# rknightion/iq-to-audio

Measured on AMD Instinct MI355X. Metric: complex IQ MS/s end-to-end (ingest->48 kHz audio), higher is better.
Workload: dtype i8; 1 GPU; BASELINE config 2: synthetic 60 s @ 10 MS/s int16 I/Q, 1 NFM channel, +25 kHz, bw 12.5 kHz, D=104, 6401 taps, chunk 4194304; frames_per_gpu=600000000, parallelism=1 independent capture(s), one per GPU; RCCL gather of 48 kHz audio only, audio_samples_48k=2879996, mix_sign=1, settle_steps=55

## Files before the change

### iq-to-audio_amd/batch.py

```python
from __future__ import annotations

from ctypes import c_int32, c_int64, c_void_p

import numpy as np

from . import _dev as D
from . import _native as N
from . import dsp_plan as P
from .decoders.side import NAMES
from .processing import (PRECISION_GUARD, ChannelBank, ChannelDemod, Channelizer, MixSignProbe, Resampler48k, _ChannelKernel,
                         base_precision, immutable_taps, pick_precision, probe_targets, reserve_pinned_scalars)


def reject_wfm(modes) -> None:
    if any((m or "").lower() == "wfm" for m in modes):
        raise ValueError("wfm targets are not supported by the resident batch runners or sharded runs: "
                         "use ProcessingPipeline / MultiChannelPipeline")


def reject_side_decoders(**flags) -> None:
    for name in NAMES:
        if flags.get(name):
            raise ValueError(f"{name}=True is not supported by the resident batch runners or sharded runs: "
                             "use ProcessingPipeline / MultiChannelPipeline")


def _rank(precision: str) -> int:
    return _ChannelKernel.PRECISIONS.index(precision)


class ResidentCaptureRunner:

    SLOTS = 3

    def __init__(self, taps: np.ndarray, *, sample_rate: float, freq_offset: float, decimation: int, fs_channel: float,
                 chunk: int, n_frames: int, demod_mode: str = "nfm", deemph_us: float = 300.0, agc_enabled: bool = True,
                 fmt: str = "s16", iq_order: str = "iq", mix_sign_override: int | None = None, precision: str | None = None,
                 precision_guard: float | None = None, slots: int | None = None, graph_streams: int = 1, pocsag: bool = False,
                 ax25: bool = False, tones: bool = False, acars: bool = False, ais: bool = False, adsb: bool = False):
        reject_wfm([demod_mode])
        reject_side_decoders(pocsag=pocsag, ax25=ax25, tones=tones, acars=acars, ais=ais, adsb=adsb)
        torch = D.torch_mod()
        if slots is not None:
            if slots < 2:
                raise ValueError("at least two slots")
            self.SLOTS = int(slots)
        self.taps, self.fs, self.f_off, self.d, self.fs_ch = immutable_taps(taps), float(sample_rate), float(freq_offset), int(decimation), float(fs_channel)
        self.chunk, self.n_frames, self.fmt, self.iq_order = int(chunk), int(n_frames), fmt, iq_order
        self.demod_args = dict(mode=demod_mode, deemph_us=deemph_us, agc_enabled=agc_enabled)
        self.override = mix_sign_override if mix_sign_override in (1, -1) else None
        self.base_precision = precision or base_precision(demod_mode, agc_enabled)
        self.guard = PRECISION_GUARD if precision_guard is None else float(precision_guard)
        self._guarded = bool(self.guard) and self.override is None and (demod_mode or "").lower() in ("nfm", "fm")
        self._spec_sign, self._spec_precision = 1, self.base_precision
        self.redone = dict(sign=0, precision=0)
        self.n_dec = -(-self.n_frames // self.d)
        self.starts = P.chunk_output_starts(self.chunk, self.d, 0, self.n_frames)
        self.rs = Resampler48k(self.fs_ch)
        self.n48 = self.rs.plan.n_out(self.n_dec)
        self.compute = torch.cuda.current_stream()
        self._compute_raw = int(self.compute.cuda_stream)
        self.aux = D.side_stream("aux")
        self.egress = D.side_stream("egress")
        self._ring_done = None
        self.slots = [dict(z=D.empty(self.n_dec, "complex64"), audio=D.empty(self.n_dec, "float32"),
                           pcm_host=torch.empty(self.n48, dtype=torch.int16).pin_memory(), busy=None,
                           dem=ChannelDemod(demod_mode, self.fs_ch, deemph_us=deemph_us, agc_enabled=agc_enabled))
                      for _ in range(self.SLOTS)]
        self._next = 0
        self._graph_streams = [D.side_stream(f"graph{i}") for i in range(int(graph_streams))] if int(graph_streams) > 1 else []
        self._egress_pending = None
        self.egress_workgroups = 8

    def _probe(self, raw_dev, resident: bool):
        if self.override is not None:
            return None
        torch = D.torch_mod()
        warm = raw_dev[: 2 * min(self.chunk, self.n_frames)] if self.fmt != "f32" else raw_dev[: min(self.chunk, self.n_frames)]
        with D.on_stream(self.aux if resident else self.compute, self.compute):
            return MixSignProbe(warm, self.fs, self.f_off, self.taps, self.d, fmt=self.fmt, iq_order=self.iq_order,
                                record_done=False, measure_level=self._guarded)

    def _kernel_for(self, sign: int):
        return lambda name: Channelizer(self.taps, sample_rate=self.fs, freq_offset=self.f_off, mix_sign=sign, decimation=self.d,
                                        fmt=self.fmt, iq_order=self.iq_order, precision=name)._kernel

    def _needed_precision(self, probe, sign: int) -> str:
        if not self._guarded or probe is None:
            return self.base_precision
        memo = self.__dict__.setdefault("_guard_memo", {}).setdefault(sign, {})
        return pick_precision(self._kernel_for(sign), self.base_precision, self.demod_args["mode"], probe.power, probe.wideband_rms,
                              self.guard, memo)

    def _chain(self, raw_dev, slot, sign: int, events=None, halo=None, resident: bool = False, probe=None, precision: str | None = None,
               make_probe=None):
        torch = D.torch_mod()
        chan = Channelizer(self.taps, sample_rate=self.fs, freq_offset=self.f_off, mix_sign=sign, decimation=self.d,
                           fmt=self.fmt, iq_order=self.iq_order, precision=precision or self.base_precision)
        chan.plan_ahead()
        dem = slot["dem"]
        side = self.aux if resident else None
        with D.on_stream(self.aux if resident else self.compute, self.compute):
            dem.reset(ahead=resident)
        dem.prepare(self.n_dec, self.starts)
        gate = None
        if events is None:
            gate = torch.cuda.Event()
            gate.record(self.compute)
        prev = self._egress_pending
        chan.process(raw_dev, out_dev=slot["z"], events=events, last_block=True, halo=halo, edge_stream=side)
        if make_probe is not None:
            probe = make_probe()
        if events is None:
            ring_done = torch.cuda.Event()
            ring_done.record(self.compute)
        else:
            gate, ring_done = events[0], events[1]
        self._ring_done = ring_done
        if prev is not None:
            self._flush_egress(gate)
        aux_done = None
        if resident:
            aux_done = torch.cuda.Event()
            aux_done.record(self.aux)
            self.compute.wait_event(aux_done)
        if probe is not None:
            probe._done = [aux_done] if resident else [gate]
        dem.process(slot["z"], self.starts, slot["audio"])
        pcm = self.rs.process(slot["audio"], want="pcm16")
        done = torch.cuda.Event()
        ticket = dict(chan=chan, dem=dem, pcm=pcm, done=done, tail_done=None, kernel=chan._kernel.last_kernel,
                      slot=slot, egress_queued=False, resident=resident, precision=chan.precision, probe=probe)
        self._egress_pending = ticket
        return ticket

    def tail_event(self, ticket: dict):
        if ticket.get("tail_done") is None:
            ev = D.torch_mod().cuda.Event()
            ev.record(self.compute)
            ticket["tail_done"] = ev
        return ticket["tail_done"]

    def _flush_egress(self, gate=None) -> None:
        t = self._egress_pending
        if t is None or t["egress_queued"]:
            return
        torch = D.torch_mod()
        if gate is not None:
            self.egress.wait_event(gate)
        else:
            self.egress.wait_event(self.tail_event(t))
        with D.on_stream(self.egress, self.compute):
            t["pcm"].record_stream(self.egress)
            host = t["slot"]["pcm_host"]
            N.call("iqa_trickle_copy", N.ptr(t["pcm"]), c_void_p(host.data_ptr()), c_int64(host.numel() * host.element_size()),
                   c_int32(self.egress_workgroups if gate is not None else max(self.egress_workgroups, 64)), N.stream_ptr())
            t["done"].record(self.egress)
        t["egress_queued"] = True
        self._egress_pending = None

    @staticmethod
    def padded_capture_frames(decimation: int, ntaps: int) -> tuple[int, int]:
        ksteps = -(-2 * decimation // 32)
        return 0, 512 * ksteps + 34 * decimation

    def submit(self, raw_dev, events=None, enclosing=None, lead_frames: int = 0, resident: bool = False) -> dict:
        torch = D.torch_mod()
        if D.current_raw_stream() != self._compute_raw:
            raise RuntimeError("submit() must be called with the stream the runner was created on as the current stream")
        slot = self.slots[self._next % self.SLOTS]
        self._next += 1
        if slot["busy"] is not None:
            self.collect(slot["busy"])
        if resident and self._ring_done is not None:
            self.aux.wait_event(self._ring_done)
        sign = self.override if self.override is not None else self._spec_sign
        halo = (enclosing, int(lead_frames)) if enclosing is not None else None
        if resident:
            ticket = self._chain(raw_dev, slot, sign, events, halo, resident, None, self._spec_precision,
                                 make_probe=lambda: self._probe(raw_dev, True))
        else:
            ticket = self._chain(raw_dev, slot, sign, events, halo, resident, self._probe(raw_dev, resident), self._spec_precision)
        ticket.update(sign=sign, raw=raw_dev, halo=halo)
        slot["busy"] = ticket
        return ticket


    def _captured_step(self, raw_dev, slot, halo):
        sign = self.override or self._spec_sign
        chan = Channelizer(self.taps, sample_rate=self.fs, freq_offset=self.f_off, mix_sign=sign, decimation=self.d,
                           fmt=self.fmt, iq_order=self.iq_order, precision=self._spec_precision)
        chan.plan_ahead()
        dem = slot["dem"]
        probe = None
        if self.override is None:
            warm = raw_dev[: 2 * min(self.chunk, self.n_frames)] if self.fmt != "f32" else raw_dev[: min(self.chunk, self.n_frames)]
            probe = MixSignProbe(warm, self.fs, self.f_off, self.taps, self.d, fmt=self.fmt, iq_order=self.iq_order, record_done=False,
                                 measure_level=self._guarded)
        dem.reset(force=True)
        dem.prepare(self.n_dec, self.starts)
        chan.process(raw_dev, out_dev=slot["z"], last_block=True, halo=halo)
        dem.process(slot["z"], self.starts, slot["audio"])
        pcm = self.rs.process(slot["audio"], want="pcm16")
        host = slot["pcm_host"]
        N.call("iqa_trickle_copy", N.ptr(pcm), c_void_p(host.data_ptr()), c_int64(host.numel() * host.element_size()),
               c_int32(max(self.egress_workgroups, 64)), N.stream_ptr())
        return dict(chan=chan, dem=dem, pcm=pcm, probe=probe, kernel=chan._kernel.last_kernel, sign=sign, precision=chan.precision)

    def submit_captured(self, raw_dev, enclosing=None, lead_frames: int = 0) -> dict:
        torch = D.torch_mod()
        if D.current_raw_stream() != self._compute_raw:
            raise RuntimeError("submit_captured() must be called with the stream the runner was created on as the current stream")
        index = self._next % self.SLOTS
        slot = self.slots[index]
        if slot["busy"] is not None:
            self.collect(slot["busy"])
        halo = (enclosing, int(lead_frames)) if enclosing is not None else None
        def graph_key():
            return (int(raw_dev.data_ptr()), index, None if enclosing is None else int(enclosing.data_ptr()), int(lead_frames),
                    self._spec_sign, self._spec_precision)

        key = graph_key()
        graphs = self.__dict__.setdefault("_graphs", {})
        entry = graphs.get(key)
        if entry is None:
            self.collect(self.submit(raw_dev, enclosing=enclosing, lead_frames=lead_frames))
            key = graph_key()
            torch.cuda.synchronize()
            reserve_pinned_scalars(1)
            g = torch.cuda.CUDAGraph()
            with torch.cuda.graph(g):
                parts = self._captured_step(raw_dev, slot, halo)
            entry = graphs[key] = dict(graph=g, **parts)
        else:
            self._next += 1
        entry["dem"].chunk_sumsq = entry["dem"].chunk_sumsq[-1:]
        done = entry.get("done_event")
        if done is None:
            done = entry["done_event"] = torch.cuda.Event()
        if self._graph_streams:
            side = self._graph_streams[index % len(self._graph_streams)]
            with torch.cuda.stream(side):
                entry["graph"].replay()
                done.record(side)
        else:
            entry["graph"].replay()
            done.record()
        ticket = dict(chan=entry["chan"], dem=entry["dem"], pcm=entry["pcm"], done=done, tail_done=done, kernel=entry["kernel"],
                      slot=slot, egress_queued=True, resident=False, probe=None, graph_probe=entry["probe"],
                      sign=entry["sign"], precision=entry["precision"], raw=raw_dev, halo=halo)
        slot["busy"] = ticket
        return ticket

    def submit_captured_batch(self, captures: list) -> list:
        torch = D.torch_mod()
        if D.current_raw_stream() != self._compute_raw:
            raise RuntimeError("submit_captured_batch() must be called with the stream the runner was created on as the current stream")
        if not 1 <= len(captures) <= self.SLOTS:
            raise ValueError(f"a batch holds 1..{self.SLOTS} captures")
        for slot in self.slots[: len(captures)]:
            if slot["busy"] is not None:
                self.collect(slot["busy"])
        halos = [(enc, int(lead)) if enc is not None else None for _, enc, lead in captures]
        def graph_key():
            return ("batch", self._spec_sign, self._spec_precision) + tuple((int(raw.data_ptr()), None if enc is None else int(enc.data_ptr()), int(lead))
                                                                            for raw, enc, lead in captures)

        key = graph_key()
        graphs = self.__dict__.setdefault("_graphs", {})
        entry = graphs.get(key)
        if entry is None:
            self._next = 0
            for raw, enc, lead in captures:
                self.collect(self.submit(raw, enclosing=enc, lead_frames=lead))
            key = graph_key()
            torch.cuda.synchronize()
            reserve_pinned_scalars(len(captures))
            g = torch.cuda.CUDAGraph()
            with torch.cuda.graph(g):
                parts = [self._captured_step(raw, slot, halo) for (raw, _, _), slot, halo in zip(captures, self.slots, halos)]
            entry = graphs[key] = dict(graph=g, parts=parts)
        for p_ in entry["parts"]:
            p_["dem"].chunk_sumsq = p_["dem"].chunk_sumsq[-1:]
        entry["graph"].replay()
        done = torch.cuda.Event()
        done.record()
        tickets = []
        for (raw, _, _), slot, halo, p_ in zip(captures, self.slots, halos, entry["parts"]):
            t = dict(chan=p_["chan"], dem=p_["dem"], pcm=p_["pcm"], done=done, tail_done=done, kernel=p_["kernel"], slot=slot,
                     egress_queued=True, resident=False, probe=None, graph_probe=p_["probe"], sign=p_["sign"], precision=p_["precision"],
                     raw=raw, halo=halo)
            slot["busy"] = t
            tickets.append(t)
        return tickets

    def collect(self, ticket: dict) -> dict:
        slot = ticket["slot"]
        if ticket.get("collected"):
            return ticket["result"]
        if ticket.get("graph_probe") is not None:
            ticket["done"].synchronize()
            sign = ticket["graph_probe"].peek()
            need = self._needed_precision(ticket["graph_probe"], sign)
            self._spec_sign, self._spec_precision = sign, need
            if sign != ticket["sign"] or _rank(need) > _rank(ticket["precision"]):
                self.replays_redone = getattr(self, "replays_redone", 0) + 1
                self.redone["sign" if sign != ticket["sign"] else "precision"] += 1
                redo = self._chain(ticket["raw"], slot, sign, None, ticket.get("halo"), False, precision=need)
                self._flush_egress()
                ticket.update(redo, sign=sign, probe=None, raw=ticket["raw"], graph_probe=None)
        if D.current_raw_stream() != self._compute_raw:
            raise RuntimeError("collect() must be called with the stream the runner was created on as the current stream")
        sign = ticket["sign"]
        if self._egress_pending is ticket:
            self._flush_egress()
        if ticket["probe"] is not None:
            sign = ticket["probe"].result()
            need = self._needed_precision(ticket["probe"], sign)
            self._spec_sign, self._spec_precision = sign, need
            if sign != ticket["sign"] or _rank(need) > _rank(ticket["precision"]):
                self.redone["sign" if sign != ticket["sign"] else "precision"] += 1
                ticket["done"].synchronize()
                probe, raw = ticket["probe"], ticket["raw"]
                redo = self._chain(raw, slot, sign, None, ticket.get("halo"), ticket.get("resident", False), precision=need)
                self._flush_egress()
                ticket.update(redo, sign=sign, probe=probe, raw=raw)
        ticket["done"].synchronize()
        ticket["collected"] = True
        ticket["raw"] = ticket["pcm"] = None
        if slot["busy"] is ticket:
            slot["busy"] = None
        ticket["result"] = dict(pcm_host=slot["pcm_host"], sign=int(sign), audio=slot["audio"], z=slot["z"],
                                kernel=ticket["kernel"], demod=ticket["dem"], done=ticket["done"], precision=ticket["precision"])
        return ticket["result"]


class ResidentBankRunner:

    SLOTS = 3

    def __init__(self, targets: list, *, sample_rate: float, n_frames: int, chunk_size: int = 1_048_576,
                 fs_ch_target: float = 96_000.0, fmt: str = "s16", iq_order: str = "iq", precision_guard: float | None = None,
                 pocsag: bool = False, ax25: bool = False, tones: bool = False, acars: bool = False, ais: bool = False, adsb: bool = False):
        reject_wfm([t.get("demod_mode") for t in targets])
        reject_side_decoders(pocsag=pocsag, ax25=ax25, tones=tones, acars=acars, ais=ais, adsb=adsb)
        torch = D.torch_mod()
        if not targets:
            raise ValueError("at least one target is required")
        self.fs, self.n_frames, self.fmt, self.iq_order = float(sample_rate), int(n_frames), fmt, iq_order
        self.d, self.fs_ch = P.choose_decimation(self.fs, fs_ch_target)
        self.chunk = P.tune_chunk_size(self.fs, chunk_size)
        self.n_dec = -(-self.n_frames // self.d)
        self.starts = P.chunk_output_starts(self.chunk, self.d, 0, self.n_frames)
        self.rs = Resampler48k(self.fs_ch)
        self.n48 = self.rs.plan.n_out(self.n_dec)
        self.targets = []
        for t in targets:
            spec = dict(bandwidth=12_500.0, demod_mode="nfm", deemph_us=300.0, agc_enabled=True, mix_sign=None, precision=None)
            spec.update(t)
            spec["taps"] = immutable_taps(P.design_channel_filter(self.fs, spec["bandwidth"], self.d))
            spec["base_precision"] = spec["precision"] or base_precision(spec["demod_mode"], spec["agc_enabled"])
            self.targets.append(spec)
        self.guard = PRECISION_GUARD if precision_guard is None else float(precision_guard)
        self._spec_sign = [1] * len(self.targets)
        self._spec_precision = [s["base_precision"] for s in self.targets]
        self.redone = dict(sign=0, precision=0)
        self.slots = []
        for _ in range(self.SLOTS):
            per = [dict(z=D.empty(self.n_dec, "complex64"), audio=D.empty(self.n_dec, "float32"),
                        pcm_host=torch.empty(self.n48, dtype=torch.int16).pin_memory(),
                        dem=ChannelDemod(s["demod_mode"], self.fs_ch, deemph_us=s["deemph_us"], agc_enabled=s["agc_enabled"]))
                   for s in self.targets]
            self.slots.append(dict(per=per, busy=None, probe_host=torch.zeros(2 * len(self.targets) + 1, dtype=torch.float64).pin_memory()))
        self._next = 0

    def _channelizer(self, spec, sign: int, precision: str | None = None) -> Channelizer:
        return Channelizer(spec["taps"], sample_rate=self.fs, freq_offset=spec["freq_offset"], mix_sign=sign, decimation=self.d,
                           fmt=self.fmt, iq_order=self.iq_order, precision=precision or spec["base_precision"])

    def _guarded(self, spec) -> bool:
        return bool(self.guard) and spec["mix_sign"] not in (1, -1) and (spec["demod_mode"] or "").lower() in ("nfm", "fm")

    def _needed_precision(self, spec, probe, sign: int) -> str:
        if probe is None or not self._guarded(spec):
            return spec["base_precision"]
        memo = spec.setdefault("_guard_memo", {}).setdefault(sign, {})
        return pick_precision(lambda name: self._channelizer(spec, sign, name)._kernel, spec["base_precision"], spec["demod_mode"],
                              probe.power, probe.wideband_rms, self.guard, memo)

    def _finish_target(self, per, raw_unused=None) -> None:
        dem = per["dem"]
        dem.reset()
        dem.process(per["z"], self.starts, per["audio"])
        pcm = self.rs.process(per["audio"], want="pcm16")
        per["pcm_host"].copy_(pcm, non_blocking=True)
        per["pcm"] = pcm

    def submit(self, raw_dev, enclosing=None, lead_frames: int = 0, events=None) -> dict:
        torch = D.torch_mod()
        slot = self.slots[self._next % self.SLOTS]
        self._next += 1
        if slot["busy"] is not None:
            self.collect(slot["busy"])
        warm = raw_dev[: 2 * min(self.chunk, self.n_frames)] if self.fmt != "f32" else raw_dev[: min(self.chunk, self.n_frames)]
        main = torch.cuda.current_stream()
        side = D.side_stream("tail")
        arrived = torch.cuda.Event()
        arrived.record(main)
        side.wait_event(arrived)
        probes = self._queue_probes(warm, slot)
        signs = [s["mix_sign"] if s["mix_sign"] in (1, -1) else sp for s, sp in zip(self.targets, self._spec_sign)]
        precisions = list(self._spec_precision)
        chans = [self._channelizer(s, sg, pr) for s, sg, pr in zip(self.targets, signs, precisions)]
        for c in chans:
            c.plan_ahead()
        halo = (enclosing, int(lead_frames)) if enclosing is not None else None
        return self._submit_rest(raw_dev, slot, probes, signs, precisions, chans, halo, events, main, side)

    def _queue_probes(self, warm, slot) -> list:
        todo = [i for i, s in enumerate(self.targets) if s["mix_sign"] not in (1, -1)]
        grouped = probe_targets(warm, self.fs, [(self.targets[i]["freq_offset"], self.targets[i]["taps"]) for i in todo], self.d,
                                fmt=self.fmt, iq_order=self.iq_order, host=slot["probe_host"]) if len(todo) > 1 else None
        if grouped is not None:
            probes = [None] * len(self.targets)
            for i, pr in zip(todo, grouped):
                probes[i] = pr
        else:
            probes = [None if s["mix_sign"] in (1, -1) else
                      MixSignProbe(warm, self.fs, s["freq_offset"], s["taps"], self.d, fmt=self.fmt, iq_order=self.iq_order,
                                   measure_level=self._guarded(s))
                      for s in self.targets]
        return probes

    def _submit_rest(self, raw_dev, slot, probes, signs, precisions, chans, halo, events, main, side) -> dict:
        torch = D.torch_mod()
        if events:
            events[0].record()
        bank = ChannelBank(chans)
        bank.process(raw_dev, outs=[p["z"] for p in slot["per"]], last_block=True, halo=halo)
        if events:
            events[1].record()
        self.last_bank_launches = getattr(bank, "launches", None) or [bank.last_launch]
        after_pass = torch.cuda.Event()
        after_pass.record(main)
        side.wait_event(after_pass)
        for per in slot["per"]:
            with D.on_stream(side, main):
                self._finish_target(per)
                for key in ("z", "audio"):
                    per[key].record_stream(side)
        done = torch.cuda.Event()
        done.record(side)
        ticket = dict(slot=slot, probes=probes, signs=signs, precisions=[c.precision for c in chans], raw=raw_dev, halo=halo, done=done,
                      launch=bank.last_launch, kernel=chans[0]._kernel.last_kernel, collected=False)
        slot["busy"] = ticket
        return ticket

    def collect(self, ticket: dict) -> list:
        if ticket["collected"]:
            return ticket["result"]
        slot = ticket["slot"]
        ticket["done"].synchronize()
        redo = False
        for i, (probe, per, spec) in enumerate(zip(ticket["probes"], slot["per"], self.targets)):
            if probe is None:
                continue
            sign = probe.result()
            need = self._needed_precision(spec, probe, sign)
            self._spec_sign[i], self._spec_precision[i] = sign, need
            if sign != ticket["signs"][i] or _rank(need) > _rank(ticket["precisions"][i]):
                self.redone["sign" if sign != ticket["signs"][i] else "precision"] += 1
                ticket["signs"][i] = sign
                chan = self._channelizer(spec, sign, need)
                ticket["precisions"][i] = chan.precision
                chan.process(ticket["raw"], out_dev=per["z"], last_block=True, halo=ticket["halo"])
                self._finish_target(per)
                redo = True
        if redo:
            D.torch_mod().cuda.current_stream().synchronize()
        ticket["collected"] = True
        ticket["raw"] = None
        if slot["busy"] is ticket:
            slot["busy"] = None
        ticket["result"] = [dict(pcm_host=per["pcm_host"], pcm=per.get("pcm"), audio=per["audio"], z=per["z"], sign=int(sg), demod=per["dem"], precision=pr)
                            for per, sg, pr in zip(slot["per"], ticket["signs"], ticket["precisions"])]
        return ticket["result"]


def demodulate_sharded(targets: list, *, sample_rate: float, n_frames: int, axis: str, capture=None, captures=None,
                       chunk_size: int = 1_048_576, fmt: str = "s16", iq_order: str = "iq", pocsag: bool = False,
                       ax25: bool = False, tones: bool = False, acars: bool = False, ais: bool = False, adsb: bool = False):
    from . import dist as DS

    reject_wfm([t.get("demod_mode") for t in targets])
    reject_side_decoders(pocsag=pocsag, ax25=ax25, tones=tones, acars=acars, ais=ais, adsb=adsb)
    torch = D.torch_mod()
    if axis not in ("channels", "captures"):
        raise ValueError("axis must be 'channels' or 'captures'")

    def run_bank(specs, raw_dev):
        runner = ResidentBankRunner(specs, sample_rate=sample_rate, n_frames=n_frames, chunk_size=chunk_size, fmt=fmt, iq_order=iq_order)
        res = runner.collect(runner.submit(raw_dev))
        return [(r["pcm"].clone(), r["demod"].peak) for r in res]

    if axis == "channels":
        dtype = {"s16": torch.int16, "u8": torch.uint8, "f32": torch.float32}[fmt]
        shared = dict(tensor=capture, numel=2 * n_frames, dtype=dtype, device=D.device())
        return DS.run_sharded(list(targets), run_bank, shared=shared)

    def every_target_of(mine, _):
        out = []
        for unit in mine:
            raw = (unit() if callable(unit) else unit).to(D.device())
            res = run_bank(list(targets), raw)
            out.append((torch.cat([a for a, _ in res]), max(p for _, p in res)))
        return out

    got, peak = DS.run_sharded(list(captures), every_target_of)
    if got is not None:
        got = {k: v.reshape(len(targets), -1) for k, v in got.items()}
    return got, peak
```

### iq-to-audio_amd/channelizer.py

```python
from __future__ import annotations

import threading
from collections import OrderedDict
from ctypes import byref, c_double, c_int32, c_int64, c_void_p

import numpy as np

from . import _dev as D
from . import _native as N
from . import dsp_plan as P
from . import iqio


def _as_frames(raw, fmt: str):
    if fmt == "f32":
        is_c = raw.is_complex() if D.is_tensor(raw) else np.iscomplexobj(raw)
        if is_c:
            x = D.to_device(raw, "complex64")
            return x, int(x.numel())
        x = D.to_device(raw, "float32").reshape(-1)
        return x, int(x.numel()) // 2
    x = D.to_device(raw, {"s16": "int16", "u8": "uint8"}[fmt]).reshape(-1)
    return x, int(x.numel()) // 2


def _block_size(n: int, ranges: int, floor: int, cap: int = 1 << 24) -> int:
    return int(min(cap, max(floor, -(-(-(-n // ranges)) // 32) * 32)))


def _tap_unit(group, fmt: str) -> float:
    return group.unit / (256.0 if fmt == "u8" else 1.0)


def _launch_lanes(lanes: list, pairs: bool, outputs_per_block: int, raw_dev, n_frames: int, consumed: int, m_first: int,
                  n_out: int) -> None:
    (k0, ps0), fmt = lanes[0][:2], lanes[0][0].plan.fmt
    table = (N.MfmaLane * len(lanes))()
    for lane, spec in zip(table, lanes):
        if spec is None:
            continue
        k, ps, z_out, partial_in, partial_out, raw_partials = spec
        group = k.mfma.groups[ps.group]
        lane.afrag_dev = k.afrag_dev[ps.group][ps.k_first * P.MFMA_KSTEP_BYTES :].data_ptr()
        lane.z_out_dev, lane.partial_in_dev, lane.partial_out_dev = z_out, partial_in, partial_out
        lane.unit = _tap_unit(group, fmt)
        lane.c_re, lane.c_im = ps.c_re, ps.c_im
        lane.rot_step, lane.rot_base = k.params.rot_step, k.params.rot_base
        lane.out_scale_re, lane.out_scale_im = k.params.out_scale_re, k.params.out_scale_im
        lane.conj_sum, lane.rotate = k.params.conj_sum, k.params.rotate
        lane.q_group, lane.finalize, lane.raw_partials = group.q, int(partial_out is None), int(raw_partials)
        lane.reserved = (0 if k.acc32 else 1) | (2 if group.high_only else 0)
        k.last_kernel = f"k_channelize_mfma_{fmt}_ring"
    N.call("iqa_channelize_mfma_pairs" if pairs else "iqa_channelize_mfma_multi", c_int32(P.FMT_CODE[fmt]),
           c_int32(k0.plan.decimation), c_int32(ps0.k_first), c_int32(ps0.k_count), c_int32(outputs_per_block), table,
           c_int32(len(lanes)), N.ptr(raw_dev), c_int64(n_frames), c_int64(consumed), c_int64(m_first), c_int64(n_out),
           N.stream_ptr())


class _ChannelKernel:

    use_mfma = True
    mfma_variant = "ring"
    ring_acc32 = True
    RING_ROWS_KSTEPS = 11
    mfma_min_outputs = 32768

    PRECISIONS = ("fast", "fine", "full", "float32")

    def __init__(self, plan: P.ChannelPlan, exact: bool = False, precision: str | None = None):
        self.plan = plan
        precision = precision or ("float32" if exact else "fast")
        if precision not in self.PRECISIONS:
            raise ValueError(f"precision must be one of {self.PRECISIONS}, not {precision!r}")
        if plan.fmt == "f32" and precision != "fast":
            precision = "float32"
        if plan.fmt == "u8" and precision == "full":
            precision = "fine"
        self.precision = precision
        self.exact = precision == "float32"
        self.variant = self.mfma_variant
        self.acc32 = bool(self.ring_acc32) and precision != "full"
        self.residual = precision in ("fine", "full")
        lpad = int(N.lib().iqa_taps_padded_len(plan.ntaps))
        if plan.taps_window.size != lpad:
            raise ValueError("tap window padding does not match the library")
        self.taps_dev = D.from_numpy(plan.taps_window)
        self.params = N.ChanParams(
            fmt=P.FMT_CODE[plan.fmt], ntaps=plan.ntaps, decimation=plan.decimation, conj_sum=plan.conj_sum,
            rotate=plan.rotate, reserved=0, rot_step=plan.rot_step, rot_base=plan.rot_base,
            out_scale_re=float(np.real(plan.out_scale)), out_scale_im=float(np.imag(plan.out_scale)),
        )
        self.mfma = None
        self._lock = threading.Lock()
        self.last_kernel = "k_channelize_v1"
        ks_all = -(-2 * plan.decimation // 32)
        self._ring_mode = 0
        if plan.fmt in ("s16", "u8") and self.variant == "ring":
            acc32, code = int(bool(self.acc32)), P.FMT_CODE[plan.fmt]
            self._ring_mode = int(N.lib().iqa_mfma_ring_mode(code, plan.decimation, 0, ks_all, acc32))
            if self._ring_mode == 0:
                self._ring_mode = int(N.lib().iqa_mfma_ring_mode(code, plan.decimation, 0, min(ks_all, self.RING_ROWS_KSTEPS), acc32))
        self._mfma_ok = bool(self.use_mfma and not self.exact and P.mfma_supported(plan) and (plan.fmt == "s16" or self._ring_mode == 2))

    def _ensure_mfma(self):
        with self._lock:
            if self.mfma is None:
                ring = self.variant == "ring" and self._ring_mode != 0
                mp = P.plan_mfma(self.plan, acc32=ring and self.acc32,
                                 max_ksteps=self.RING_ROWS_KSTEPS if self._ring_mode == 2 else None, residual=self.residual)
                self.afrag_dev = [D.from_numpy(g.afrag.reshape(-1).view(np.uint8)) for g in mp.groups]
                self._passes = [(ps, None if ring else N.MfmaParams(
                    reserved=0, unit=mp.groups[ps.group].unit, c_re=ps.c_re, c_im=ps.c_im, q_group=mp.groups[ps.group].q,
                    k_first=ps.k_first, k_count=ps.k_count)) for ps in mp.passes]
                self.mfma = mp
            return self.mfma

    def fixed_point_error_norm(self) -> float:
        return float(self._ensure_mfma().err_norm) if self._mfma_ok else 0.0

    def fixed_point_error_rms(self, wideband_rms: float) -> float:
        return float(self._ensure_mfma().z_error_rms(wideband_rms)) if self._mfma_ok else 0.0

    @staticmethod
    def _plain_range_max(k_count: int) -> int:
        lds = 160 * 1024 - k_count * P.MFMA_KSTEP_BYTES
        return int(min(6144, (lds // 16 - 160) // 32 * 32))

    launch_blocks = 256

    @classmethod
    def _block_outputs(cls, n_out: int, rmax: int, per_cu: int = 1) -> int:
        blocks = cls.launch_blocks * per_cu
        rounds = max(1, -(-n_out // (blocks * rmax)))
        return _block_size(n_out, blocks * rounds, 512, rmax)

    def _workgroups_per_cu(self, ps) -> int:
        lds = int(N.lib().iqa_mfma_ring_lds_bytes(P.FMT_CODE[self.plan.fmt], self.plan.decimation, ps.k_first, ps.k_count,
                                                  1 if self.acc32 else 0))
        return 2 if 0 < lds <= 80 * 1024 else 1

    def _valu(self, raw_dev, n_frames, consumed, hist_dev, m_first, n_out, out_dev):
        if n_out > 0:
            N.call("iqa_channelize", byref(self.params), N.ptr(self.taps_dev), N.ptr(raw_dev), c_int64(n_frames),
                   c_int64(consumed), N.ptr(hist_dev), c_int64(m_first), c_int64(n_out), N.ptr(out_dev), N.stream_ptr())

    def _interior(self, consumed: int, n_frames: int, m_first: int, n_out: int) -> tuple[int, int]:
        d = self.plan.decimation
        ksteps = -(-2 * d // 32)
        n_groups = max(1, -(-(-(-self.plan.ntaps // d)) // P.MFMA_Q))
        m_a, m_b = P.mfma_interior(consumed, n_frames, m_first, n_out, d, ksteps, n_groups)
        if self.variant == "ring" and self._ring_mode == 1:
            m_b = min(m_b, (n_frames + consumed - 512 * ksteps - 1) // d + 2)
        return (m_a, m_b) if m_b > m_a else (m_first, m_first)

    def _mfma_passes(self, raw_dev, n_frames: int, consumed: int, m_a: int, n_int: int, out_dev, min_block: int = 512):
        self._ensure_mfma()
        buf = D.empty(2 * n_int, "float64") if len(self._passes) > 1 else None
        partial = N.ptr(buf).value
        for i, (ps, prm) in enumerate(self._passes):
            last = i == len(self._passes) - 1
            partial_in, partial_out = (partial if i > 0 else None), (None if last else partial)
            if prm is None:
                rng = self._block_outputs(n_int, 1 << 24, self._workgroups_per_cu(ps))
                if min_block < 512:
                    rng = _block_size(n_int, 256, min_block, rng)
                _launch_lanes([(self, ps, out_dev.data_ptr() if last else None, partial_in, partial_out, False)], False, rng,
                              raw_dev, n_frames, consumed, m_a, n_int)
            else:
                self.last_kernel = "k_channelize_mfma_s16"
                afrag = self.afrag_dev[ps.group][ps.k_first * P.MFMA_KSTEP_BYTES :]
                with self._lock:
                    prm.outputs_per_block = self._block_outputs(n_int, self._plain_range_max(ps.k_count))
                    prm.finalize = int(last)
                    prm.partial_in_dev, prm.partial_out_dev = partial_in, partial_out
                    N.call("iqa_channelize_mfma", byref(self.params), byref(prm), N.ptr(afrag), N.ptr(raw_dev),
                           c_int64(n_frames), c_int64(consumed), c_int64(m_a), c_int64(n_int), N.ptr(out_dev), N.stream_ptr())

    def run_interior_only(self, raw_dev, n_frames: int, m_first: int, n_out: int, out_dev) -> bool:
        if not (self._mfma_ok and self.variant == "ring" and self._ring_mode) or n_out < 64:
            return False
        m_a, m_b = self._interior(0, n_frames, m_first, n_out)
        if m_a != m_first or m_b != m_first + n_out:
            return False
        self._mfma_passes(raw_dev, n_frames, 0, m_first, n_out, out_dev, min_block=64)
        return True

    def _edges(self, edge_stream, *args):
        if edge_stream is None:
            return self._valu(*args)
        with D.torch_mod().cuda.stream(edge_stream):
            self._valu(*args)

    def run(self, raw_dev, n_frames: int, consumed: int, hist_dev, m_first: int, n_out: int, out_dev=None,
            events=None, halo=None, edge_stream=None):
        if out_dev is None:
            out_dev = D.empty(n_out, "complex64")
        self.last_kernel = "k_channelize_v1"
        if self._mfma_ok and n_out >= self.mfma_min_outputs:
            big, big_frames, big_consumed = raw_dev, n_frames, consumed
            if halo is not None:
                big, lead = halo
                big_frames, big_consumed = int(big.numel()) // 2, consumed - int(lead)
            m_a, m_b = self._interior(big_consumed, big_frames, m_first, n_out)
            if m_b - m_a >= self.mfma_min_outputs:
                self._edges(edge_stream, raw_dev, n_frames, consumed, hist_dev, m_first, m_a - m_first, out_dev)
                if events:
                    events[0].record()
                self._mfma_passes(big, big_frames, big_consumed, m_a, m_b - m_a, out_dev[m_a - m_first :])
                if events:
                    events[1].record()
                self._edges(edge_stream, raw_dev, n_frames, consumed, hist_dev, m_b, m_first + n_out - m_b,
                            out_dev[m_b - m_first :])
                return out_dev
        if events:
            events[0].record()
        self._valu(raw_dev, n_frames, consumed, hist_dev, m_first, n_out, out_dev)
        if events:
            events[1].record()
        return out_dev


_KERNEL_CACHE: "OrderedDict[tuple, tuple]" = OrderedDict()
_KERNEL_CACHE_MAX = 192
_KERNEL_CACHE_LOCK = threading.Lock()


_TAPS_MEMO: dict = {}


def _taps_fingerprint(taps: np.ndarray):
    frozen = (not taps.flags.writeable) and taps.base is None
    if frozen:
        memo = _TAPS_MEMO.get(id(taps))
        if memo is not None and memo[0] is taps:
            return memo[1], memo[2]
    raw = taps.tobytes()
    h = hash(raw)
    if frozen:
        with _KERNEL_CACHE_LOCK:
            if len(_TAPS_MEMO) >= 64:
                _TAPS_MEMO.clear()
            _TAPS_MEMO[id(taps)] = (taps, raw, h)
    return raw, h


def immutable_taps(taps) -> np.ndarray:
    out = np.array(taps, copy=True, order="C")
    out.setflags(write=False)
    return out


def _cached_kernel(taps: np.ndarray, *, sample_rate: float, freq_offset: float, mix_sign: int, decimation: int,
                   fmt: str, iq_order: str, exact: bool = False, precision: str | None = None):
    taps = np.ascontiguousarray(taps)
    raw, raw_hash = _taps_fingerprint(taps)
    key = (raw_hash, taps.dtype.str, taps.shape, float(sample_rate), float(freq_offset), int(mix_sign), int(decimation),
           fmt, iq_order, _ChannelKernel.use_mfma, _ChannelKernel.mfma_variant, _ChannelKernel.ring_acc32,
           precision or ("float32" if exact else "fast"), D.torch_mod().cuda.current_device())
    with _KERNEL_CACHE_LOCK:
        hit = _KERNEL_CACHE.get(key)
        if hit is not None and (hit[0] is raw or hit[0] == raw):
            _KERNEL_CACHE.move_to_end(key)
            return hit[1], hit[2]
    lpad = int(N.lib().iqa_taps_padded_len(len(taps)))
    plan = P.plan_channel(taps, sample_rate=sample_rate, freq_offset=freq_offset, mix_sign=mix_sign,
                          decimation=decimation, fmt=fmt, iq_order=iq_order, padded_len=lpad)
    kernel = _ChannelKernel(plan, exact, precision)
    with _KERNEL_CACHE_LOCK:
        _KERNEL_CACHE[key] = (raw, plan, kernel)
        while len(_KERNEL_CACHE) > _KERNEL_CACHE_MAX:
            _KERNEL_CACHE.popitem(last=False)
    return plan, kernel


class Channelizer:

    def __init__(self, taps: np.ndarray, *, sample_rate: float, freq_offset: float, mix_sign: int, decimation: int,
                 fmt: str = "s16", iq_order: str = "iq", exact: bool = False, precision: str | None = None):
        self.plan, self._kernel = _cached_kernel(taps, sample_rate=sample_rate, freq_offset=freq_offset, mix_sign=mix_sign,
                                                 decimation=decimation, fmt=fmt, iq_order=iq_order, exact=exact, precision=precision)
        self.precision = self._kernel.precision
        self.fmt = fmt
        self.decimation = int(decimation)
        self.ntaps = len(taps)
        self.consumed = 0
        self._hist = None

    def plan_ahead(self) -> None:
        if self._kernel._mfma_ok:
            self._kernel._ensure_mfma()

    def outputs_for(self, n_frames: int) -> tuple[int, int]:
        d = self.decimation
        m_first = -(-self.consumed // d)
        m_end = -(-(self.consumed + n_frames) // d)
        return m_first, m_end - m_first

    def process(self, raw, out_dev=None, events=None, last_block: bool = False, halo=None, edge_stream=None):
        x, n = _as_frames(raw, self.fmt)
        if n == 0:
            return D.like_input(D.empty(0, "complex64"), raw)
        m_first, n_out = self.outputs_for(n)
        if halo is not None and (self.fmt not in ("s16", "u8") or not D.is_tensor(raw)):
            halo = None
        z = None
        if n_out and D.is_tensor(raw) and self._several_lanes():
            if events:
                events[0].record()
            zs = ChannelBank([self])._run_shared(x, n, m_first, n_out, [out_dev], halo, edge_stream)
            if zs is not None:
                z = zs[0]
                if events:
                    events[1].record()
        if z is None:
            z = (self._kernel.run(x, n, self.consumed, self._hist, m_first, n_out, out_dev, events, halo, edge_stream)
                 if n_out else D.empty(0, "complex64"))
        self._advance(x, n, last_block)
        return D.like_input(z, raw)

    def _several_lanes(self) -> bool:
        k = self._kernel
        if not (self.lanes_for_groups and self.fmt in ("s16", "u8") and ChannelBank._lane_capable(k)):
            return False
        return len(k._ensure_mfma().groups) > 1

    lanes_for_groups = True

    def _advance(self, x, n: int, last_block: bool = False) -> None:
        keep = 0 if last_block else self.ntaps - 1
        if keep:
            nxt = D.empty(keep * iqio.FRAME_BYTES[self.fmt], "uint8")
            N.call("iqa_history_update", c_int32(P.FMT_CODE[self.fmt]), c_int32(self.ntaps), N.ptr(self._hist),
                   N.ptr(x), c_int64(n), N.ptr(nxt), N.stream_ptr())
            self._hist = nxt
        self.consumed += n


class ChannelBank:

    MAX_LANES = 16
    pair_lanes = True

    def __init__(self, channelizers: list):
        if not channelizers:
            raise ValueError("a bank needs at least one channelizer")
        self.chans = list(channelizers)
        first = self.chans[0]
        self.fmt, self.decimation = first.fmt, first.decimation
        for c in self.chans:
            if (c.fmt, c.decimation, c.consumed) != (self.fmt, self.decimation, first.consumed):
                raise ValueError("the channels of a bank share the capture: same sample format, decimation and position")
        self.last_launch = None

    @staticmethod
    def _lane_capable(k) -> bool:
        return bool(k._mfma_ok and k.variant == "ring" and k._ring_mode and (k.acc32 or k._ring_mode == 1))

    def _shared_shape(self) -> bool:
        ks = [c._kernel for c in self.chans]
        if not ks or not all(self._lane_capable(k) for k in ks) or len({k.acc32 for k in ks}) != 1:
            return False
        if len(ks) == 1:
            return len(ks[0]._ensure_mfma().groups) > 1
        return len({k._ring_mode for k in ks}) == 1

    def process(self, raw, outs=None, last_block: bool = False, halo=None, edge_stream=None) -> list:
        x, n = _as_frames(raw, self.fmt)
        outs = list(outs) if outs is not None else [None] * len(self.chans)
        first = self.chans[0]
        m_first, n_out = first.outputs_for(n)
        zs = None
        if n and n_out and D.is_tensor(raw) and self._shared_shape():
            zs = self._run_shared(x, n, m_first, n_out, outs, halo, edge_stream)
        if zs is None:
            self.last_launch = None
            capable = [i for i, c in enumerate(self.chans) if self._lane_capable(c._kernel)]
            widths = sorted({self.chans[i]._kernel.acc32 for i in capable}, reverse=True)
            if D.is_tensor(raw) and capable and (len(capable) < len(self.chans) or len(widths) > 1):
                res = [None] * len(self.chans)
                self.last_launch, self.launches = None, []
                for acc32 in widths:
                    lanes = [i for i in capable if self.chans[i]._kernel.acc32 == acc32]
                    sub = ChannelBank([self.chans[i] for i in lanes])
                    got = sub.process(raw, outs=[outs[i] for i in lanes], last_block=last_block, halo=halo, edge_stream=edge_stream)
                    self.launches.append(sub.last_launch)
                    if self.last_launch is None:
                        self.last_launch = sub.last_launch
                    for i, z in zip(lanes, got):
                        res[i] = z
                for i, (c, o) in enumerate(zip(self.chans, outs)):
                    if res[i] is None:
                        res[i] = c.process(raw, out_dev=o, last_block=last_block, halo=halo)
                return res
            return [c.process(raw, out_dev=o, last_block=last_block, halo=halo) for c, o in zip(self.chans, outs)]
        for c in self.chans:
            c._advance(x, n, last_block)
        return zs

    def run_interior_only(self, x_all, n_frames: int, m_first: int, n_out: int, outs: list) -> bool:
        if n_out < 64 or not self._shared_shape():
            return False
        kernels = [c._kernel for c in self.chans]
        plans = [k._ensure_mfma() for k in kernels]
        if len(kernels) > self.MAX_LANES or any(len(mp.groups) != 1 or len(mp.passes) != 1 for mp in plans):
            return self._run_shared(x_all, n_frames, m_first, n_out, list(outs), None, None, interior_only=True) is not None
        if any(k._interior(0, n_frames, m_first, n_out) != (m_first, m_first + n_out) for k in kernels):
            return False
        if len({(mp.passes[0].k_first, mp.passes[0].k_count) for mp in plans}) != 1:
            return False
        rng = _block_size(n_out, 8 * max(1, (_ChannelKernel.launch_blocks // 8) // len(kernels)), 64)
        _launch_lanes([(k, mp.passes[0], z.data_ptr(), None, None, False) for k, mp, z in zip(kernels, plans, outs)], False,
                      rng, x_all, n_frames, 0, m_first, n_out)
        self.last_launch = dict(lanes=len(kernels), launches=1, combines=0, pairs=0)
        return True

    def _run_shared(self, x, n: int, m_first: int, n_out: int, outs: list, halo, edge_stream=None, interior_only: bool = False):
        kernels = [c._kernel for c in self.chans]
        consumed = self.chans[0].consumed
        big, big_frames, big_consumed = x, n, consumed
        if halo is not None:
            big, lead = halo
            big_frames, big_consumed = int(big.numel()) // 2, consumed - int(lead)
        spans = [k._interior(big_consumed, big_frames, m_first, n_out) for k in kernels]
        m_a, m_b = max(s[0] for s in spans), min(s[1] for s in spans)
        if interior_only:
            if any(s != (m_first, m_first + n_out) for s in spans):
                return None
        elif any(s[1] <= s[0] for s in spans) or m_b - m_a < _ChannelKernel.mfma_min_outputs:
            return None
        n_int = m_b - m_a
        plans = [k._ensure_mfma() for k in kernels]
        if len({tuple((ps.k_first, ps.k_count) for ps in mp.passes if ps.group == 0) for mp in plans}) != 1:
            return None
        zs = [o if o is not None else D.empty(n_out, "complex64") for o in outs]
        if not interior_only:
            for c, k, z in zip(self.chans, kernels, zs):
                k._edges(edge_stream, x, n, consumed, c._hist, m_first, m_a - m_first, z)
                k._edges(edge_stream, x, n, consumed, c._hist, m_b, m_first + n_out - m_b, z[m_b - m_first :])
        kranges = [(ps.k_first, ps.k_count) for ps in plans[0].passes if ps.group == 0]
        ids = [(ci, gi) for ci, mp in enumerate(plans) for gi in range(len(mp.groups))]
        need_partial = {(ci, gi): (len(kranges) > 1 or len(plans[ci].groups) > 1) for ci, gi in ids}
        acc32 = bool(kernels[0].acc32)
        raw = len(kranges) == 1 and acc32
        partial = {key: D.empty(2 * n_int, "int32" if raw else "float64") for key, needed in need_partial.items() if needed}
        cpx = max(1, _ChannelKernel.launch_blocks // 8)
        launches = 0

        def launch(part, pairs: bool, units: int) -> None:
            nonlocal launches
            rng = _block_size(n_int, 8 * max(1, cpx // units), 128)
            for ri, (k_first, _) in enumerate(kranges):
                lanes = []
                for ident in part:
                    if ident is None:
                        lanes.append(None)
                        continue
                    ci, gi = ident
                    mp = plans[ci]
                    ps = next(p_ for p_ in mp.passes if p_.group == gi and p_.k_first == k_first)
                    fin = ri == len(kranges) - 1 and len(mp.groups) == 1
                    buf = partial.get((ci, gi))
                    lanes.append((kernels[ci], ps, zs[ci][m_a - m_first :].data_ptr() if fin else None,
                                  buf.data_ptr() if (buf is not None and ri > 0) else None, None if fin else buf.data_ptr(),
                                  raw and not fin))
                _launch_lanes(lanes, pairs, rng, big, big_frames, big_consumed, m_a, n_int)
                launches += 1

        if self.pair_lanes and len(kranges) == 1 and (N.lib().iqa_mfma_ring_lanes(P.FMT_CODE[self.fmt], self.decimation, *kranges[0], int(acc32)) & 2):
            paired = sorted(ids, key=lambda i: -plans[i[0]].groups[i[1]].q)
            if len(paired) & 1:
                paired.append(None)
            for lo in range(0, len(paired), self.MAX_LANES):
                part = paired[lo : lo + self.MAX_LANES]
                launch(part, True, len(part) // 2)
            n_pairs = len(paired) // 2
        else:
            n_pairs = 0
            for lo in range(0, len(ids), self.MAX_LANES):
                part = ids[lo : lo + self.MAX_LANES]
                launch(part, False, len(part))
        main = None
        if edge_stream is not None and any(len(mp.groups) > 1 for mp in plans):
            torch = D.torch_mod()
            main = torch.cuda.current_stream()
            passed = torch.cuda.Event()
            passed.record(main)
            edge_stream.wait_event(passed)
            for t in partial.values():
                t.record_stream(edge_stream)
            torch.cuda.set_stream(edge_stream)
        try:
            combines = self._combine(plans, kernels, partial, raw, m_a, m_first, n_int, zs)
        finally:
            if main is not None:
                D.torch_mod().cuda.set_stream(main)
        self.last_launch = dict(lanes=len(ids), launches=launches, combines=combines, pairs=n_pairs)
        return zs

    def _combine(self, plans, kernels, partial, raw, m_a, m_first, n_int, zs) -> int:
        combines = 0
        for ci, mp in enumerate(plans):
            if len(mp.groups) > 1:
                ptrs = (c_void_p * len(mp.groups))(*[partial[(ci, gi)].data_ptr() for gi in range(len(mp.groups))])
                scale = None
                if raw:
                    vals = []
                    for gi in range(len(mp.groups)):
                        ps = next(p_ for p_ in mp.passes if p_.group == gi)
                        vals += [_tap_unit(mp.groups[gi], self.fmt), ps.c_re, ps.c_im]
                    scale = (c_double * len(vals))(*vals)
                N.call("iqa_mfma_combine", byref(kernels[ci].params), ptrs, c_int32(len(mp.groups)), scale, c_int64(m_a),
                       c_int64(n_int), N.ptr(zs[ci][m_a - m_first :]), N.stream_ptr())
                combines += 1
        return combines
```

### iq-to-audio_amd/csrc/channelize_mfma.hip

```cpp
#include "mfma_common.h"

#include <atomic>
#include <cmath>
#include <type_traits>

namespace iqa {

__global__ __launch_bounds__(MF_THREADS, 2) void k_channelize_mfma_s16(MfmaArgs a)
{
    extern __shared__ __attribute__((aligned(16))) char smem[];
    const int tid = threadIdx.x, lane = tid & 63, wave = tid >> 6;
    const int col = lane & 31, h = lane >> 5;

    const long long i0 = static_cast<long long>(blockIdx.x) * a.range;
    const int cnt = static_cast<int>(min(static_cast<long long>(a.range), a.n_out - i0));
    const long long m0 = a.m_lo + i0;
    const int tiles = (cnt + 63 + 31) >> 5;
    const int acc_len = tiles * 32 + MF_Q + 4;

    const bool stamp = (a.debug & 2) && a.stamps != nullptr;
    unsigned long long t_begin = 0, t_loop0 = 0, t_scatter = 0, t_loop1 = 0;
    if (stamp) t_begin = __builtin_amdgcn_s_memtime();
    v4i_t *s_a = reinterpret_cast<v4i_t *>(smem);
    int *s_acc = reinterpret_cast<int *>(smem + static_cast<size_t>(a.ksteps) * MF_KSTEP_BYTES);
    {
        const int n16 = a.ksteps * (MF_KSTEP_BYTES / 16);
        for (int i0f = tid; i0f < n16; i0f += MF_THREADS * 8) {
            v4i_t tmp[8];
#pragma unroll
            for (int u = 0; u < 8; ++u) {
                const int i = i0f + u * MF_THREADS;
                tmp[u] = (i < n16) ? a.afrag[i] : v4i_t{0, 0, 0, 0};
            }
#pragma unroll
            for (int u = 0; u < 8; ++u) {
                const int i = i0f + u * MF_THREADS;
                if (i < n16) s_a[i] = tmp[u];
            }
        }
    }
    for (int i = tid; i < 4 * acc_len; i += MF_THREADS) s_acc[i] = 0;
    __syncthreads();

    int pf_tile = wave, pf_ks = 0;
    auto row_ptr = [&](int tile) -> const int * {
        const long long b = m0 - MF_Q - a.col_shift + tile * 32 + col;
        return a.raw + (b * a.D + 1 - a.consumed) + 16 * a.k_first + 8 * h;
    };
    const int *pf_row = row_ptr(min(pf_tile, tiles - 1));
#define MF_LOAD_PAIR(X0, X1)                                                        \
    {                                                                               \
        X0 = *reinterpret_cast<const v4i_a4 *>(pf_row + 16 * pf_ks);                \
        X1 = *reinterpret_cast<const v4i_a4 *>(pf_row + 16 * pf_ks + 4);            \
        if (++pf_ks == a.ksteps) {                                                  \
            pf_ks = 0;                                                              \
            pf_tile += MF_WAVES;                                                    \
            pf_row = row_ptr(min(pf_tile, tiles - 1));   \
        }                                                                           \
    }
    v4i_t a0, a1, b0, b1;
    MF_LOAD_PAIR(a0, a1);
    MF_LOAD_PAIR(b0, b1);
    v4i_t fr[2 * MF_ROWTILES];
    {
        const v4i_t *fa = s_a + lane;
#pragma unroll
        for (int i = 0; i < 2 * MF_ROWTILES; ++i) fr[i] = fa[i * 64];
    }
    v16i_t acc1[MF_ROWTILES], acc2[MF_ROWTILES];
#pragma unroll
    for (int rt = 0; rt < MF_ROWTILES; ++rt) {
        acc1[rt] = v16i_t{0};
        acc2[rt] = v16i_t{0};
    }
    const v16i_t zero16 = {0, 0, 0, 0, 0, 0, 0, 0, 0, 0, 0, 0, 0, 0, 0, 0};
    if (stamp) t_loop0 = __builtin_amdgcn_s_memtime();
    int t = wave, ks = 0;
    const bool skip_scatter = (a.debug & 1) != 0;

#define MF_PAIR(X0, X1)                                                                              \
    {                                                                                                \
        v4i_t hi, lo;                                                                                \
        hi.x = __builtin_amdgcn_perm(X0.y, X0.x, 0x07050301);                                        \
        hi.y = __builtin_amdgcn_perm(X0.w, X0.z, 0x07050301);                                        \
        hi.z = __builtin_amdgcn_perm(X1.y, X1.x, 0x07050301);                                        \
        hi.w = __builtin_amdgcn_perm(X1.w, X1.z, 0x07050301);                                        \
        lo.x = __builtin_amdgcn_perm(X0.y, X0.x, 0x06040200) ^ 0x80808080;                           \
        lo.y = __builtin_amdgcn_perm(X0.w, X0.z, 0x06040200) ^ 0x80808080;                           \
        lo.z = __builtin_amdgcn_perm(X1.y, X1.x, 0x06040200) ^ 0x80808080;                           \
        lo.w = __builtin_amdgcn_perm(X1.w, X1.z, 0x06040200) ^ 0x80808080;                           \
        MF_LOAD_PAIR(X0, X1);                                                                        \
        const int kn = (ks + 1 < a.ksteps) ? ks + 1 : 0;                                             \
        const v4i_t *fa = s_a + kn * (MF_KSTEP_BYTES / 16) + lane;                                   \
        if (ks == 0) {      \
            _Pragma("unroll") for (int rt = 0; rt < MF_ROWTILES; ++rt)                               \
            {                                                                                        \
                acc1[rt] = __builtin_amdgcn_mfma_i32_32x32x32_i8(fr[2 * rt], hi, zero16, 0, 0, 0);   \
                acc2[rt] = __builtin_amdgcn_mfma_i32_32x32x32_i8(fr[2 * rt], lo, zero16, 0, 0, 0);   \
                acc2[rt] = __builtin_amdgcn_mfma_i32_32x32x32_i8(fr[2 * rt + 1], hi, acc2[rt], 0, 0, 0); \
                fr[2 * rt] = fa[(2 * rt) * 64];                                                      \
                fr[2 * rt + 1] = fa[(2 * rt + 1) * 64];                                              \
            }                                                                                        \
        } else {                                                                                     \
            _Pragma("unroll") for (int rt = 0; rt < MF_ROWTILES; ++rt)                               \
            {                                                                                        \
                acc1[rt] = __builtin_amdgcn_mfma_i32_32x32x32_i8(fr[2 * rt], hi, acc1[rt], 0, 0, 0); \
                acc2[rt] = __builtin_amdgcn_mfma_i32_32x32x32_i8(fr[2 * rt], lo, acc2[rt], 0, 0, 0); \
                acc2[rt] = __builtin_amdgcn_mfma_i32_32x32x32_i8(fr[2 * rt + 1], hi, acc2[rt], 0, 0, 0); \
                fr[2 * rt] = fa[(2 * rt) * 64];                                                      \
                fr[2 * rt + 1] = fa[(2 * rt + 1) * 64];                                              \
            }                                                                                        \
        }                                                                                            \
        if (++ks == a.ksteps) {    \
            unsigned long long ts0 = 0;                                                              \
            if (stamp) ts0 = __builtin_amdgcn_s_memtime();                                           \
            if (!skip_scatter) {                                                                     \
                int *base = s_acc + (t * 32 + col + 4 * h + 1);                                      \
                _Pragma("unroll") for (int rt = 0; rt < MF_ROWTILES; ++rt)                           \
                {                                                                                    \
                    int *p1 = base + (rt >> 1) * acc_len + (rt & 1) * 32;                            \
                    int *p2 = p1 + 2 * acc_len;                                                      \
                    _Pragma("unroll") for (int r = 0; r < 16; ++r)                                   \
                    {                                                                                \
                        const int off = (r & 3) + 8 * (r >> 2);                                      \
                        atomicAdd(p1 + off, acc1[rt][r]);                                            \
                        atomicAdd(p2 + off, acc2[rt][r]);                                            \
                    }                                                                                \
                }                                                                                    \
            } else {                                                                                 \
                _Pragma("unroll") for (int rt = 0; rt < MF_ROWTILES; ++rt)                           \
                    asm volatile("" ::"v"(acc1[rt]), "v"(acc2[rt]));                                 \
            }                                                                                        \
            if (stamp) {                                                                             \
                asm volatile("s_waitcnt lgkmcnt(0)" ::: "memory");                                   \
                t_scatter += __builtin_amdgcn_s_memtime() - ts0;                                     \
            }                                                                                        \
            ks = 0;                                                                                  \
            t += MF_WAVES;                                                                           \
        }                                                                                            \
    }

    while (t < tiles) {
        MF_PAIR(a0, a1);
        if (t >= tiles) break;
        MF_PAIR(b0, b1);
    }
#undef MF_PAIR
#undef MF_LOAD_PAIR
    if (stamp) t_loop1 = __builtin_amdgcn_s_memtime();
    __syncthreads();

    mfma_emit<MF_THREADS>(a, s_acc, acc_len, cnt, i0, m0, tid);
    if (stamp && lane == 0) {
        const unsigned long long t_end = __builtin_amdgcn_s_memtime();
        unsigned long long *o = a.stamps + (static_cast<size_t>(blockIdx.x) * MF_WAVES + wave) * 8;
        o[0] = t_loop0 - t_begin;
        o[1] = t_loop1 - t_loop0;
        o[2] = t_scatter;
        o[3] = t_end - t_loop1;
        o[4] = static_cast<unsigned long long>((tiles - wave + MF_WAVES - 1) / MF_WAVES);
    }
}

}

using namespace iqa;

extern "C" int64_t iqa_mfma_ring_bytes(int32_t decimation)
{
    if (decimation < 1 || !mfma_ring_supported(decimation)) return 0;
    return static_cast<int64_t>(mfma_ring_lds_bytes((2 * decimation + 31) / 32, false, false));
}

extern "C" int64_t iqa_mfma_ring_lds_bytes(int32_t fmt, int32_t decimation, int32_t k_first, int32_t k_count, int32_t acc32)
{
    if (decimation < 1 || (fmt != IQA_FMT_S16 && fmt != IQA_FMT_U8)) return 0;
    const int ks_all = (2 * decimation + 31) / 32;
    const int ks = k_count > 0 ? k_count : ks_all - k_first;
    const int mode = mfma_ring_mode(decimation, k_first, ks, acc32 == 0, fmt == IQA_FMT_U8);
    return mode ? static_cast<int64_t>(mfma_ring_lds_bytes(ks, mode == 2, fmt == IQA_FMT_U8)) : 0;
}

extern "C" int32_t iqa_mfma_ring_mode(int32_t fmt, int32_t decimation, int32_t k_first, int32_t k_count, int32_t acc32)
{
    if (decimation < 1 || (fmt != IQA_FMT_S16 && fmt != IQA_FMT_U8)) return 0;
    return mfma_ring_mode(decimation, k_first, k_count, acc32 == 0, fmt == IQA_FMT_U8);
}

extern "C" int64_t iqa_mfma_afrag_bytes(int32_t decimation)
{
    if (decimation < 1) return 0;
    const int64_t ksteps = (2 * static_cast<int64_t>(decimation) + 31) / 32;
    return ksteps * MF_KSTEP_BYTES;
}

static int channelize_mfma_lanes(int32_t fmt, int32_t decimation, int32_t k_first, int32_t k_count, int32_t outputs_per_block,
                                 const iqa_mfma_lane *lanes, int32_t n_lanes, const void *raw_dev, int64_t n_frames, int64_t consumed,
                                 int64_t m_first, int64_t n_out, void *stream, bool pairs);

extern "C" int iqa_channelize_mfma(const iqa_chan_params *p, const iqa_mfma_params *q, const void *afrag_dev,
                                   const void *raw_dev, int64_t n_frames, int64_t consumed, int64_t m_first,
                                   int64_t n_out, void *z_out_dev, void *stream)
{
    if (p == nullptr || q == nullptr) return fail_inval("params is NULL");
    const bool ring = (q->reserved & 64) != 0;
    if (p->fmt != IQA_FMT_S16 && !(p->fmt == IQA_FMT_U8 && ring))
        return fail_inval("the MFMA channelizer takes int16 captures (and uint8 ones with the ring variant) only");
    if (p->ntaps <= 0 || p->decimation < 1) return fail_inval("bad ntaps/decimation");
    const int64_t D = p->decimation;
    if (n_out < 0 || n_frames < 0 || m_first < 0) return fail_inval("negative size");
    if (n_out == 0) return IQA_OK;
    if (!afrag_dev || !raw_dev || !z_out_dev) return fail_inval("NULL device pointer");
    const int ksteps_all = static_cast<int>((2 * D + 31) / 32);
    const int k_first = q->k_first;
    const int ksteps = q->k_count > 0 ? q->k_count : ksteps_all - k_first;
    if (k_first < 0 || ksteps <= 0 || k_first + ksteps > ksteps_all) return fail_inval("bad k-step range");
    if (q->q_group < 0) return fail_inval("bad q group");
    if (!q->finalize && !q->partial_out_dev) return fail_inval("non-final pass needs partial_out_dev");
    int range = q->outputs_per_block;
    if (range <= 0 || (range & 31)) return fail_inval("outputs_per_block must be a positive multiple of 32");
    if (ring) {
        iqa_mfma_lane l{};
        l.afrag_dev = afrag_dev;
        l.z_out_dev = z_out_dev;
        l.partial_in_dev = q->partial_in_dev;
        l.partial_out_dev = q->partial_out_dev;
        l.unit = q->unit;
        l.c_re = q->c_re;
        l.c_im = q->c_im;
        l.rot_step = p->rot_step;
        l.rot_base = p->rot_base;
        l.out_scale_re = p->out_scale_re;
        l.out_scale_im = p->out_scale_im;
        l.q_group = q->q_group;
        l.finalize = q->finalize;
        l.conj_sum = p->conj_sum;
        l.rotate = p->rotate;
        l.reserved = (q->reserved & 128) ? 0 : 1;
        return channelize_mfma_lanes(p->fmt, p->decimation, k_first, ksteps, range, &l, 1, raw_dev, n_frames, consumed, m_first, n_out,
                                     stream, false);
    }
    const int64_t blocks = (n_out + range - 1) / range;
    const int64_t last_cnt = n_out - (blocks - 1) * range;
    const int64_t last_tiles = (last_cnt + 63 + 31) / 32;
    const int64_t col_shift = static_cast<int64_t>(MF_Q) * q->q_group;
    const int64_t b_min = m_first - MF_Q - col_shift;
    const int64_t b_max = m_first + (blocks - 1) * range - MF_Q - col_shift + last_tiles * 32 - 1;
    const int64_t f_min = b_min * D + 1 - consumed;
    const int64_t f_max = b_max * D + 1 - consumed + 16LL * (k_first + ksteps) - 1;
    const int64_t full_tiles = (static_cast<int64_t>(range) + 63 + 31) / 32;
    const int64_t b_max_full = blocks > 1 ? m_first + (blocks - 2) * range - MF_Q - col_shift + full_tiles * 32 - 1 : b_max;
    const int64_t f_max_full = b_max_full * D + 1 - consumed + 16LL * (k_first + ksteps) - 1;
    if (f_min < 0 || f_max >= n_frames || f_max_full >= n_frames)
        return fail_inval("MFMA channelizer range reads outside the block (use iqa_channelize for the edges)");
    const int64_t acc_len = full_tiles * 32 + MF_Q + 4;
    const size_t lds = static_cast<size_t>(ksteps) * MF_KSTEP_BYTES + 4 * acc_len * sizeof(int);
    if (lds > 160 * 1024) return fail_inval("tap fragments + accumulators exceed 160 KiB of LDS");

    MfmaArgs a{};
    a.afrag = static_cast<const v4i_t *>(afrag_dev);
    a.raw = static_cast<const int *>(raw_dev);
    a.out = static_cast<float2 *>(z_out_dev);
    a.consumed = consumed;
    a.m_lo = m_first;
    a.n_out = n_out;
    a.D = static_cast<int>(D);
    a.ksteps = ksteps;
    a.range = range;
    a.k_first = k_first;
    a.col_shift = static_cast<int>(col_shift);
    a.finalize = q->finalize;
    a.partial_in = static_cast<const double2 *>(q->partial_in_dev);
    a.partial_out = static_cast<double2 *>(q->partial_out_dev);
    a.debug = q->reserved;
    a.stamps = static_cast<unsigned long long *>(q->debug_stamps);
    a.unit = q->unit;
    a.c_re = q->c_re;
    a.c_im = q->c_im;
    a.conj_sum = p->conj_sum;
    a.rotate = p->rotate;
    a.rot_step = p->rot_step;
    a.rot_base = p->rot_base;
    a.sc_re = p->out_scale_re;
    a.sc_im = p->out_scale_im;
    {
        static std::atomic<unsigned long long> done{0};
        int dev = 0;
        (void)hipGetDevice(&dev);
        const unsigned long long bit = 1ull << (dev & 63);
        if (!(done.load(std::memory_order_acquire) & bit)) {
            const hipError_t e = hipFuncSetAttribute(reinterpret_cast<const void *>(k_channelize_mfma_s16),
                                                     hipFuncAttributeMaxDynamicSharedMemorySize, 160 * 1024);
            if (e != hipSuccess) {
                set_error("k_channelize_mfma_s16: cannot raise the dynamic LDS limit on device %d: %s", dev, hipGetErrorString(e));
                return IQA_EHIP;
            }
            done.fetch_or(bit, std::memory_order_release);
        }
    }
    hipLaunchKernelGGL(k_channelize_mfma_s16, dim3(static_cast<unsigned>(blocks)), dim3(MF_THREADS), lds,
                       as_stream(stream), a);
    return check_launch("k_channelize_mfma_s16");
}


static int channelize_mfma_lanes(int32_t fmt, int32_t decimation, int32_t k_first, int32_t k_count, int32_t outputs_per_block,
                                 const iqa_mfma_lane *lanes, int32_t n_lanes, const void *raw_dev, int64_t n_frames, int64_t consumed,
                                 int64_t m_first, int64_t n_out, void *stream, bool pairs)
{
    if (lanes == nullptr || n_lanes < 1) return fail_inval("no lanes");
    const bool u8 = fmt == IQA_FMT_U8;
    if (fmt != IQA_FMT_S16 && !u8) return fail_inval("the MFMA channelizer takes int16 and uint8 captures only");
    if (decimation < 1) return fail_inval("bad decimation");
    const int64_t D = decimation;
    if (n_out < 0 || n_frames < 0 || m_first < 0) return fail_inval("negative size");
    if (n_out == 0) return IQA_OK;
    if (!raw_dev) return fail_inval("NULL device pointer");
    const int ksteps_all = static_cast<int>((2 * D + 31) / 32);
    const int ksteps = k_count > 0 ? k_count : ksteps_all - k_first;
    if (k_first < 0 || ksteps <= 0 || k_first + ksteps > ksteps_all) return fail_inval("bad k-step range");
    const int range = outputs_per_block;
    if (range <= 0 || (range & 31)) return fail_inval("outputs_per_block must be a positive multiple of 32");
    const bool acc64 = (lanes[0].reserved & 1) != 0;
    for (int i = 1; i < n_lanes; ++i)
        if (lanes[i].afrag_dev && ((lanes[i].reserved & 1) != 0) != acc64) return fail_inval("the lanes of a launch share the sum width (reserved bit 0)");
    const int ring_mode = mfma_ring_mode(static_cast<int>(D), k_first, ksteps, acc64, u8);
    if (ring_mode == 0) return fail_inval("the ring kernel does not cover this (decimation, k-step range, sum width): see iqa_mfma_ring_mode");
    if (acc64 && ring_mode != 1) return fail_inval("64-bit sums: contiguous slots only");
    if (pairs && !mfma_ring_pairs_supported(static_cast<int>(D), k_first, ksteps, u8, acc64))
        return fail_inval("lane pairs are not available for this (format, decimation, k-step range, sum width): see iqa_mfma_ring_lanes");
    int q_max = 0, q_min = INT32_MAX;
    for (int i = 0; i < n_lanes; ++i) {
        if (lanes[i].q_group < 0) return fail_inval("bad q group");
        if (!lanes[i].afrag_dev) {
            if (pairs && (i & 1)) continue;
            return fail_inval("lane without tap fragments");
        }
        if (lanes[i].finalize ? !lanes[i].z_out_dev : !lanes[i].partial_out_dev) return fail_inval("lane without an output buffer");
        q_max = lanes[i].q_group > q_max ? lanes[i].q_group : q_max;
        q_min = lanes[i].q_group < q_min ? lanes[i].q_group : q_min;
    }
    const int64_t blocks = (n_out + range - 1) / range;
    const int64_t last_cnt = n_out - (blocks - 1) * range;
    const int64_t last_tiles = (last_cnt + 63 + 31) / 32, full_tiles = (static_cast<int64_t>(range) + 63 + 31) / 32;
    const int64_t f_min = (m_first - MF_Q - static_cast<int64_t>(MF_Q) * q_max) * D + 1 - consumed;
    const int64_t tail = ring_mode == 1 ? 512LL * ksteps : 16LL * (k_first + ksteps);
    const int64_t b_last = m_first - MF_Q - static_cast<int64_t>(MF_Q) * q_min;
    const int64_t t_last = b_last + (blocks - 1) * range + (last_tiles - 1) * 32;
    const int64_t t_full = blocks > 1 ? b_last + (blocks - 2) * range + (full_tiles - 1) * 32 : t_last;
    const int64_t row_span = ring_mode == 1 ? 0 : 31;
    if (f_min < 0 || (t_last + row_span) * D + 1 - consumed + tail > n_frames || (t_full + row_span) * D + 1 - consumed + tail > n_frames)
        return fail_inval("multi-lane ring launch reads outside the block (use iqa_channelize for the edges)");
    const size_t lds = mfma_ring_lds_bytes(ksteps, ring_mode == 2, u8);
    if (lds == 0 || lds > 160 * 1024) return fail_inval("ring + window exceed 160 KiB of LDS");

    MfmaArgs a{};
    a.raw = static_cast<const int *>(raw_dev);
    a.consumed = consumed;
    a.m_lo = m_first;
    a.n_out = n_out;
    a.D = static_cast<int>(D);
    a.ksteps = ksteps;
    a.range = range;
    a.k_first = k_first;
    a.debug = 64 | (acc64 ? 0 : 128);
    MfmaLane packed[16];
    if (n_lanes > 16) return fail_inval("at most 16 lanes per launch");
    for (int i = 0; i < n_lanes; ++i) {
        const iqa_mfma_lane &s = lanes[i];
        MfmaLane &l = packed[i];
        l.afrag = static_cast<const v4i_t *>(s.afrag_dev);
        l.out = static_cast<float2 *>(s.z_out_dev);
        l.partial_in = static_cast<const double2 *>(s.partial_in_dev);
        l.partial_out = static_cast<double2 *>(s.partial_out_dev);
        l.unit = s.unit;
        l.c_re = s.c_re;
        l.c_im = s.c_im;
        l.rot_step = s.rot_step;
        l.rot_base = s.rot_base;
        const unsigned long long st = s.rot_step * 64ULL;
        const double turns = static_cast<double>(st >> 11) * (1.0 / 9007199254740992.0);
        l.rot64_re = std::cos(2.0 * M_PI * turns);
        l.rot64_im = std::sin(2.0 * M_PI * turns);
        l.sc_re = s.out_scale_re;
        l.sc_im = s.out_scale_im;
        l.col_shift = MF_Q * s.q_group;
        l.finalize = s.finalize;
        l.conj_sum = s.conj_sum;
        l.rotate = s.rotate;
        l.raw_partials = (s.raw_partials != 0 && !s.finalize && !s.partial_in_dev) ? 1 : 0;
        if (s.raw_partials && !l.raw_partials) return fail_inval("raw partials need finalize == 0 and no partial_in");
        if (s.raw_partials && acc64) return fail_inval("raw partials are int32 sums: not with 64-bit sums");
        l.high_taps_only = (s.reserved & 2) != 0 ? 1 : 0;
    }
    return mfma_ring_launch_multi(a, packed, n_lanes, lds, as_stream(stream), ring_mode == 2, u8, pairs, acc64);
}

extern "C" int iqa_channelize_mfma_multi(int32_t fmt, int32_t decimation, int32_t k_first, int32_t k_count,
                                         int32_t outputs_per_block, const iqa_mfma_lane *lanes, int32_t n_lanes,
                                         const void *raw_dev, int64_t n_frames, int64_t consumed, int64_t m_first,
                                         int64_t n_out, void *stream)
{
    return channelize_mfma_lanes(fmt, decimation, k_first, k_count, outputs_per_block, lanes, n_lanes, raw_dev, n_frames, consumed,
                                 m_first, n_out, stream, false);
}

extern "C" int iqa_channelize_mfma_pairs(int32_t fmt, int32_t decimation, int32_t k_first, int32_t k_count,
                                         int32_t outputs_per_block, const iqa_mfma_lane *lanes, int32_t n_lanes,
                                         const void *raw_dev, int64_t n_frames, int64_t consumed, int64_t m_first,
                                         int64_t n_out, void *stream)
{
    return channelize_mfma_lanes(fmt, decimation, k_first, k_count, outputs_per_block, lanes, n_lanes, raw_dev, n_frames, consumed,
                                 m_first, n_out, stream, true);
}

extern "C" int32_t iqa_mfma_ring_lanes(int32_t fmt, int32_t decimation, int32_t k_first, int32_t k_count, int32_t acc32)
{
    if (decimation < 1 || (fmt != IQA_FMT_S16 && fmt != IQA_FMT_U8)) return 0;
    const bool u8 = fmt == IQA_FMT_U8, acc64 = acc32 == 0;
    const int ks_all = (2 * decimation + 31) / 32;
    const int ks = k_count > 0 ? k_count : ks_all - k_first;
    const int mode = mfma_ring_mode(decimation, k_first, ks, acc64, u8);
    if (mode == 0 || (acc64 && mode != 1)) return 0;
    return 1 | (mfma_ring_pairs_supported(decimation, k_first, ks, u8, acc64) ? 2 : 0);
}

extern "C" int32_t iqa_mfma_ring_pairs(int32_t fmt, int32_t decimation, int32_t k_first, int32_t k_count)
{
    if (decimation < 1 || fmt != IQA_FMT_S16) return 0;
    const int ks_all = (2 * decimation + 31) / 32;
    return mfma_ring_pairs_supported(decimation, k_first, k_count > 0 ? k_count : ks_all - k_first, false) ? 1 : 0;
}

namespace iqa {
struct CombineArgs {
    const double2 *part[16];
    double unit[16], c_re[16], c_im[16];
    int raw;
    int n_parts;
    float2 *out;
    long long m_first, n_out;
    int conj_sum, rotate;
    unsigned long long rot_step, rot_base;
    float sc_re, sc_im;
};

__global__ __launch_bounds__(256) void k_mfma_combine(CombineArgs a)
{
    const long long i = static_cast<long long>(blockIdx.x) * 256 + threadIdx.x;
    if (i >= a.n_out) return;
    auto part = [&](int k) -> double2 {
        if (!a.raw) return a.part[k][i];
        const int2 v = reinterpret_cast<const int2 *>(a.part[k])[i];
        return make_double2(mfma_scaled_sum(static_cast<double>(v.x), a.c_re[k], a.unit[k]),
                            mfma_scaled_sum(static_cast<double>(v.y), a.c_im[k], a.unit[k]));
    };
    double2 d = part(0);
    for (int k = 1; k < a.n_parts; ++k) {
        const double2 v = part(k);
        d.x = __dadd_rn(v.x, d.x);
        d.y = __dadd_rn(v.y, d.y);
    }
    double cs = 1.0, sn = 0.0;
    if (a.rotate) {
        const unsigned long long ph = a.rot_base + static_cast<unsigned long long>(a.m_first + i) * a.rot_step;
        sincospi(2.0 * (static_cast<double>(ph >> 11) * (1.0 / 9007199254740992.0)), &sn, &cs);
    }
    a.out[i] = mfma_finish(d.x, d.y, a.conj_sum, a.rotate, cs, sn, a.sc_re, a.sc_im);
}
}

extern "C" int iqa_mfma_combine(const iqa_chan_params *p, const void *const *partials_dev, int32_t n_partials,
                                const double *raw_scale, int64_t m_first, int64_t n_out, void *z_out_dev, void *stream)
{
    if (p == nullptr || partials_dev == nullptr) return fail_inval("params is NULL");
    if (n_partials < 1 || n_partials > 16) return fail_inval("1..16 partial buffers");
    if (n_out < 0 || m_first < 0) return fail_inval("negative size");
    if (n_out == 0) return IQA_OK;
    if (!z_out_dev) return fail_inval("NULL device pointer");
    CombineArgs a{};
    for (int k = 0; k < n_partials; ++k) {
        if (!partials_dev[k]) return fail_inval("NULL partial buffer");
        a.part[k] = static_cast<const double2 *>(partials_dev[k]);
    }
    a.n_parts = n_partials;
    a.raw = raw_scale != nullptr;
    for (int k = 0; k < n_partials && raw_scale; ++k) {
        a.unit[k] = raw_scale[3 * k];
        a.c_re[k] = raw_scale[3 * k + 1];
        a.c_im[k] = raw_scale[3 * k + 2];
    }
    a.out = static_cast<float2 *>(z_out_dev);
    a.m_first = m_first;
    a.n_out = n_out;
    a.conj_sum = p->conj_sum;
    a.rotate = p->rotate;
    a.rot_step = p->rot_step;
    a.rot_base = p->rot_base;
    a.sc_re = p->out_scale_re;
    a.sc_im = p->out_scale_im;
    hipLaunchKernelGGL(k_mfma_combine, dim3(static_cast<unsigned>((n_out + 255) / 256)), dim3(256), 0, as_stream(stream), a);
    return check_launch("k_mfma_combine");
}
```

### iq-to-audio_amd/csrc/channelize_ring.hip

```cpp
#include "mfma_common.h"

#include <atomic>
#include <mutex>
#include <cmath>
#include <type_traits>

namespace iqa {

typedef __attribute__((address_space(3))) void ring_lds_t;

constexpr int RG_WAVES = 8;

constexpr int RG_MAX_KS = 16;
constexpr int RG_ROWS_MAX_KS_C = 11;
constexpr int RG_W = 512;
constexpr int RG_GUARD = 64;
constexpr int RG_AS = RG_W + RG_GUARD;
constexpr int RG_ACC_BYTES = 2 * RG_AS * 8;
constexpr int RG_EMIT_WAVE = 2;
constexpr int RG_EMIT_LAG = 3;
constexpr unsigned int RG_PACE_AHEAD = 2;
constexpr int RG_PACE_SPINS = 20000;
constexpr int RG_PACE_WORDS = 16384;
constexpr int RG_PAIR_IDLE = 1 << 28;
constexpr int RG_LOADERS_MAX_KS = 13;
constexpr int RG_ROUNDS_MAX = 5;
constexpr int RG_PAIR_ROUNDS = 3;
constexpr int RG_PD = 2;

__device__ __forceinline__ void ring_dma16(const void *src, ring_lds_t *dst)
{
#if defined(__HIP_DEVICE_COMPILE__)
    __builtin_amdgcn_global_load_lds(src, dst, 16, 0, 0);
#else
    (void)src;
    (void)dst;
#endif
}

__device__ __forceinline__ unsigned lds_addr(const void *p)
{
    return static_cast<unsigned>(reinterpret_cast<size_t>((__attribute__((address_space(3))) const void *)p));
}

template <int KS, bool ROWS, bool U8 = false, bool PAIR = false>
struct RingGeo {
    static_assert(ROWS || !U8, "uint8 captures use row-staged slots");
    static_assert(!PAIR || (!ROWS && !U8), "lane pairs: contiguous slots only");
    static constexpr int TPR = PAIR ? 1 : 2;
    static constexpr int ACCS = PAIR ? 2 : 1;
    static constexpr int KBYTES = U8 ? 32 : 64;
    static constexpr int PITCH = KBYTES * KS + 16;
    static constexpr bool PADDED = KS <= 13;
    static constexpr int NI = 2 * KS + 1;
    static constexpr int UNITS_ROW = PITCH / 16;
    static constexpr int NI_ROWS = (32 * UNITS_ROW + 63) / 64;
    static constexpr int SLOT_RAW = ROWS ? (32 * PITCH > 1024 * NI_ROWS ? 32 * PITCH : 1024 * NI_ROWS) : 1024 * NI;
    static constexpr bool LOADERS = (!PAIR && (ROWS || KS <= RG_LOADERS_MAX_KS)) || (PAIR && KS <= 13);
    static constexpr bool SPLIT = LOADERS && !U8;
    static constexpr int PLANE_PITCH = 32 * KS + 16;
    static constexpr int SPLIT_F = PAIR ? 3 : 2;
    static constexpr int NLOADERS = SPLIT ? 4 : (LOADERS ? 2 : 0);
    static constexpr int SLOT = SPLIT ? 64 * PLANE_PITCH : SLOT_RAW;
    static constexpr int NDMA = ROWS ? NI_ROWS : (LOADERS ? NI : KS + 1);
    static constexpr int FIT = (160 * 1024 - ACCS * RG_ACC_BYTES) / (TPR * SLOT);
    static constexpr int RMAX = 63 / NDMA + 2;
    static constexpr int R0 = FIT < RMAX ? FIT : RMAX;
    static constexpr int RCAP = PAIR ? RG_PAIR_ROUNDS : RG_ROUNDS_MAX;
    static constexpr int R = SPLIT ? 2 : R0 > RCAP ? RCAP : (R0 < 2 ? 2 : R0);
    static constexpr int THREADS = (RG_WAVES + NLOADERS) * kWave;
    static constexpr int LDS_BYTES = R * TPR * SLOT + ACCS * RG_ACC_BYTES;
    static_assert(LDS_BYTES <= 160 * 1024, "ring + window exceed LDS");
    static_assert((R - 2) * NDMA <= 63, "vmcnt is a 6-bit counter");
};

struct RingCtx {
    char *smem;
    int *s_acc;
    const char *stream0;
    long long tile_bytes, i0, m0;
    int tiles, rounds, cnt, lane_off, rt, cp, col, h, lane;
    int row_units, pitch_units;
    int tshift;
    int half_last;
};

__device__ __forceinline__ int ring_src_off(int idx, int lane, int row_units, int pitch_units)
{
    const int q = 64 * idx + lane;
    int r = q / pitch_units;
    int u = q - r * pitch_units;
    if (r > 31) {
        r = 31;
        u = row_units - 1;
    }
    return (r * row_units + min(u, row_units - 1)) * 16;
}

struct RingEmit {
    double wc, ws;
};

struct RingEmitRegs {
    double v_re, v_im;
    double2 pr;
    int i;
};

template <bool ACC64, bool EARLY>
__device__ __forceinline__ void ring_emit_load(const MfmaArgs &a, const RingCtx &c, int k, RingEmitRegs &g)
{
    const int pos = 64 * k + 1 + c.lane;
    g.i = pos - MF_Q;
    const int s = pos & (RG_W - 1);
    if constexpr (ACC64) {
        long long *acc = reinterpret_cast<long long *>(c.s_acc);
        long long sr = acc[s], si = acc[RG_AS + s];
        if (s < RG_GUARD) {
            sr += acc[RG_W + s];
            si += acc[RG_AS + RG_W + s];
            acc[RG_W + s] = 0;
            acc[RG_AS + RG_W + s] = 0;
        }
        acc[s] = 0;
        acc[RG_AS + s] = 0;
        const int s2r = static_cast<int>(sr), s2i = static_cast<int>(si);
        const long long s1r = (sr - s2r) >> 32, s1i = (si - s2i) >> 32;
        g.v_re = static_cast<double>(s1r) * 256.0 + static_cast<double>(s2r);
        g.v_im = static_cast<double>(s1i) * 256.0 + static_cast<double>(s2i);
    } else {
        int *acc = c.s_acc;
        int sr = acc[s], si = acc[RG_AS + s];
        if (s < RG_GUARD) {
            sr += acc[RG_W + s];
            si += acc[RG_AS + RG_W + s];
            acc[RG_W + s] = 0;
            acc[RG_AS + RG_W + s] = 0;
        }
        acc[s] = 0;
        acc[RG_AS + s] = 0;
        g.v_re = static_cast<double>(sr);
        g.v_im = static_cast<double>(si);
    }
    g.pr = make_double2(0.0, 0.0);
    if constexpr (EARLY) {
        if (a.partial_in != nullptr && g.i >= 0 && g.i < c.cnt) g.pr = a.partial_in[c.i0 + g.i];
    }
}

template <bool EARLY>
__device__ __forceinline__ void ring_emit_store(const MfmaArgs &a, const RingCtx &c, RingEmit &e, const RingEmitRegs &g)
{
    const int i = g.i;
    if (i >= 0 && i < c.cnt) {
        double d_re = mfma_scaled_sum(g.v_re, a.c_re, a.unit);
        double d_im = mfma_scaled_sum(g.v_im, a.c_im, a.unit);
        if (a.partial_in != nullptr) {
            const double2 pr = EARLY ? g.pr : a.partial_in[c.i0 + i];
            d_re = __dadd_rn(d_re, pr.x);
            d_im = __dadd_rn(d_im, pr.y);
        }
        if (!a.finalize) {
            if (a.raw_partials)
                reinterpret_cast<int2 *>(a.partial_out)[c.i0 + i] = make_int2(static_cast<int>(g.v_re), static_cast<int>(g.v_im));
            else
                a.partial_out[c.i0 + i] = make_double2(d_re, d_im);
        } else {
            a.out[c.i0 + i] = mfma_finish(d_re, d_im, a.conj_sum, a.rotate, e.wc, e.ws, a.sc_re, a.sc_im);
        }
    }
    const double nc = e.wc * a.rot64_re - e.ws * a.rot64_im;
    e.ws = fma(e.wc, a.rot64_im, e.ws * a.rot64_re);
    e.wc = nc;
}

template <bool ACC64>
__device__ __forceinline__ void ring_emit_group(const MfmaArgs &a, const RingCtx &c, RingEmit &e, int k)
{
    RingEmitRegs g;
    ring_emit_load<ACC64, false>(a, c, k, g);
    ring_emit_store<false>(a, c, e, g);
}

template <int KS, bool ROWS, bool U8, bool PAIR = false>
__device__ __forceinline__ void ring_wait_and_barrier(int younger)
{
    using G = RingGeo<KS, ROWS, U8, PAIR>;
    constexpr int R = G::R, N = G::NDMA;
    if (R >= 5 && younger == 3) asm volatile("s_waitcnt vmcnt(%0)\n\ts_barrier" ::"n"(R >= 5 ? 3 * N : 0) : "memory");
    else if (R >= 4 && younger == 2) asm volatile("s_waitcnt vmcnt(%0)\n\ts_barrier" ::"n"(R >= 4 ? 2 * N : 0) : "memory");
    else if (R >= 3 && younger == 1) asm volatile("s_waitcnt vmcnt(%0)\n\ts_barrier" ::"n"(R >= 3 ? N : 0) : "memory");
    else asm volatile("s_waitcnt vmcnt(0)\n\ts_barrier" ::: "memory");
}

template <int KS, bool ACC64>
__device__ __forceinline__ void ring_loader(const MfmaArgs &a, const RingCtx &c)
{
    using G = RingGeo<KS, true, true>;
    constexpr int R = G::R, SLOT = G::SLOT;
    const int cp = c.cp;
    int soff[G::NI_ROWS];
    const int row_bytes = static_cast<int>(c.tile_bytes >> 5);
#pragma unroll
    for (int i = 0; i < G::NI_ROWS; ++i) {
        const int q = 64 * i + c.lane;
        int r = q / G::UNITS_ROW;
        int u = q - r * G::UNITS_ROW;
        if (r > 31) {
            r = 31;
            u = G::UNITS_ROW - 2;
        }
        soff[i] = r * row_bytes + min(u, G::UNITS_ROW - 2) * 16;
    }
    auto issue_tile = [&](int tile, int slot) {
        const char *src = c.stream0 + static_cast<long long>(min(tile, c.tiles - 1)) * c.tile_bytes;
        char *dst = c.smem + (slot * 2 + cp) * SLOT;
#pragma unroll
        for (int i = 0; i < G::NI_ROWS; ++i)
            ring_dma16(src + soff[i], (ring_lds_t *)(dst + i * 1024));
    };
#pragma unroll
    for (int rr = 0; rr < R - 1; ++rr) issue_tile(2 * rr + cp, rr);
    RingEmit em{1.0, 0.0};
    double st_re = a.rot64_re * a.rot64_re - a.rot64_im * a.rot64_im, st_im = 2.0 * a.rot64_re * a.rot64_im;
    if (a.finalize && a.rotate) {
        const unsigned long long m = static_cast<unsigned long long>(c.m0 + (64 * cp + 1 + c.lane - MF_Q));
        const unsigned long long ph = a.rot_base + m * a.rot_step;
        sincospi(2.0 * (static_cast<double>(ph >> 11) * (1.0 / 9007199254740992.0)), &em.ws, &em.wc);
    }
    MfmaArgs a2 = a;
    a2.rot64_re = st_re;
    a2.rot64_im = st_im;
    int slot = 0;
    for (int r = 0; r < c.rounds; ++r) {
        ring_wait_and_barrier<KS, true, true>(min(R - 2, c.rounds - 1 - r));
        if (r + R - 1 < c.rounds) issue_tile(2 * (r + R - 1) + cp, (slot == 0) ? R - 1 : slot - 1);
        if (r >= RG_EMIT_LAG && ((r - RG_EMIT_LAG) & 1) == cp) {
            asm volatile("" ::: "memory");
            ring_emit_group<ACC64>(a2, c, em, r - RG_EMIT_LAG);
            asm volatile("" ::: "memory");
        }
        slot = (slot + 1 == R) ? 0 : slot + 1;
    }
    asm volatile("s_waitcnt vmcnt(0) lgkmcnt(0)\n\ts_barrier" ::: "memory");
    const int k_last = (c.cnt + 62) >> 6;
    for (int k = max(c.rounds - RG_EMIT_LAG, 0); k <= k_last; ++k)
        if ((k & 1) == cp) ring_emit_group<ACC64>(a2, c, em, k);
}

struct __attribute__((packed, aligned(4))) ring_raw16 {
    int x, y, z, w;
};

template <int KS, bool ACC64, bool ROWS, int HALF, bool PAIR = false>
__device__ __forceinline__ void ring_loader_split(const MfmaArgs &a, const RingCtx &c)
{
    constexpr bool EMITTER = PAIR ? HALF < 2 : HALF == 0;
    constexpr bool UNEVEN = !PAIR && KS >= 12;
    constexpr int P0 = KS >= 12 ? KS - 2 : KS;
    constexpr int STRIDE = PAIR ? RingGeo<KS, ROWS, false, PAIR>::NLOADERS : 2;
    constexpr int NP = UNEVEN ? (HALF ? 2 * KS - P0 : P0) : (2 * KS + STRIDE - 1) / STRIDE;
    auto piece = [](int j) { return UNEVEN ? (HALF ? P0 + j : j) : STRIDE * j + HALF; };
    using G = RingGeo<KS, ROWS, false, PAIR>;
    constexpr int SLOT = G::SLOT, PP = G::PLANE_PITCH, F = G::SPLIT_F;
    const int cp = c.cp;
    const int upr = ROWS ? 4 * KS : c.row_units;
    const int row_bytes = static_cast<int>(c.tile_bytes >> 5);
    constexpr bool TABLE = KS <= 8;
    int doff[TABLE ? NP : 1], soff[TABLE ? NP : 1];
    unsigned rowu[TABLE ? 1 : (NP + 1) / 2];
    if constexpr (!TABLE) {
#pragma unroll
        for (int j = 0; j < (NP + 1) / 2; ++j) rowu[j] = 0;
    }
#pragma unroll
    for (int j = 0; j < NP; ++j) {
        const int q = 64 * piece(j) + c.lane;
        const int row = q / upr, u = q - row * upr;
        if constexpr (TABLE) {
            doff[j] = row < 32 ? row * PP + 8 * u : -1;
            soff[j] = row < 32 ? row * row_bytes + 16 * u : 31 * row_bytes + 16 * (upr - 1);
        } else {
            const unsigned f = row < 32 ? static_cast<unsigned>((row << 6) | u) : static_cast<unsigned>((31 << 6) | (upr - 1) | (1 << 11));
            rowu[j >> 1] |= f << (16 * (j & 1));
        }
    }
    int4 buf[F][NP];
    auto request = [&](int round, auto set) {
        constexpr int S = decltype(set)::value;
        const char *src = c.stream0 + static_cast<long long>(PAIR ? min(round, c.rounds - 1) : min(2 * round + cp, c.tiles - 1)) * c.tile_bytes;
#pragma unroll
        for (int j = 0; j < NP; ++j) {
            int so;
            if constexpr (TABLE) so = soff[j];
            else {
                const unsigned f = rowu[j >> 1] >> (16 * (j & 1));
                so = static_cast<int>((f >> 6) & 31u) * row_bytes + 16 * static_cast<int>(f & 63u);
            }
            const ring_raw16 t = *reinterpret_cast<const ring_raw16 *>(src + so);
            buf[S][j] = make_int4(t.x, t.y, t.z, t.w);
        }
    };
    auto stage = [&](int slot, auto set) {
        constexpr int S = decltype(set)::value;
        char *hi0 = c.smem + (PAIR ? slot : slot * 2 + cp) * SLOT;
#pragma unroll
        for (int j = 0; j < NP; ++j) {
            const int4 d = buf[S][j];
            int2 hi, lo;
            hi.x = __builtin_amdgcn_perm(d.y, d.x, 0x07050301);
            hi.y = __builtin_amdgcn_perm(d.w, d.z, 0x07050301);
            lo.x = __builtin_amdgcn_perm(d.y, d.x, 0x06040200) ^ 0x80808080;
            lo.y = __builtin_amdgcn_perm(d.w, d.z, 0x06040200) ^ 0x80808080;
            int dq;
            if constexpr (TABLE) dq = doff[j];
            else {
                const unsigned f = rowu[j >> 1] >> (16 * (j & 1));
                dq = (f & 2048u) ? -1 : static_cast<int>((f >> 6) & 31u) * PP + 8 * static_cast<int>(f & 63u);
            }
            if (dq >= 0) {
                *reinterpret_cast<int2 *>(hi0 + dq) = hi;
                *reinterpret_cast<int2 *>(hi0 + 32 * PP + dq) = lo;
            }
        }
    };
    request(0, std::integral_constant<int, 0>{});
    stage(0, std::integral_constant<int, 0>{});
    request(1, std::integral_constant<int, 1 % F>{});
    request(2, std::integral_constant<int, 2 % F>{});
    if constexpr (F == 3) request(3, std::integral_constant<int, 0>{});
    static_assert(F == 2 || F == 3, "the prologue and the unrolled loop below are written for two or three rounds in flight");
    RingEmit em{1.0, 0.0};
    double st_re = a.rot64_re * a.rot64_re - a.rot64_im * a.rot64_im, st_im = 2.0 * a.rot64_re * a.rot64_im;
    if (EMITTER && a.finalize && a.rotate) {
        const unsigned long long m = static_cast<unsigned long long>(c.m0 + ((PAIR ? 0 : 64 * cp) + 1 + c.lane - MF_Q));
        const unsigned long long ph = a.rot_base + m * a.rot_step;
        sincospi(2.0 * (static_cast<double>(ph >> 11) * (1.0 / 9007199254740992.0)), &em.ws, &em.wc);
    }
    MfmaArgs a2 = a;
    if constexpr (!PAIR) {
        a2.rot64_re = st_re;
        a2.rot64_im = st_im;
    }
    auto group_of = [&](int r) {
        if constexpr (PAIR) {
            const int re = r - c.tshift, lag = 5 + cp;
            return (re >= lag && ((re - lag) & 1) == 0) ? (re - lag) >> 1 : -1;
        } else {
            return (r >= RG_EMIT_LAG && ((r - RG_EMIT_LAG) & 1) == cp) ? r - RG_EMIT_LAG : -1;
        }
    };
    constexpr bool PR_AHEAD = PAIR || KS <= 11;
    double2 pr_next = make_double2(0.0, 0.0);
    auto round_body = [&](int r, auto set) {
        asm volatile("s_waitcnt lgkmcnt(0)\n\ts_barrier" ::: "memory");
        if (r + 1 < c.rounds) stage((r + 1) & 1, set);
        const double2 pr_now = pr_next;
        if (PR_AHEAD && EMITTER && a.partial_in != nullptr) {
            const int kn = group_of(r + 1);
            if (kn >= 0) {
                const int i = 64 * kn + 1 + c.lane - MF_Q;
                pr_next = (i >= 0 && i < c.cnt) ? a.partial_in[c.i0 + i] : make_double2(0.0, 0.0);
            }
        }
        request(r + 1 + F, set);
        const int k = EMITTER ? group_of(r) : -1;
        if (k >= 0) {
            asm volatile("" ::: "memory");
            if constexpr (PR_AHEAD) {
                RingEmitRegs g;
                ring_emit_load<ACC64, false>(a2, c, k, g);
                g.pr = pr_now;
                ring_emit_store<true>(a2, c, em, g);
            } else {
                ring_emit_group<ACC64>(a2, c, em, k);
            }
            asm volatile("" ::: "memory");
        }
    };
    int r = 0;
    if constexpr (F == 3) {
        for (; r + 3 <= c.rounds; r += 3) {
            round_body(r, std::integral_constant<int, 1>{});
            round_body(r + 1, std::integral_constant<int, 2>{});
            round_body(r + 2, std::integral_constant<int, 0>{});
        }
        if (r < c.rounds) {
            round_body(r, std::integral_constant<int, 1>{});
            if (r + 1 < c.rounds) round_body(r + 1, std::integral_constant<int, 2>{});
        }
    } else {
        for (; r + 2 <= c.rounds; r += 2) {
            round_body(r, std::integral_constant<int, 1>{});
            round_body(r + 1, std::integral_constant<int, 0>{});
        }
        if (r < c.rounds) round_body(r, std::integral_constant<int, 1>{});
    }
    asm volatile("s_waitcnt vmcnt(0) lgkmcnt(0)\n\ts_barrier" ::: "memory");
    if constexpr (EMITTER) {
        const int k_last = (c.cnt + 62) >> 6;
        if constexpr (PAIR) {
            const int own = c.rounds - c.tshift, lag = 5 + cp;
            const int k_next = own > lag ? ((own - 1 - lag) >> 1) + 1 : 0;
            if (c.tshift < RG_PAIR_IDLE)
                for (int k = k_next; k <= k_last; ++k) ring_emit_group<ACC64>(a2, c, em, k);
        } else {
            for (int k = max(c.rounds - RG_EMIT_LAG, 0); k <= k_last; ++k)
                if ((k & 1) == cp) ring_emit_group<ACC64>(a2, c, em, k);
        }
    }
}

template <int KS, bool ACC64, bool ROWS, bool U8, bool ISSUER, bool EMIT, bool DEFER, bool PAIR, typename SKIPT, bool HALF = false>
__device__ __forceinline__ void ring_main(const MfmaArgs &a, const RingCtx &c, const v4i_t (&fq)[KS][2], SKIPT)
{
    constexpr int SKIP = SKIPT::value;
    using G = RingGeo<KS, ROWS, U8, PAIR>;
    constexpr int R = G::R, SLOT = G::SLOT;
    static_assert(!(ROWS && ISSUER), "row-staged slots are always fed by loader waves");
    const int RG_EMIT_LAG_PAIR = 5 + c.cp;
    const int rt = c.rt, cp = c.cp;
    int soff[(ISSUER && G::PADDED) ? KS + 1 : 1];
    if constexpr (ISSUER && G::PADDED) {
#pragma unroll
        for (int i = 0; i <= KS; ++i) soff[i] = ring_src_off(min(2 * i + (rt & 1), 2 * KS), c.lane, c.row_units, c.pitch_units);
    } else {
        soff[0] = c.lane * 16;
    }
    const int odd_kib = (rt & 1) * 1024;
    auto issue = [&](int tile, int slot, int i) {
        const char *tile0 = c.stream0 + static_cast<long long>(min(tile, (PAIR ? c.rounds : c.tiles) - 1)) * c.tile_bytes;
        char *slot0 = c.smem + (PAIR ? slot : slot * 2 + cp) * SLOT;
        const int at = (i < KS) ? odd_kib + i * 2048 : 2 * KS * 1024;
        if constexpr (ISSUER && G::PADDED) {
            ring_dma16(tile0 + soff[i], (ring_lds_t *)(slot0 + at));
        } else {
            ring_dma16(tile0 + soff[0] + at, (ring_lds_t *)(slot0 + at));
        }
    };
    if (ISSUER) {
#pragma unroll
        for (int rr = 0; rr < R - 1; ++rr)
#pragma unroll
            for (int i = 0; i <= KS; ++i) issue(PAIR ? rr : 2 * rr + cp, rr, i);
    }
    RingEmit em{1.0, 0.0};
    if (EMIT && a.finalize && a.rotate) {
        const unsigned long long m = static_cast<unsigned long long>(c.m0 + (1 + c.lane - MF_Q));
        const unsigned long long ph = a.rot_base + m * a.rot_step;
        sincospi(2.0 * (static_cast<double>(ph >> 11) * (1.0 / 9007199254740992.0)), &em.ws, &em.wc);
    }
    const v16i_t zero16 = {0, 0, 0, 0, 0, 0, 0, 0, 0, 0, 0, 0, 0, 0, 0, 0};
    auto scatter = [&](int t, const v16i_t &acc1, const v16i_t &acc2) {
        const int slot_idx = ((t * 32 + c.col + 4 * c.h + 1) & (RG_W - 1)) + (rt >> 1) * RG_AS + (rt & 1) * 32;
        if constexpr (ACC64) {
            const unsigned p = lds_addr(reinterpret_cast<long long *>(c.s_acc) + slot_idx);
#pragma unroll
            for (int q = 0; q < 16; ++q) {
                const long long comb = (static_cast<long long>(acc1[q]) << 32) + static_cast<long long>(acc2[q]);
                const int off = 8 * ((q & 3) + 8 * (q >> 2));
                asm volatile("ds_add_u64 %0, %1 offset:%2" ::"v"(p), "v"(comb), "n"(off));
            }
        } else {
            const unsigned p = lds_addr(c.s_acc + slot_idx);
#pragma unroll
            for (int q = 0; q < 16; ++q) {
                const int comb = (acc1[q] << 8) + acc2[q];
                const int off = 4 * ((q & 3) + 8 * (q >> 2));
                asm volatile("ds_add_u32 %0, %1 offset:%2" ::"v"(p), "v"(comb), "n"(off));
            }
        }
    };
    constexpr bool DEFER_ADDS = DEFER && !G::SPLIT;
    v16i_t held1 = zero16, held2 = zero16;
    int held_t = -1;
    int slot = 0;
    bool pace_on = PAIR && a.pace != nullptr && a.pace_units > 1 && c.rounds < 8000;
    for (int r = 0; r < c.rounds; ++r) {
        if (ISSUER) ring_wait_and_barrier<KS, ROWS, U8, PAIR>(min(R - 2, c.rounds - 1 - r));
        else asm volatile("s_barrier" ::: "memory");
        if constexpr (PAIR && !ISSUER && !EMIT && !DEFER) {
            if (c.rt == 3 && c.cp == 0 && pace_on && (r & 1) == 0) {
                const unsigned int mine = static_cast<unsigned int>(r >> 1);
                if (c.lane == 0) __hip_atomic_store(a.pace + a.pace_slot, (a.pace_token << 12) | mine, __ATOMIC_RELAXED, __HIP_MEMORY_SCOPE_AGENT);
                for (int spin = 0;; ++spin) {
                    unsigned int q = mine;
                    if (c.lane < a.pace_units) {
                        const unsigned int v = __hip_atomic_load(a.pace + (a.pace_slot - a.pace_slot % a.pace_units) + c.lane, __ATOMIC_RELAXED,
                                                                 __HIP_MEMORY_SCOPE_AGENT);
                        if ((v >> 12) == a.pace_token) q = v & 0xFFFu;
                    }
#pragma unroll
                    for (int o = 1; o < 16; o <<= 1) q = min(q, static_cast<unsigned int>(__shfl_xor(static_cast<int>(q), o, kWave)));
                    q = static_cast<unsigned int>(__builtin_amdgcn_readfirstlane(static_cast<int>(q)));
                    if (mine <= q + RG_PACE_AHEAD) break;
                    if (spin >= RG_PACE_SPINS) {
                        pace_on = false;
                        break;
                    }
                    __builtin_amdgcn_s_sleep(32);
                }
            }
        }
        const bool pf = ISSUER && (r + R - 1 < c.rounds);
        const int pf_tile = PAIR ? r + R - 1 : 2 * (r + R - 1) + cp;
        const int pf_slot = (slot == 0) ? R - 1 : slot - 1;
        if (pf) {
#pragma unroll
            for (int i = 0; i <= KS; ++i) issue(pf_tile, pf_slot, i);
        }
        const int re = r - c.tshift;
        const bool emit_now = EMIT && (PAIR ? (re >= RG_EMIT_LAG_PAIR && ((re - RG_EMIT_LAG_PAIR) & 1) == 0) : re >= RG_EMIT_LAG);
        RingEmitRegs eg;
        if (emit_now) {
            asm volatile("" ::: "memory");
            ring_emit_load<ACC64, true>(a, c, PAIR ? (re - RG_EMIT_LAG_PAIR) >> 1 : re - RG_EMIT_LAG, eg);
            asm volatile("" ::: "memory");
        }
        if (DEFER_ADDS && held_t >= 0) {
            scatter(held_t, held1, held2);
            held_t = -1;
        }
        bool store_pending = emit_now;
#pragma unroll
        for (int j = 0; j < 1; ++j) {
        const int t = PAIR ? re : 2 * r + cp;
        if (t >= 0 && t < c.tiles) {
            const bool store_here = store_pending;
            store_pending = false;
            const char *la = c.smem + (PAIR ? slot : slot * 2 + cp) * SLOT + c.lane_off;
            auto tile_body = [&](auto skip_low) {
                constexpr bool SKIP_LOW = decltype(skip_low)::value;
                constexpr int PD = KS < RG_PD ? KS : RG_PD;
                v16i_t acc1, acc2;
                if constexpr (U8) {
                    v4i_t du[KS];
#pragma unroll
                    for (int ks = 0; ks < PD; ++ks) du[ks] = *reinterpret_cast<const v4i_t *>(la + 32 * ks);
#pragma unroll
                    for (int ks = 0; ks < KS; ++ks) {
                        v4i_t v = du[ks];
                        v.x ^= 0x80808080;
                        v.y ^= 0x80808080;
                        v.z ^= 0x80808080;
                        v.w ^= 0x80808080;
                        if (ks + PD < KS) du[ks + PD] = *reinterpret_cast<const v4i_t *>(la + 32 * (ks + PD));
                        acc1 = __builtin_amdgcn_mfma_i32_32x32x32_i8(fq[ks][0], v, ks ? acc1 : zero16, 0, 0, 0);
                        acc2 = __builtin_amdgcn_mfma_i32_32x32x32_i8(fq[ks][1], v, ks ? acc2 : zero16, 0, 0, 0);
                    }
                } else if constexpr (G::SPLIT) {
                    v4i_t hh[KS], ll[KS];
                    constexpr bool half_last = HALF;
                    auto fetch = [&](int ks) {
                        if (ks == KS - 1 && half_last) {
                            const int2 h2 = *reinterpret_cast<const int2 *>(la - 8 * c.h + 32 * ks);
                            const int2 l2 = *reinterpret_cast<const int2 *>(la - 8 * c.h + 32 * G::PLANE_PITCH + 32 * ks);
                            hh[ks].x = h2.x;
                            hh[ks].y = h2.y;
                            ll[ks].x = l2.x;
                            ll[ks].y = l2.y;
                        } else {
                            hh[ks] = *reinterpret_cast<const v4i_t *>(la + 32 * ks);
                            ll[ks] = *reinterpret_cast<const v4i_t *>(la + 32 * G::PLANE_PITCH + 32 * ks);
                        }
                    };
#pragma unroll
                    for (int ks = 0; ks < PD; ++ks) fetch(ks);
#pragma unroll
                    for (int ks = 0; ks < KS; ++ks) {
                        const v4i_t hi = hh[ks], lo = ll[ks];
                        if (ks + PD < KS) fetch(ks + PD);
                        if (ks == KS - 1 && half_last) {
                            auto pack = [](int x, int y) { return static_cast<long>((static_cast<unsigned long long>(static_cast<unsigned>(y)) << 32) | static_cast<unsigned>(x)); };
                            const long a1 = pack(fq[ks][0].x, fq[ks][0].y), a2 = pack(fq[ks][1].x, fq[ks][1].y);
                            const long bh = pack(hi.x, hi.y), bl = pack(lo.x, lo.y);
                            acc1 = __builtin_amdgcn_mfma_i32_32x32x16_i8(a1, bh, ks ? acc1 : zero16, 0, 0, 0);
                            acc2 = __builtin_amdgcn_mfma_i32_32x32x16_i8(a1, bl, ks ? acc2 : zero16, 0, 0, 0);
                            if constexpr (!SKIP_LOW) acc2 = __builtin_amdgcn_mfma_i32_32x32x16_i8(a2, bh, acc2, 0, 0, 0);
                        } else {
                            acc1 = __builtin_amdgcn_mfma_i32_32x32x32_i8(fq[ks][0], hi, ks ? acc1 : zero16, 0, 0, 0);
                            acc2 = __builtin_amdgcn_mfma_i32_32x32x32_i8(fq[ks][0], lo, ks ? acc2 : zero16, 0, 0, 0);
                            if constexpr (!SKIP_LOW) acc2 = __builtin_amdgcn_mfma_i32_32x32x32_i8(fq[ks][1], hi, acc2, 0, 0, 0);
                        }
                    }
                } else {
                    v4i_t dd[KS][2];
#pragma unroll
                    for (int ks = 0; ks < PD; ++ks) {
                        dd[ks][0] = *reinterpret_cast<const v4i_t *>(la + 64 * ks);
                        dd[ks][1] = *reinterpret_cast<const v4i_t *>(la + 64 * ks + 16);
                    }
#pragma unroll
                    for (int ks = 0; ks < KS; ++ks) {
                        if (EMIT && ks == KS - 3 && store_here) ring_emit_store<true>(a, c, em, eg);
                        const v4i_t d0 = dd[ks][0], d1 = dd[ks][1];
                        v4i_t hi, lo;
                        hi.x = __builtin_amdgcn_perm(d0.y, d0.x, 0x07050301);
                        hi.y = __builtin_amdgcn_perm(d0.w, d0.z, 0x07050301);
                        hi.z = __builtin_amdgcn_perm(d1.y, d1.x, 0x07050301);
                        hi.w = __builtin_amdgcn_perm(d1.w, d1.z, 0x07050301);
                        lo.x = __builtin_amdgcn_perm(d0.y, d0.x, 0x06040200) ^ 0x80808080;
                        lo.y = __builtin_amdgcn_perm(d0.w, d0.z, 0x06040200) ^ 0x80808080;
                        lo.z = __builtin_amdgcn_perm(d1.y, d1.x, 0x06040200) ^ 0x80808080;
                        lo.w = __builtin_amdgcn_perm(d1.w, d1.z, 0x06040200) ^ 0x80808080;
                        if (ks + PD < KS) {
                            dd[ks + PD][0] = *reinterpret_cast<const v4i_t *>(la + 64 * (ks + PD));
                            dd[ks + PD][1] = *reinterpret_cast<const v4i_t *>(la + 64 * (ks + PD) + 16);
                        }
                        acc1 = __builtin_amdgcn_mfma_i32_32x32x32_i8(fq[ks][0], hi, ks ? acc1 : zero16, 0, 0, 0);
                        acc2 = __builtin_amdgcn_mfma_i32_32x32x32_i8(fq[ks][0], lo, ks ? acc2 : zero16, 0, 0, 0);
                        if constexpr (!SKIP_LOW) acc2 = __builtin_amdgcn_mfma_i32_32x32x32_i8(fq[ks][1], hi, acc2, 0, 0, 0);
                    }
                }
                if (DEFER_ADDS) {
                    held1 = acc1;
                    held2 = acc2;
                    held_t = t;
                } else {
                    scatter(t, acc1, acc2);
                }
            };
            if constexpr (SKIP == 2 && !U8) {
                tile_body(std::true_type{});
            } else if constexpr (SKIP == 1 && !U8) {
                if (a.high_taps_only) tile_body(std::true_type{});
                else tile_body(std::false_type{});
            } else {
                tile_body(std::false_type{});
            }
        }
        }
        if (store_pending) ring_emit_store<true>(a, c, em, eg);
        slot = (slot + 1 == R) ? 0 : slot + 1;
    }
    if (DEFER_ADDS && held_t >= 0) scatter(held_t, held1, held2);
    asm volatile("s_waitcnt vmcnt(0) lgkmcnt(0)\n\ts_barrier" ::: "memory");
    if (EMIT) {
        const int k_last = (c.cnt + 62) >> 6;
        const int own = c.rounds - c.tshift;
        const int k_next = PAIR ? (own > RG_EMIT_LAG_PAIR ? ((own - 1 - RG_EMIT_LAG_PAIR) >> 1) + 1 : 0) : max(own - RG_EMIT_LAG, 0);
        if (!PAIR || c.tshift < RG_PAIR_IDLE)
            for (int k = k_next; k <= k_last; ++k) ring_emit_group<ACC64>(a, c, em, k);
    }
}

template <int KS, bool ACC64, bool ROWS, bool U8, bool PAIR = false, bool SKIPK = false, bool HALF = false>
__device__ __forceinline__ void ring_block(const MfmaArgs &a, long long range_idx)
{
    using G = RingGeo<KS, ROWS, U8, PAIR>;
    constexpr int R = G::R, SLOT = G::SLOT;
    constexpr bool LOADERS = G::LOADERS;
    extern __shared__ __attribute__((aligned(16))) char smem[];
    const int tid = threadIdx.x;
    const int wave = __builtin_amdgcn_readfirstlane(tid >> 6);
    RingCtx c;
    c.lane = tid & 63;
    c.rt = wave & 3;
    c.cp = wave >= RG_WAVES ? (wave - RG_WAVES) & 1 : (wave >> 2) & 1;
    c.col = c.lane & 31;
    c.h = c.lane >> 5;

    c.i0 = range_idx * a.range;
    c.cnt = static_cast<int>(min(static_cast<long long>(a.range), a.n_out - c.i0));
    c.m0 = a.m_lo + c.i0;
    c.tiles = (c.cnt + 63 + 31) >> 5;
    c.rounds = PAIR ? c.tiles + a.pair_extra : (c.tiles + 1) >> 1;
    c.tshift = PAIR ? a.pair_shift : 0;
    c.smem = smem;
    c.s_acc = reinterpret_cast<int *>(smem + R * G::TPR * SLOT);
    for (int i = tid; i < G::ACCS * RG_ACC_BYTES / 4; i += G::THREADS) c.s_acc[i] = 0;
    if (PAIR) c.s_acc += c.cp * (RG_ACC_BYTES / 4);

    constexpr int FB = U8 ? 2 : 4;
    const long long row_bytes = static_cast<long long>(FB) * a.D;
    c.tile_bytes = 32 * row_bytes;
    const char *stream = reinterpret_cast<const char *>(a.raw) + FB * ((c.m0 - MF_Q - a.col_shift) * a.D + 1 - a.consumed) +
                         (ROWS ? G::KBYTES * a.k_first : 0);
    c.row_units = static_cast<int>(row_bytes >> 4);
    c.pitch_units = G::PADDED ? (c.row_units | 1) : c.row_units;
    c.lane_off = G::SPLIT ? c.col * G::PLANE_PITCH + 16 * c.h : c.col * (ROWS ? G::PITCH : 16 * c.pitch_units) + (G::KBYTES / 2) * c.h;

    if constexpr (LOADERS) {
        if (wave >= RG_WAVES) {
            c.stream0 = stream;
            __syncthreads();
            if constexpr (G::SPLIT && PAIR) {
                switch (wave - RG_WAVES) {
                    case 0: ring_loader_split<KS, ACC64, ROWS, 0, true>(a, c); break;
                    case 1: ring_loader_split<KS, ACC64, ROWS, 1, true>(a, c); break;
                    case 2: ring_loader_split<KS, ACC64, ROWS, 2, true>(a, c); break;
                    default: ring_loader_split<KS, ACC64, ROWS, 3, true>(a, c); break;
                }
            } else if constexpr (G::SPLIT) {
                if ((wave - RG_WAVES) >> 1) ring_loader_split<KS, ACC64, ROWS, 1>(a, c);
                else ring_loader_split<KS, ACC64, ROWS, 0>(a, c);
            } else {
                ring_loader<KS, ACC64>(a, c);
            }
            return;
        }
    }
    v4i_t fq[KS][2];
    {
        const v4i_t *fa = a.afrag + c.rt * 128 + c.lane;
#pragma unroll
        for (int ks = 0; ks < KS; ++ks)
#pragma unroll
            for (int pc = 0; pc < 2; ++pc) fq[ks][pc] = fa[(ks * 8 + pc) * 64];
#pragma unroll
        for (int ks = 0; ks < KS; ++ks) asm volatile("" ::"v"(fq[ks][0]), "v"(fq[ks][1]));
    }
    c.half_last = HALF;
    if constexpr (HALF) {
        static_assert(!ROWS && !U8 && !PAIR, "the half last k step exists for single lanes over contiguous byte-plane slots");
#pragma unroll
        for (int pc = 0; pc < 2; ++pc) {
            const v4i_t f = fq[KS - 1][pc];
            const int z0 = __shfl(f.z, c.lane ^ 32, kWave), w0 = __shfl(f.w, c.lane ^ 32, kWave);
            if (c.h) {
                fq[KS - 1][pc].x = z0;
                fq[KS - 1][pc].y = w0;
            }
        }
    }
    __syncthreads();
    c.stream0 = stream;
    if constexpr (PAIR && G::SPLIT) {
        constexpr int SA = SKIPK ? 2 : 0, SB = 0;
        if (c.cp) ring_main<KS, ACC64, ROWS, U8, false, false, true, true>(a, c, fq, std::integral_constant<int, SB>{});
        else ring_main<KS, ACC64, ROWS, U8, false, false, false, true>(a, c, fq, std::integral_constant<int, SA>{});
    } else if constexpr (PAIR) {
        constexpr int SA = SKIPK ? 2 : 0, SB = 0;
        if (c.cp == 0 && c.rt < 2) ring_main<KS, ACC64, ROWS, U8, true, false, false, true>(a, c, fq, std::integral_constant<int, SA>{});
        else if (c.cp == 0 && c.rt == 2) ring_main<KS, ACC64, ROWS, U8, false, true, false, true>(a, c, fq, std::integral_constant<int, SA>{});
        else if (c.cp == 1 && c.rt == 3) ring_main<KS, ACC64, ROWS, U8, false, true, false, true>(a, c, fq, std::integral_constant<int, SB>{});
        else if (c.cp) ring_main<KS, ACC64, ROWS, U8, false, false, true, true>(a, c, fq, std::integral_constant<int, SB>{});
        else ring_main<KS, ACC64, ROWS, U8, false, false, false, true>(a, c, fq, std::integral_constant<int, SA>{});
    } else if constexpr (LOADERS) {
        constexpr int S1 = SKIPK ? 1 : 0;
        if (c.cp) ring_main<KS, ACC64, ROWS, U8, false, false, true, false, std::integral_constant<int, S1>, HALF>(a, c, fq, std::integral_constant<int, S1>{});
        else ring_main<KS, ACC64, ROWS, U8, false, false, false, false, std::integral_constant<int, S1>, HALF>(a, c, fq, std::integral_constant<int, S1>{});
    } else {
        constexpr int S1 = SKIPK ? 1 : 0;
        if ((c.rt >> 1) == c.cp) {
            if (c.cp) ring_main<KS, ACC64, ROWS, U8, true, false, true, false>(a, c, fq, std::integral_constant<int, S1>{});
            else ring_main<KS, ACC64, ROWS, U8, true, false, false, false>(a, c, fq, std::integral_constant<int, S1>{});
        } else if (wave == RG_EMIT_WAVE) ring_main<KS, ACC64, ROWS, U8, false, true, false, false>(a, c, fq, std::integral_constant<int, S1>{});
        else if (c.cp) ring_main<KS, ACC64, ROWS, U8, false, false, true, false>(a, c, fq, std::integral_constant<int, S1>{});
        else ring_main<KS, ACC64, ROWS, U8, false, false, false, false>(a, c, fq, std::integral_constant<int, S1>{});
    }
}

constexpr int RG_MAX_LANES = 16;

struct RingMultiArgs {
    MfmaArgs c;
    int n_lanes;
    MfmaLane lane[RG_MAX_LANES];
};

template <int KS, bool ROWS, bool U8, bool PAIR = false, bool ACC64 = false, bool SKIPK = false, bool HALF = false>
__device__ __forceinline__ void ring_multi_block(const RingMultiArgs &m)
{
    const int idx = blockIdx.x >> 3;
    const int units = PAIR ? m.n_lanes >> 1 : m.n_lanes;
    const int wv = __builtin_amdgcn_readfirstlane(static_cast<int>(threadIdx.x >> 6));
    const int li = PAIR ? 2 * (idx % units) + (wv >= RG_WAVES ? wv & 1 : (wv >> 2) & 1) : idx % units;
    const long long range_idx = static_cast<long long>(idx / units) * 8 + (blockIdx.x & 7);
    const MfmaLane &l = m.lane[li];
    MfmaArgs a = m.c;
    a.pair_shift = a.pair_extra = 0;
    a.afrag = l.afrag;
    a.out = l.out;
    a.partial_in = l.partial_in;
    a.partial_out = l.partial_out;
    a.unit = l.unit;
    a.c_re = l.c_re;
    a.c_im = l.c_im;
    a.rot_step = l.rot_step;
    a.rot_base = l.rot_base;
    a.rot64_re = l.rot64_re;
    a.rot64_im = l.rot64_im;
    a.sc_re = l.sc_re;
    a.sc_im = l.sc_im;
    a.col_shift = l.col_shift;
    a.finalize = l.finalize;
    a.conj_sum = l.conj_sum;
    a.rotate = l.rotate;
    a.raw_partials = l.raw_partials;
    a.high_taps_only = l.high_taps_only;
    if constexpr (PAIR) {
        const MfmaLane &la = m.lane[li & ~1], &lb = m.lane[li | 1];
        const bool idle_b = lb.afrag == nullptr;
        a.pair_extra = idle_b ? 0 : (la.col_shift - lb.col_shift) >> 5;
        a.col_shift = la.col_shift;
        if (li & 1) {
            a.pair_shift = idle_b ? RG_PAIR_IDLE : a.pair_extra;
            if (idle_b) a.afrag = la.afrag;
        }
        a.pace_units = units;
        a.pace_slot = static_cast<int>(range_idx) * units + idx % units;
    }
    if (range_idx * a.range >= a.n_out) return;
    ring_block<KS, ACC64, ROWS, U8, PAIR, SKIPK, HALF>(a, range_idx);
}

template <int KS, bool ACC64 = false, bool SKIPK = false>
__global__ __launch_bounds__((RingGeo<KS, false>::THREADS), (RingGeo<KS, false>::LOADERS ? 3 : 2)) void k_channelize_mfma_s16_ring_multi(RingMultiArgs m)
{
    ring_multi_block<KS, false, false, false, ACC64, SKIPK>(m);
}

template <int KS>
__global__ __launch_bounds__((RingGeo<KS, false>::THREADS), 3) void k_channelize_mfma_s16_ring_multi_half(RingMultiArgs m)
{
    static_assert(RingGeo<KS, false>::SPLIT, "byte-plane kernels only");
    ring_multi_block<KS, false, false, false, false, false, true>(m);
}

template <int KS, bool ACC64 = false, bool SKIPK = false>
__global__ __launch_bounds__((RingGeo<KS, false, false, true>::THREADS), (RingGeo<KS, false, false, true>::LOADERS ? 3 : 2)) void k_channelize_mfma_s16_ring_pairs(RingMultiArgs m)
{
    ring_multi_block<KS, false, false, true, ACC64, SKIPK>(m);
}

template <int KS, bool SKIPK = false>
__global__ __launch_bounds__((RingGeo<KS, true>::THREADS), 3) void k_channelize_mfma_s16_ring_rows_multi(RingMultiArgs m)
{
    ring_multi_block<KS, true, false, false, false, SKIPK>(m);
}

template <int KS>
__global__ __launch_bounds__((RingGeo<KS, true, true>::THREADS), 3) void k_channelize_mfma_u8_ring_rows_multi(RingMultiArgs m)
{
    ring_multi_block<KS, true, true>(m);
}

template <typename K, typename A>
static int ring_launch_kernel(K kernel, const char *name, int threads, const A &a, unsigned blocks, size_t lds, hipStream_t stream,
                              std::atomic<unsigned long long> &done)
{
    int dev = 0;
    (void)hipGetDevice(&dev);
    const unsigned long long bit = 1ull << (dev & 63);
    if (!(done.load(std::memory_order_acquire) & bit)) {
        const hipError_t e = hipFuncSetAttribute(reinterpret_cast<const void *>(kernel), hipFuncAttributeMaxDynamicSharedMemorySize, 160 * 1024);
        if (e != hipSuccess) {
            set_error("%s: cannot raise the dynamic LDS limit on device %d: %s", name, dev, hipGetErrorString(e));
            return IQA_EHIP;
        }
        done.fetch_or(bit, std::memory_order_release);
    }
    hipLaunchKernelGGL(kernel, dim3(blocks), dim3(threads), lds, stream, a);
    return check_launch(name);
}

template <int KS>
static int ring_launch_multi(const RingMultiArgs &m, unsigned blocks, size_t lds, hipStream_t stream, bool rows, bool u8, bool acc64, bool skipk)
{
    static std::atomic<unsigned long long> done[8] = {{0}, {0}, {0}, {0}, {0}, {0}, {0}, {0}};
    if (acc64) {
        if constexpr (KS < RG_MAX_KS) {
            if (!rows && !u8) {
                if (skipk)
                    return ring_launch_kernel(k_channelize_mfma_s16_ring_multi<KS, true, true>, "k_channelize_mfma_s16_ring_multi64", RingGeo<KS, false>::THREADS, m, blocks, lds, stream, done[4]);
                return ring_launch_kernel(k_channelize_mfma_s16_ring_multi<KS, true>, "k_channelize_mfma_s16_ring_multi64", RingGeo<KS, false>::THREADS, m, blocks, lds, stream, done[3]);
            }
        }
        set_error("multi-lane launches with 64-bit sums: contiguous int16 slots, at most %d k steps (got %d)", RG_MAX_KS - 1, KS);
        return IQA_EINVAL;
    }
    if constexpr (KS <= RG_ROWS_MAX_KS_C) {
        if (u8) return ring_launch_kernel(k_channelize_mfma_u8_ring_rows_multi<KS>, "k_channelize_mfma_u8_ring_rows_multi", RingGeo<KS, true, true>::THREADS, m, blocks, lds, stream, done[2]);
        if (rows && skipk) return ring_launch_kernel(k_channelize_mfma_s16_ring_rows_multi<KS, true>, "k_channelize_mfma_s16_ring_rows_multi", RingGeo<KS, true>::THREADS, m, blocks, lds, stream, done[5]);
        if (rows) return ring_launch_kernel(k_channelize_mfma_s16_ring_rows_multi<KS>, "k_channelize_mfma_s16_ring_rows_multi", RingGeo<KS, true>::THREADS, m, blocks, lds, stream, done[1]);
    } else {
        if (u8 || rows) {
            set_error("row-staged ring kernels take at most %d k steps per pass (got %d)", RG_ROWS_MAX_KS_C, KS);
            return IQA_EINVAL;
        }
    }
    if (skipk) return ring_launch_kernel(k_channelize_mfma_s16_ring_multi<KS, false, true>, "k_channelize_mfma_s16_ring_multi", RingGeo<KS, false>::THREADS, m, blocks, lds, stream, done[6]);
    if constexpr (KS <= 8) {
        const int rem = (2 * m.c.D) & 31;
        if (rem != 0 && rem <= 16)
            return ring_launch_kernel(k_channelize_mfma_s16_ring_multi_half<KS>, "k_channelize_mfma_s16_ring_multi", RingGeo<KS, false>::THREADS, m, blocks, lds, stream, done[7]);
    }
    return ring_launch_kernel(k_channelize_mfma_s16_ring_multi<KS>, "k_channelize_mfma_s16_ring_multi", RingGeo<KS, false>::THREADS, m, blocks, lds, stream, done[0]);
}

constexpr int RG_PAIR_MIN_KS = 9;

template <int KS>
static int ring_launch_pairs(const RingMultiArgs &m, unsigned blocks, hipStream_t stream, bool acc64, bool skipk)
{
    static std::atomic<unsigned long long> done{0}, done64{0}, done_s{0}, done64_s{0};
    if constexpr (KS >= RG_PAIR_MIN_KS && KS != 15) {
        using G = RingGeo<KS, false, false, true>;
        if (acc64) {
            if constexpr (KS <= 14) {
                if (skipk)
                    return ring_launch_kernel(k_channelize_mfma_s16_ring_pairs<KS, true, true>, "k_channelize_mfma_s16_ring_pairs64", G::THREADS, m, blocks, G::LDS_BYTES, stream, done64_s);
                return ring_launch_kernel(k_channelize_mfma_s16_ring_pairs<KS, true>, "k_channelize_mfma_s16_ring_pairs64", G::THREADS, m, blocks, G::LDS_BYTES, stream, done64);
            }
            set_error("lane pairs with 64-bit sums: 9..14 k steps (got %d)", KS);
            return IQA_EINVAL;
        }
        if (skipk) return ring_launch_kernel(k_channelize_mfma_s16_ring_pairs<KS, false, true>, "k_channelize_mfma_s16_ring_pairs", G::THREADS, m, blocks, G::LDS_BYTES, stream, done_s);
        return ring_launch_kernel(k_channelize_mfma_s16_ring_pairs<KS>, "k_channelize_mfma_s16_ring_pairs", G::THREADS, m, blocks, G::LDS_BYTES, stream, done);
    } else {
        set_error("lane pairs: %d k steps not instantiated (%d..14, 16)", KS, RG_PAIR_MIN_KS);
        return IQA_EINVAL;
    }
}

static unsigned int *ring_pace_buffer(unsigned int &token, int words, hipStream_t stream)
{
    static std::mutex mu;
    static unsigned int *buf[64] = {};
    static int next_off[64] = {};
    static unsigned int next_token = 1;
    int dev = 0;
    (void)hipGetDevice(&dev);
    std::lock_guard<std::mutex> lock(mu);
    token = next_token = (next_token % 0xFFFFFu) + 1;
    unsigned int *&b = buf[dev & 63];
    if (b == nullptr) {
        hipStreamCaptureStatus st = hipStreamCaptureStatusNone;
        if (hipStreamIsCapturing(stream, &st) != hipSuccess || st != hipStreamCaptureStatusNone) {
            (void)hipGetLastError();
            return nullptr;
        }
        void *p = nullptr;
        if (hipMalloc(&p, RG_PACE_WORDS * sizeof(unsigned int)) != hipSuccess) {
            (void)hipGetLastError();
            return nullptr;
        }
        if (hipMemset(p, 0, RG_PACE_WORDS * sizeof(unsigned int)) != hipSuccess || hipDeviceSynchronize() != hipSuccess) {
            (void)hipGetLastError();
            (void)hipFree(p);
            return nullptr;
        }
        b = static_cast<unsigned int *>(p);
    }
    if (words > RG_PACE_WORDS) return nullptr;
    int &off = next_off[dev & 63];
    if (off + words > RG_PACE_WORDS) off = 0;
    unsigned int *mine = b + off;
    off += (words + 63) & ~63;
    return mine;
}

bool mfma_ring_pairs_supported(int decimation, int k_first, int k_count, bool u8, bool acc64)
{
    return mfma_ring_mode(decimation, k_first, k_count, acc64, u8) == 1 && k_count >= RG_PAIR_MIN_KS && k_count != 15 && (!acc64 || k_count <= 14);
}

constexpr int RG_ROWS_MAX_KS = RG_ROWS_MAX_KS_C;

int mfma_ring_mode(int decimation, int k_first, int k_count, bool acc64, bool u8)
{
    const int ks_all = (2 * decimation + 31) / 32;
    if (!u8 && decimation >= 4 && (decimation & 3) == 0 && ks_all <= (acc64 ? RG_MAX_KS - 1 : RG_MAX_KS) && k_first == 0 && k_count == ks_all) return 1;
    if (!acc64 && decimation >= 1 && k_count >= 1 && k_count <= RG_ROWS_MAX_KS && k_first >= 0 && k_first + k_count <= ks_all) return 2;
    return 0;
}

bool mfma_ring_supported(int decimation)
{
    const int ks = (2 * decimation + 31) / 32;
    return decimation >= 4 && (decimation & 3) == 0 && ks <= RG_MAX_KS;
}

template <int LO, int HI, class F>
static auto with_ks(int ks, F &&f)
{
    if constexpr (LO < HI) {
        if (ks > LO) return with_ks<LO + 1, HI>(ks, f);
    }
    return f(std::integral_constant<int, LO>{});
}

template <int KS>
static constexpr size_t ring_bytes_of(bool rows, bool u8)
{
    return u8     ? static_cast<size_t>(RingGeo<KS, true, true>::R) * 2 * RingGeo<KS, true, true>::SLOT + RG_ACC_BYTES
           : rows ? static_cast<size_t>(RingGeo<KS, true>::R) * 2 * RingGeo<KS, true>::SLOT + RG_ACC_BYTES
                  : static_cast<size_t>(RingGeo<KS, false>::R) * 2 * RingGeo<KS, false>::SLOT + RG_ACC_BYTES;
}

size_t mfma_ring_lds_bytes(int ksteps, bool rows, bool u8)
{
    if (ksteps < 1 || ksteps > (rows ? RG_ROWS_MAX_KS : RG_MAX_KS)) return 0;
    return with_ks<1, RG_MAX_KS>(ksteps, [&](auto k) { return ring_bytes_of<decltype(k)::value>(rows, u8); });
}

int mfma_ring_launch_multi(const MfmaArgs &a, const MfmaLane *lanes, int n_lanes, size_t lds, hipStream_t stream, bool rows, bool u8,
                           bool pairs, bool acc64)
{
    if (n_lanes < 1 || n_lanes > RG_MAX_LANES) {
        set_error("a multi-lane launch takes 1..%d lanes (got %d)", RG_MAX_LANES, n_lanes);
        return IQA_EINVAL;
    }
    if (pairs) {
        if (rows || u8 || (n_lanes & 1)) {
            set_error("lane pairs: contiguous int16 slots and an even number of lanes");
            return IQA_EINVAL;
        }
        for (int i = 0; i < n_lanes; i += 2)
            if (lanes[i].afrag == nullptr || (lanes[i + 1].afrag != nullptr && lanes[i].col_shift < lanes[i + 1].col_shift)) {
                set_error("lane pairs: lane %d must exist and have the larger (or the same) tap-row group of its pair", i);
                return IQA_EINVAL;
            }
    }
    RingMultiArgs m;
    m.c = a;
    m.n_lanes = n_lanes;
    for (int i = 0; i < n_lanes; ++i) m.lane[i] = lanes[i];
    for (int i = n_lanes; i < RG_MAX_LANES; ++i) m.lane[i] = m.lane[0];
    bool skipk = false;
    if (!u8) {
        if (pairs) {
            skipk = true;
            for (int i = 0; i < n_lanes; i += 2)
                if (!lanes[i].high_taps_only || (lanes[i + 1].afrag != nullptr && lanes[i + 1].high_taps_only)) skipk = false;
        } else {
            for (int i = 0; i < n_lanes; ++i) skipk = skipk || lanes[i].high_taps_only != 0;
        }
    }
    if (!skipk)
        for (int i = 0; i < RG_MAX_LANES; ++i) m.lane[i].high_taps_only = 0;
    const long long ranges = (a.n_out + a.range - 1) / a.range;
    const long long groups = (ranges + 7) / 8;
    const unsigned blocks = static_cast<unsigned>(groups * (pairs ? n_lanes / 2 : n_lanes) * 8);
    if (a.ksteps < 1 || a.ksteps > RG_MAX_KS) {
        set_error("ring kernel: %d k steps not instantiated (1..%d)", a.ksteps, RG_MAX_KS);
        return IQA_EINVAL;
    }
    if (pairs) {
        m.c.pace = nullptr;
        m.c.pace = ring_pace_buffer(m.c.pace_token, static_cast<int>(std::min<long long>(groups * 8 * (n_lanes / 2), RG_PACE_WORDS + 1)), stream);
        return with_ks<1, RG_MAX_KS>(a.ksteps, [&](auto k) { return ring_launch_pairs<decltype(k)::value>(m, blocks, stream, acc64, skipk); });
    }
    return with_ks<1, RG_MAX_KS>(a.ksteps, [&](auto k) {
        return ring_launch_multi<decltype(k)::value>(m, blocks, lds, stream, rows, u8, acc64, skipk);
    });
}

}
```

### iq-to-audio_amd/csrc/mfma_common.h

```cpp
#pragma once

#include "common.h"

namespace iqa {

typedef int v4i_t __attribute__((ext_vector_type(4)));
typedef v4i_t v4i_a4 __attribute__((aligned(4)));
typedef int v16i_t __attribute__((ext_vector_type(16)));

constexpr int MF_WAVES = 8;
constexpr int MF_THREADS = MF_WAVES * kWave;
constexpr int MF_Q = 64;
constexpr int MF_ROWTILES = 4;
constexpr int MF_KSTEP_BYTES = MF_ROWTILES * 2 * 1024;

struct MfmaArgs {
    const v4i_t *afrag;
    const int *raw;
    float2 *out;
    long long consumed, m_lo, n_out;
    int D, ksteps, range, debug;
    int k_first;
    int col_shift;
    int finalize;
    const double2 *partial_in;
    double2 *partial_out;
    unsigned long long *stamps;
    double unit, c_re, c_im;
    int conj_sum, rotate;
    unsigned long long rot_step, rot_base;
    float sc_re, sc_im;
    double rot64_re, rot64_im;
    int raw_partials;
    int high_taps_only;
    int pair_shift, pair_extra;
    unsigned int *pace;
    unsigned int pace_token;
    int pace_slot, pace_units;
};

__device__ __forceinline__ double mfma_scaled_sum(double v, double c, double unit)
{
    return __dmul_rn(__fma_rn(v, 256.0, c), unit);
}
__device__ __forceinline__ float2 mfma_finish(double d_re, double d_im, int conj_sum, int rotate, double cw, double sw, float sc_re,
                                              float sc_im)
{
    if (conj_sum) d_im = -d_im;
    double yr = d_re, yi = d_im;
    if (rotate) {
        yr = __fma_rn(d_re, cw, -__dmul_rn(d_im, sw));
        yi = __fma_rn(d_re, sw, __dmul_rn(d_im, cw));
    }
    const double sr = static_cast<double>(sc_re), si = static_cast<double>(sc_im);
    return make_float2(static_cast<float>(__fma_rn(yr, sr, -__dmul_rn(yi, si))), static_cast<float>(__fma_rn(yr, si, __dmul_rn(yi, sr))));
}

template <int THREADS>
__device__ __forceinline__ void mfma_emit(const MfmaArgs &a, const int *s_acc, int acc_len, int cnt, long long i0,
                                          long long m0, int tid)
{
    for (int i = tid; i < cnt; i += THREADS) {
        const int pos = MF_Q + i;
        const double s1r = s_acc[pos], s1i = s_acc[acc_len + pos];
        const double s2r = s_acc[2 * acc_len + pos], s2i = s_acc[3 * acc_len + pos];
        double d_re = mfma_scaled_sum(s1r * 256.0 + s2r, a.c_re, a.unit);
        double d_im = mfma_scaled_sum(s1i * 256.0 + s2i, a.c_im, a.unit);
        if (a.partial_in != nullptr) {
            const double2 pr = a.partial_in[i0 + i];
            d_re = __dadd_rn(d_re, pr.x);
            d_im = __dadd_rn(d_im, pr.y);
        }
        if (!a.finalize) {
            a.partial_out[i0 + i] = make_double2(d_re, d_im);
            continue;
        }
        double cw = 1.0, sw = 0.0;
        if (a.rotate) {
            const unsigned long long m = static_cast<unsigned long long>(m0 + i);
            const unsigned long long ph = a.rot_base + m * a.rot_step;
            const double frac = static_cast<double>(ph >> 11) * (1.0 / 9007199254740992.0);
            sincospi(2.0 * frac, &sw, &cw);
        }
        a.out[i0 + i] = mfma_finish(d_re, d_im, a.conj_sum, a.rotate, cw, sw, a.sc_re, a.sc_im);
    }
}

int mfma_ring_mode(int decimation, int k_first, int k_count, bool acc64, bool u8);
bool mfma_ring_supported(int decimation);
size_t mfma_ring_lds_bytes(int ksteps, bool rows, bool u8);

struct MfmaLane {
    const v4i_t *afrag;
    float2 *out;
    const double2 *partial_in;
    double2 *partial_out;
    double unit, c_re, c_im;
    unsigned long long rot_step, rot_base;
    double rot64_re, rot64_im;
    float sc_re, sc_im;
    int col_shift, finalize, conj_sum, rotate, raw_partials, high_taps_only;
};
int mfma_ring_launch_multi(const MfmaArgs &common, const MfmaLane *lanes, int n_lanes, size_t lds_bytes, hipStream_t stream, bool rows,
                           bool u8, bool pairs, bool acc64);
bool mfma_ring_pairs_supported(int decimation, int k_first, int k_count, bool u8, bool acc64 = false);

}
```

### iq-to-audio_amd/dsp_plan.py

```python
from __future__ import annotations

import functools
import math
from dataclasses import dataclass
from fractions import Fraction

import numpy as np

MAX_CHUNK = 4_194_304
TWO64 = 1 << 64
IQ_ORDERS = ("iq", "qi", "iq_inv", "qi_inv")
INGEST_SCALE = {"s16": 1.0 / 32768.0, "u8": 1.0 / 128.0, "f32": 1.0}
FMT_CODE = {"s16": 0, "u8": 1, "f32": 2}
FMT_NUMPY = {"s16": np.int16, "u8": np.uint8, "f32": np.float32}


_CHUNK_SECONDS = ((5_000_000.0, 0.50), (2_000_000.0, 0.40), (0.0, 0.25))


def tune_chunk_size(sample_rate: float, requested: int) -> int:
    floor = max(1, requested)
    if sample_rate <= 0:
        return floor
    seconds = next(s for rate, s in _CHUNK_SECONDS if sample_rate >= rate)
    wanted = int(round(sample_rate * seconds))
    if wanted <= floor:
        return floor
    wanted = min(wanted, MAX_CHUNK)
    return int(min(max(1 << (wanted - 1).bit_length(), floor), MAX_CHUNK))


def choose_decimation(sample_rate: float, fs_ch_target: float) -> tuple[int, float]:
    decimation = max(1, int(round(sample_rate / fs_ch_target)))
    fs_channel = sample_rate / decimation
    if fs_channel > fs_ch_target * 1.5:
        decimation = max(int(math.floor(sample_rate / fs_ch_target)), 1)
        fs_channel = sample_rate / decimation
    return decimation, fs_channel


def kaiser_beta(atten_db: float) -> float:
    a = abs(atten_db)
    if a > 50:
        return 0.1102 * (a - 8.7)
    if a > 21:
        return 0.5842 * (a - 21) ** 0.4 + 0.07886 * (a - 21)
    return 0.0


def design_channel_filter(sample_rate: float, bandwidth: float, decimation: int) -> np.ndarray:
    guard = max(1_000.0, bandwidth * 0.5)
    cutoff = min(bandwidth * 0.5 * 1.05, (sample_rate / (2.0 * max(decimation, 1))) * 0.9)
    if cutoff <= 0:
        raise ValueError("Invalid cutoff frequency for channel filter.")
    width = guard / sample_rate
    num_taps = int(np.clip(4.0 / max(width, 1e-8), 1024, 32768))
    if num_taps % 2 == 0:
        num_taps += 1
    beta = kaiser_beta(80.0)
    fc = cutoff / (0.5 * sample_rate)
    m = np.arange(num_taps, dtype=np.float64) - (num_taps - 1) / 2.0
    h = fc * np.sinc(fc * m) * np.kaiser(num_taps, beta)
    return np.asarray(h / h.sum(), dtype=np.float64)


def freq_ratio_turns(freq_offset: float, sample_rate: float, sign: int) -> int:
    theta = -sign * Fraction(freq_offset) / Fraction(sample_rate)
    theta -= math.floor(theta)
    return int(round(theta * TWO64)) % TWO64


@dataclass
class ChannelPlan:

    fmt: str
    ntaps: int
    decimation: int
    taps_window: np.ndarray
    conj_sum: int
    rotate: int
    rot_step: int
    rot_base: int
    out_scale: complex
    taps_natural: np.ndarray | None = None


def plan_channel(
    taps: np.ndarray,
    *,
    sample_rate: float,
    freq_offset: float,
    mix_sign: int,
    decimation: int,
    fmt: str = "s16",
    iq_order: str = "iq",
    padded_len: int | None = None,
) -> ChannelPlan:
    if iq_order not in IQ_ORDERS:
        raise ValueError(f"Unsupported iq_order '{iq_order}'")
    if fmt not in FMT_CODE:
        raise ValueError(f"unsupported sample format {fmt!r}")
    h = np.asarray(taps, dtype=np.float64)
    ntaps = h.size
    w = freq_ratio_turns(freq_offset, sample_rate, mix_sign)
    k = np.arange(ntaps, dtype=np.uint64)
    with np.errstate(over="ignore"):
        ph = np.uint64(w) * k
    turns = (ph >> np.uint64(11)).astype(np.float64) * (2.0**-53)
    g = h * np.exp(-2j * np.pi * turns)
    conj = iq_order in ("qi", "iq_inv")
    c = {"iq": 1.0 + 0j, "qi": 1j, "iq_inv": 1.0 + 0j, "qi_inv": -1j}[iq_order]
    if conj:
        g = np.conj(g)
    g = g * INGEST_SCALE[fmt]
    lpad = padded_len if padded_len is not None else -(-ntaps // 256) * 256
    win = np.zeros(lpad, dtype=np.complex64)
    win[:ntaps] = g[::-1].astype(np.complex64)
    return ChannelPlan(
        fmt=fmt, ntaps=ntaps, decimation=int(decimation), taps_window=win, conj_sum=int(conj), rotate=1,
        rot_step=(w * int(decimation)) % TWO64, rot_base=0, out_scale=c, taps_natural=g.astype(np.complex128),
    )


MFMA_Q = 64
MFMA_KSTEP_BYTES = 8192
MFMA_MAX_KSTEPS_PER_PASS = 16


@dataclass
class MfmaGroup:

    afrag: np.ndarray
    unit: float
    tq: np.ndarray
    q: int = 0
    residual: bool = False
    high_only: bool = False


@dataclass
class MfmaPass:
    group: int
    k_first: int
    k_count: int
    c_re: float
    c_im: float


@dataclass
class MfmaPlan:

    ksteps: int
    groups: list
    passes: list
    err_norm: float = 0.0
    floor_rms: float = 0.0

    @property
    def afrag(self):
        return self.groups[0].afrag

    @property
    def unit(self):
        return self.groups[0].unit

    @property
    def tq(self):
        return self.groups[0].tq

    @property
    def c_re(self):
        return sum(p.c_re for p in self.passes if p.group == 0)

    @property
    def c_im(self):
        return sum(p.c_im for p in self.passes if p.group == 0)

    def z_error_rms(self, wideband_rms: float) -> float:
        return math.hypot(self.err_norm * wideband_rms, self.floor_rms)


def mfma_supported(plan: ChannelPlan) -> bool:
    return plan.fmt in ("s16", "u8") and plan.taps_natural is not None


@functools.lru_cache(maxsize=32)
def _mfma_layout(ntaps: int, decimation: int, group: int):
    L, D = ntaps, decimation
    ksteps = -(-2 * D // 32)
    q = np.arange(1, MFMA_Q + 1, dtype=np.int64)[:, None] + MFMA_Q * group
    rho = np.arange(D, dtype=np.int64)[None, :]
    k = q * D - 1 - rho
    ok = (k >= 0) & (k < L)
    kc = np.clip(k, 0, L - 1)
    lane = np.arange(64)
    rows = (np.arange(4) * 32)[:, None] + (lane & 31)[None, :]
    cols = (32 * np.arange(ksteps))[:, None, None] + (16 * (lane >> 5))[None, :, None] + np.arange(16)[None, None, :]
    flat = (rows[None, :, :, None] * (32 * ksteps) + cols[:, None, :, :]).astype(np.int64)
    return ksteps, kc, ok, flat


_LOW_BYTE_VAR = (256.0 * 256.0 - 1.0) / 12.0


def _quantise_rows(a: np.ndarray, acc32: bool, high_byte_only: bool, col_ranges=None):
    amax = float(np.abs(a).max())
    unit = amax / 32639.0 if amax > 0 else 1.0
    while True:
        if high_byte_only:
            q1 = np.clip(np.rint(a * (1.0 / (256.0 * unit))), -127, 127).astype(np.int32)
            q2 = np.zeros_like(q1)
            t = q1 << 8
        else:
            t = np.rint(a * (1.0 / unit)).astype(np.int32)
            q2 = ((t + 128) & 255) - 128
            q1 = (t - q2) >> 8
        if not acc32:
            break
        w = 128 * (257 * np.abs(q1).astype(np.int64) + np.abs(q2))
        bound = max(int(w[r, c0:c1].sum()) for r in (slice(0, MFMA_Q), slice(MFMA_Q, 2 * MFMA_Q))
                    for c0, c1 in (col_ranges or [(0, a.shape[1])]))
        if bound < 2**31 - 1:
            break
        unit *= max(1.02, bound / (2**31 - 1) * 1.001)
    return unit, t, q1, q2


def plan_mfma(plan: ChannelPlan, acc32: bool = False, max_ksteps: int | None = None, residual: bool = False) -> MfmaPlan:
    if not mfma_supported(plan):
        raise ValueError("MFMA channelizer needs an int16 or uint8 capture")
    g = plan.taps_natural
    D = plan.decimation
    n_groups = max(1, -(-(-(-plan.ntaps // D)) // MFMA_Q))
    groups, passes = [], []
    err_sq = floor_sq = 0.0
    ksteps = -(-2 * D // 32)
    n_chunks = -(-ksteps // (max_ksteps or MFMA_MAX_KSTEPS_PER_PASS))
    bounds = [round(i * ksteps / n_chunks) for i in range(n_chunks + 1)]
    s16 = plan.fmt == "s16"
    for gi in range(n_groups):
        _, kc, ok, flat = _mfma_layout(plan.ntaps, D, gi)
        kpad = 32 * ksteps
        gk = g[kc]
        gre = np.where(ok, gk.real, 0.0)
        gim = np.where(ok, gk.imag, 0.0)
        a = np.zeros((2 * MFMA_Q, kpad), dtype=np.float64)
        a[:MFMA_Q, 0 : 2 * D : 2] = gre
        a[:MFMA_Q, 1 : 2 * D : 2] = -gim
        a[MFMA_Q:, 0 : 2 * D : 2] = gim
        a[MFMA_Q:, 1 : 2 * D : 2] = gre
        left = a
        for part in range(2 if residual else 1):
            unit, t, q1, q2 = _quantise_rows(left, acc32, high_byte_only=residual and part == 0 and s16,
                                             col_ranges=[(32 * bounds[i], 32 * bounds[i + 1]) for i in range(n_chunks)])
            left = left - t * unit
            if s16:
                floor_sq += unit * unit * _LOW_BYTE_VAR * float((q2.astype(np.float64) ** 2).sum())
            frag = np.empty((ksteps, 4, 2, 64, 16), dtype=np.int8)
            frag[:, :, 0] = q1.reshape(-1)[flat]
            frag[:, :, 1] = q2.reshape(-1)[flat]
            groups.append(MfmaGroup(frag, unit, t, q=gi, residual=part == 1, high_only=bool(s16 and not np.any(q2))))
            for ci in range(n_chunks):
                k0, k1 = bounds[ci], bounds[ci + 1]
                sl = t[:, 32 * k0 : 32 * k1]
                bias = 128.0 if s16 else 0.0
                passes.append(MfmaPass(len(groups) - 1, k0, k1 - k0, bias * float(sl[:MFMA_Q].sum(dtype=np.int64)),
                                       bias * float(sl[MFMA_Q:].sum(dtype=np.int64))))
        err_sq += 0.5 * float((left**2).sum())
    return MfmaPlan(ksteps, groups, passes, math.sqrt(err_sq) / INGEST_SCALE[plan.fmt], math.sqrt(floor_sq))


def mfma_interior(consumed: int, n_frames: int, m_first: int, n_out: int, decimation: int, ksteps: int,
                  n_groups: int = 1):
    d = decimation
    m_a = max(m_first, MFMA_Q * n_groups + -(-(consumed - 1) // d))
    m_b = min(m_first + n_out, (n_frames + consumed - 16 * ksteps) // d - 30)
    return (m_a, m_b) if m_b > m_a else (m_first, m_first)


def plan_plain_fir(taps: np.ndarray, padded_len: int | None = None) -> ChannelPlan:
    h = np.asarray(taps, dtype=np.float64)
    lpad = padded_len if padded_len is not None else -(-h.size // 256) * 256
    win = np.zeros(lpad, dtype=np.complex64)
    win[: h.size] = h[::-1].astype(np.complex64)
    return ChannelPlan("f32", h.size, 1, win, 0, 0, 0, 0, 1.0 + 0j)


def chunk_output_starts(chunk: int, decimation: int, first_frame: int, n_frames: int) -> np.ndarray:
    if first_frame % chunk:
        raise ValueError("blocks must start on a chunk boundary")
    d = decimation
    m_first = -(-first_frame // d)
    starts = np.arange(first_frame, first_frame + n_frames, chunk, dtype=np.int64)
    return (-(-starts // d) - m_first).astype(np.int64)



WFM_DEVIATION = 75_000.0
WFM_PILOT_HZ = 19_000.0
WFM_ATTEN_DB = 70.0
WFM_TRANSITION_HZ = 3_000.0
WFM_AUDIO_CUTOFF = 16_500.0
WFM_PILOT_CUTOFF = 1_500.0
WFM_MIN_RATE = 128_000.0
WFM_MAX_TAPS = 2047
WFM_STEREO_LEVEL = 0.01


@dataclass(frozen=True)
class WfmPlan:
    fs: float
    ntaps: int
    delay: int
    h_audio: np.ndarray
    h_pilot: np.ndarray
    m_scale: float
    taps_packed: np.ndarray


def wfm_num_taps(fs_channel: float) -> int:
    n = int(math.ceil((WFM_ATTEN_DB - 7.95) / (2.285 * 2.0 * math.pi * WFM_TRANSITION_HZ / float(fs_channel))))
    return n + 1 if n % 2 == 0 else n


def _kaiser_lowpass(n: int, cutoff: float, fs: float, beta: float) -> np.ndarray:
    fc = cutoff / (0.5 * fs)
    m = np.arange(n, dtype=np.float64) - (n - 1) / 2.0
    h = fc * np.sinc(fc * m) * np.kaiser(n, beta)
    return h / h.sum()


@functools.lru_cache(maxsize=16)
def plan_wfm(fs_channel: float) -> WfmPlan:
    fs = float(fs_channel)
    if not fs >= WFM_MIN_RATE:
        raise ValueError(f"wfm needs a channel rate of at least {WFM_MIN_RATE:.0f} Hz (--fs-ch), not {fs:.0f} Hz")
    n = wfm_num_taps(fs)
    if n > WFM_MAX_TAPS:
        raise ValueError(f"wfm channel rate {fs:.0f} Hz needs {n} taps; at most {WFM_MAX_TAPS} are supported (lower --fs-ch)")
    beta = kaiser_beta(WFM_ATTEN_DB)
    delay = (n - 1) // 2
    h_a = _kaiser_lowpass(n, WFM_AUDIO_CUTOFF, fs, beta)
    k = np.arange(n, dtype=np.float64) - delay
    h_p = _kaiser_lowpass(n, WFM_PILOT_CUTOFF, fs, beta) * np.exp(2j * np.pi * WFM_PILOT_HZ * k / fs)
    packed = np.concatenate([h_a[: delay + 1], h_p.real[: delay + 1], h_p.imag[: delay + 1]]).astype(np.float32)
    for arr in (h_a, h_p, packed):
        arr.setflags(write=False)
    return WfmPlan(fs, n, delay, h_a, h_p, float(np.float32(fs / (2.0 * math.pi * WFM_DEVIATION))), packed)



RDS_SUBCARRIER_HZ = 57_000.0
RDS_BIT_RATE = 1_187.5
RDS_SPAN_SYMBOLS = 2
RDS_MAX_HALF = 2400
RDS_MAX_DECIM = 80
RDS_PHASE_BITS = 44


@dataclass(frozen=True)
class RdsPlan:
    fs: float
    wfm: WfmPlan
    decim: int
    half: int
    h_matched: np.ndarray
    f_mix: float
    clock_step: float
    j0: int
    hist_len: int
    mf_packed: np.ndarray
    pilot_packed: np.ndarray


def _rds_s(v: np.ndarray) -> np.ndarray:
    return 4.0 * np.sinc(4.0 * v)


def rds_pulse(x) -> np.ndarray:
    x = np.asarray(x, dtype=np.float64)
    return 0.5 * (_rds_s(x + 0.125) + _rds_s(x - 0.125))


def rds_symbol(x) -> np.ndarray:
    x = np.asarray(x, dtype=np.float64)
    return rds_pulse(x + 0.25) - rds_pulse(x - 0.25)


@functools.lru_cache(maxsize=16)
def plan_rds(fs_channel: float) -> RdsPlan:
    wfm = plan_wfm(fs_channel)
    fs = wfm.fs
    decim = int(round(fs / WFM_PILOT_HZ))
    spp = fs / RDS_BIT_RATE
    half = int(math.ceil(RDS_SPAN_SYMBOLS * spp))
    if decim > RDS_MAX_DECIM or half > RDS_MAX_HALF:
        raise ValueError(f"RDS at a channel rate of {fs:.0f} Hz needs decimation {decim} and {2 * half + 1} taps; at most "
                         f"{RDS_MAX_DECIM} and {2 * RDS_MAX_HALF + 1} are supported (lower --fs-ch)")
    k = np.arange(2 * half + 1, dtype=np.float64)
    h = rds_symbol(-(k - half) / spp)
    h[half] = 0.0
    h = 0.5 * (h - h[::-1])
    h /= math.sqrt(float(np.sum(h * h)))
    d = wfm.delay
    pilot = np.concatenate([wfm.h_pilot.real[: d + 1], wfm.h_pilot.imag[: d + 1]]).astype(np.float32)
    mf = h[:half].astype(np.float32)
    for arr in (h, pilot, mf):
        arr.setflags(write=False)
    j0 = -(-(2 * (wfm.ntaps - 1) + 2 * half) // decim)
    return RdsPlan(fs, wfm, decim, half, h, RDS_SUBCARRIER_HZ / fs, WFM_PILOT_HZ * decim / fs, j0,
                   2 * half + 2 * (wfm.ntaps - 1), mf, pilot)



POCSAG_BAUDS = (512, 1200, 2400)
POCSAG_MIN_SPS = 8.0
POCSAG_MAX_SPS = 384
POCSAG_THETA_BITS = 20
POCSAG_BATCH_BITS = 544


@dataclass(frozen=True)
class PocsagBaud:
    baud: int
    sps: float
    L: int
    h: int
    offsets: np.ndarray


@dataclass(frozen=True)
class PocsagPlan:
    fs: float
    bauds: tuple
    skipped: tuple
    hist_len: int

    def lengths(self) -> tuple:
        by = {b.baud: b.L for b in self.bauds}
        return tuple(by.get(b, 0) for b in POCSAG_BAUDS)


@functools.lru_cache(maxsize=16)
def plan_pocsag(fs_channel: float) -> PocsagPlan:
    fs = float(fs_channel)
    if not math.isfinite(fs) or fs <= 0.0:
        raise ValueError("the channel rate must be positive")
    bauds, skipped = [], []
    for baud in POCSAG_BAUDS:
        sps = fs / baud
        if sps < POCSAG_MIN_SPS or sps > POCSAG_MAX_SPS:
            skipped.append(baud)
            continue
        offsets = np.rint(np.arange(POCSAG_BATCH_BITS + 1, dtype=np.float64) * sps).astype(np.int32)
        offsets.setflags(write=False)
        bauds.append(PocsagBaud(baud, sps, int(np.rint(sps)), int(math.floor(sps / 2.0)), offsets))
    if not bauds:
        raise ValueError(f"POCSAG needs {POCSAG_MIN_SPS:.0f} to {POCSAG_MAX_SPS} samples per bit at 512, 1200 or 2400 baud; "
                         f"a channel rate of {fs:.0f} Hz gives none of them (--fs-ch between about 20 000 and 190 000)")
    return PocsagPlan(fs, tuple(bauds), tuple(skipped), max(b.L for b in bauds) - 1)



AFSK_BAUD = 1200
AFSK_TONES = (1200, 2200)
AFSK_MIN_SPS = 8.0
AFSK_MAX_SPS = 400
AFSK_THETA_BITS = 12
AFSK_TAP_SCALE = 256.0
AFSK_PHASES = 8
AFSK_GAINS = ((1, 1), (1, 4), (4, 1))


@dataclass(frozen=True)
class AfskPlan:
    fs: float
    sps: float
    L: int
    step: float
    taps: np.ndarray

    def instant(self, i, p: int):
        return self.L - 1 + np.rint((8.0 * np.asarray(i, dtype=np.float64) + p) * self.step).astype(np.int64)

    def bit_count(self, p: int, n: int) -> int:
        i = max(int((n - self.L) / self.sps) - 2, 0)
        while int(self.instant(i, p)) < n:
            i += 1
        return i


@functools.lru_cache(maxsize=16)
def plan_afsk(fs_channel: float) -> AfskPlan:
    fs = float(fs_channel)
    if not math.isfinite(fs) or fs <= 0.0:
        raise ValueError("the channel rate must be positive")
    sps = fs / AFSK_BAUD
    if sps < AFSK_MIN_SPS or sps > AFSK_MAX_SPS:
        raise ValueError(f"AFSK at 1200 baud needs {AFSK_MIN_SPS:.0f} to {AFSK_MAX_SPS} samples per bit; a channel rate of {fs:.0f} Hz "
                         f"gives {sps:.1f} (--fs-ch between 9 600 and 480 000)")
    L = int(np.rint(sps))
    k = np.arange(L, dtype=np.float64)
    rows = []
    for f in AFSK_TONES:
        rows.append(np.rint(AFSK_TAP_SCALE * np.cos(2.0 * np.pi * f * k / fs)))
        rows.append(np.rint(AFSK_TAP_SCALE * np.sin(2.0 * np.pi * f * k / fs)))
    taps = np.ascontiguousarray(np.stack(rows).astype(np.int16))
    taps.setflags(write=False)
    return AfskPlan(fs, sps, L, sps / 8.0, taps)



TONES_RATE = 8000.0
TONES_MAX_R = 64
TONES_THETA_BITS = 12
TONES_TAP_SCALE = 256.0
TONES_NONE = 255
CTCSS_TONES = (67.0, 69.3, 71.9, 74.4, 77.0, 79.7, 82.5, 85.4, 88.5, 91.5, 94.8, 97.4, 100.0, 103.5, 107.2, 110.9, 114.8, 118.8, 123.0,
               127.3, 131.8, 136.5, 141.3, 146.2, 151.4, 156.7, 159.8, 162.2, 165.5, 167.9, 171.3, 173.8, 177.3, 179.9, 183.5, 186.2,
               189.9, 192.8, 196.6, 199.5, 203.5, 206.5, 210.7, 218.1, 225.7, 229.1, 233.6, 241.8, 250.3, 254.1)
DTMF_TONES = (697.0, 770.0, 852.0, 941.0, 1209.0, 1336.0, 1477.0, 1633.0)
DTMF_KEYS = "123A456B789C*0#D"
CTCSS_HOP_S, DTMF_HOP_S = 0.2, 0.01


def _tone_taps(tones, n: int, fd: float) -> np.ndarray:
    k = np.arange(n, dtype=np.float64)
    rows = [[np.rint(TONES_TAP_SCALE * np.cos(2.0 * np.pi * f * k / fd)), np.rint(TONES_TAP_SCALE * np.sin(2.0 * np.pi * f * k / fd))]
            for f in tones]
    taps = np.ascontiguousarray(np.array(rows).astype(np.int16))
    taps.setflags(write=False)
    return taps


@dataclass(frozen=True)
class TonesPlan:
    fs: float
    R: int
    fd: float
    Hd: int
    Nd: int
    Hc: int
    Nc: int
    ctcss_taps: np.ndarray
    dtmf_taps: np.ndarray

    def frames(self, n_frame: int, hop: int, m: int) -> int:
        return 0 if m < n_frame else (m - n_frame) // hop + 1


@functools.lru_cache(maxsize=16)
def plan_tones(fs_channel: float) -> TonesPlan:
    fs = float(fs_channel)
    if not math.isfinite(fs) or fs <= 0.0:
        raise ValueError("the channel rate must be positive")
    R = int(math.floor(fs / TONES_RATE))
    if R < 1 or R > TONES_MAX_R:
        raise ValueError(f"tone detection decimates by floor(fs / 8000), which must be 1 to {TONES_MAX_R}; a channel rate of {fs:.0f} Hz "
                         f"gives {R} (--fs-ch from 8 000 to below 520 000)")
    fd = fs / R
    Hd, Hc = int(np.rint(DTMF_HOP_S * fd)), int(np.rint(CTCSS_HOP_S * fd))
    return TonesPlan(fs, R, fd, Hd, 2 * Hd, Hc, 2 * Hc, _tone_taps(CTCSS_TONES, 2 * Hc, fd), _tone_taps(DTMF_TONES, 2 * Hd, fd))



ACARS_BAUD = 2400
ACARS_CENTRE = 1800.0
ACARS_MIN_SPS = 8.0
ACARS_MAX_SPS = 400
ACARS_TAP_SCALE = 256.0
ACARS_PHASES = 8
ACARS_Q_BITS = 15


@dataclass(frozen=True)
class AcarsPlan:
    fs: float
    sps: float
    L: int
    W: int
    step: float
    taps: np.ndarray
    cr: int
    sr: int

    def instant(self, i, p: int):
        return self.W - 1 + np.rint((8.0 * np.asarray(i, dtype=np.float64) + p) * self.step).astype(np.int64)

    def bit_count(self, p: int, n: int) -> int:
        i = max(int((n - self.W) / self.sps) - 2, 0)
        while int(self.instant(i, p)) < n:
            i += 1
        return i


@functools.lru_cache(maxsize=16)
def plan_acars(fs_channel: float) -> AcarsPlan:
    fs = float(fs_channel)
    if not math.isfinite(fs) or fs <= 0.0:
        raise ValueError("the channel rate must be positive")
    sps = fs / ACARS_BAUD
    if sps < ACARS_MIN_SPS or sps > ACARS_MAX_SPS:
        raise ValueError(f"ACARS at 2400 bit/s needs {ACARS_MIN_SPS:.0f} to {ACARS_MAX_SPS} samples per bit; a channel rate of {fs:.0f} Hz "
                         f"gives {sps:.1f} (--fs-ch between 19 200 and 960 000)")
    L, W = int(np.rint(sps)), int(np.rint(fs / ACARS_CENTRE))
    k = np.arange(W, dtype=np.float64)
    rows = np.stack([np.rint(ACARS_TAP_SCALE * np.cos(2.0 * np.pi * ACARS_CENTRE * k / fs)),
                     np.rint(ACARS_TAP_SCALE * np.sin(2.0 * np.pi * ACARS_CENTRE * k / fs))])
    assert 2 ** ACARS_Q_BITS * max(np.maximum(rows, 0).sum(axis=1).max(), -np.minimum(rows, 0).sum(axis=1).min()) < 2 ** 31
    taps = np.ascontiguousarray(rows.astype(np.int16))
    taps.setflags(write=False)
    psi = 2.0 * np.pi * ACARS_CENTRE * L / fs
    return AcarsPlan(fs, sps, L, W, sps / 8.0, taps, int(np.rint(ACARS_TAP_SCALE * np.cos(psi))), int(np.rint(ACARS_TAP_SCALE * np.sin(psi))))



AIS_BAUD = 9600
AIS_BT = 0.4
AIS_MIN_SPS = 5.0
AIS_MAX_SPS = 100
AIS_THETA_BITS = 12
AIS_T_MAX = 12_868
AIS_TAP_SCALE = 256.0
AIS_PHASES = 8


@dataclass(frozen=True)
class AisPlan:
    fs: float
    sps: float
    L: int
    W: int
    step: float
    taps: np.ndarray

    def instant(self, i, p: int):
        return self.W - 1 + np.rint((8.0 * np.asarray(i, dtype=np.float64) + p) * self.step).astype(np.int64)

    def symbol_count(self, p: int, n: int) -> int:
        i = max(int((n - self.W) / self.sps) - 2, 0)
        while int(self.instant(i, p)) < n:
            i += 1
        return i


@functools.lru_cache(maxsize=16)
def plan_ais(fs_channel: float) -> AisPlan:
    fs = float(fs_channel)
    if not math.isfinite(fs) or fs <= 0.0:
        raise ValueError("the channel rate must be positive")
    sps = fs / AIS_BAUD
    if sps < AIS_MIN_SPS or sps > AIS_MAX_SPS:
        raise ValueError(f"AIS at 9600 bit/s needs {AIS_MIN_SPS:.0f} to {AIS_MAX_SPS} samples per bit; a channel rate of {fs:.0f} Hz "
                         f"gives {sps:.1f} (--fs-ch between 48 000 and 960 000)")
    L = int(np.rint(sps))
    W = 3 * L - 1
    sigma = math.sqrt(math.log(2.0)) / (2.0 * math.pi * AIS_BT) * sps
    k = np.arange(2 * L, dtype=np.float64)
    gauss = np.exp(-((k - (2 * L - 1) / 2.0) ** 2) / (2.0 * sigma * sigma))
    pulse = np.convolve(gauss, np.ones(L, dtype=np.float64))
    h = np.rint(AIS_TAP_SCALE * pulse / pulse.max())
    assert h.size == W and AIS_T_MAX * int(np.abs(h).sum()) < 2 ** 31
    taps = np.ascontiguousarray(h.astype(np.int16))
    taps.setflags(write=False)
    return AisPlan(fs, sps, L, W, sps / 8.0, taps)



ADSB_CHIP_RATE = 2e6
ADSB_MIN_SPS = 2.0
ADSB_MAX_SPS = 20
ADSB_CHIPS = 240
ADSB_Q_MAX = 65535


@dataclass(frozen=True)
class AdsbPlan:
    fs: float
    sps: float
    h: int
    offsets: np.ndarray
    span: int
    L: int


@functools.lru_cache(maxsize=16)
def plan_adsb(fs_channel: float) -> AdsbPlan:
    fs = float(fs_channel)
    if not math.isfinite(fs) or fs <= 0.0:
        raise ValueError("the channel rate must be positive")
    sps = fs / 1e6
    if sps < ADSB_MIN_SPS or sps > ADSB_MAX_SPS:
        raise ValueError(f"Mode S on 1090 MHz needs {ADSB_MIN_SPS:.0f} to {ADSB_MAX_SPS} samples per microsecond; a channel rate of "
                         f"{fs:.0f} Hz gives {sps:.2f} (--fs-ch between 2 000 000 and 20 000 000)")
    h = int(math.floor(sps / 2.0))
    offsets = np.rint(np.arange(ADSB_CHIPS, dtype=np.float64) * (sps / 2.0)).astype(np.int32)
    assert h >= 1 and 6 * h * ADSB_Q_MAX < 2 ** 31
    offsets.setflags(write=False)
    return AdsbPlan(fs, sps, h, offsets, int(offsets[-1]) + h, int(np.rint(sps)))



RS_ZERO_CROSSINGS = 16
RS_CUTOFF = 0.97
RS_KAISER_BETA = 9.0
RS_OUT_RATE = 48_000


@dataclass
class ResamplerPlan:
    in_rate: int
    up: int
    down: int
    half_taps: int
    table: np.ndarray

    def n_out(self, n_in: int) -> int:
        return -(-n_in * self.up // self.down)


def plan_resampler(fs_channel: float, out_rate: int = RS_OUT_RATE) -> ResamplerPlan:
    return _plan_resampler(max(1, int(round(fs_channel))), int(out_rate))


@functools.lru_cache(maxsize=16)
def _plan_resampler(rin: int, out_rate: int) -> ResamplerPlan:
    g = math.gcd(out_rate, rin)
    up, down = out_rate // g, rin // g
    m = max(up, down)
    half = RS_ZERO_CROSSINGS * m
    i = np.arange(-half, half + 1, dtype=np.float64)
    u = i / half
    win = np.i0(RS_KAISER_BETA * np.sqrt(np.clip(1.0 - u * u, 0.0, 1.0))) / np.i0(RS_KAISER_BETA)
    h = np.sinc(RS_CUTOFF * i / m) * win
    h *= up / h.sum()
    t_half = -(-half // up)
    idx = np.arange(up, dtype=np.int64)[:, None] + np.arange(-t_half, t_half + 1, dtype=np.int64)[None, :] * up
    ok = np.abs(idx) <= half
    table = np.ascontiguousarray(np.where(ok, h[np.clip(idx + half, 0, 2 * half)], 0.0), dtype=np.float64)
    table.setflags(write=False)
    return ResamplerPlan(rin, up, down, int(t_half), table)
```

Baseline: 970,100 MS/s.

## Add folded MFMA ring channelizer covering two decimation phases per matrix column

After: 920,400 MS/s. 5.1% lower.

```diff
diff --git a/iq-to-audio_amd/batch.py b/iq-to-audio_amd/batch.py
--- a/iq-to-audio_amd/batch.py
+++ b/iq-to-audio_amd/batch.py
@@ -162,7 +162,10 @@
     @staticmethod
     def padded_capture_frames(decimation: int, ntaps: int) -> tuple[int, int]:
         ksteps = -(-2 * decimation // 32)
-        return 0, 512 * ksteps + 34 * decimation
+        slack = 512 * ksteps + 34 * decimation
+        if _ChannelKernel.ring_fold and P.mfma_fold_supported(ntaps, decimation):
+            slack = max(slack, 512 * -(-4 * decimation // 32) + 2 * decimation)
+        return 0, slack
 
     def submit(self, raw_dev, events=None, enclosing=None, lead_frames: int = 0, resident: bool = False) -> dict:
         torch = D.torch_mod()
diff --git a/iq-to-audio_amd/channelizer.py b/iq-to-audio_amd/channelizer.py
--- a/iq-to-audio_amd/channelizer.py
+++ b/iq-to-audio_amd/channelizer.py
@@ -33,15 +33,15 @@
 
 
 def _launch_lanes(lanes: list, pairs: bool, outputs_per_block: int, raw_dev, n_frames: int, consumed: int, m_first: int,
-                  n_out: int) -> None:
+                  n_out: int, fold: bool = False) -> None:
     (k0, ps0), fmt = lanes[0][:2], lanes[0][0].plan.fmt
     table = (N.MfmaLane * len(lanes))()
     for lane, spec in zip(table, lanes):
         if spec is None:
             continue
         k, ps, z_out, partial_in, partial_out, raw_partials = spec
-        group = k.mfma.groups[ps.group]
-        lane.afrag_dev = k.afrag_dev[ps.group][ps.k_first * P.MFMA_KSTEP_BYTES :].data_ptr()
+        group = (k.mfma_fold if fold else k.mfma).groups[ps.group]
+        lane.afrag_dev = (k.afrag_fold_dev if fold else k.afrag_dev)[ps.group][ps.k_first * P.MFMA_KSTEP_BYTES :].data_ptr()
         lane.z_out_dev, lane.partial_in_dev, lane.partial_out_dev = z_out, partial_in, partial_out
         lane.unit = _tap_unit(group, fmt)
         lane.c_re, lane.c_im = ps.c_re, ps.c_im
@@ -49,7 +49,7 @@
         lane.out_scale_re, lane.out_scale_im = k.params.out_scale_re, k.params.out_scale_im
         lane.conj_sum, lane.rotate = k.params.conj_sum, k.params.rotate
         lane.q_group, lane.finalize, lane.raw_partials = group.q, int(partial_out is None), int(raw_partials)
-        lane.reserved = (0 if k.acc32 else 1) | (2 if group.high_only else 0)
+        lane.reserved = (0 if k.acc32 else 1) | (2 if group.high_only and not fold else 0) | (4 if fold else 0)
         k.last_kernel = f"k_channelize_mfma_{fmt}_ring"
     N.call("iqa_channelize_mfma_pairs" if pairs else "iqa_channelize_mfma_multi", c_int32(P.FMT_CODE[fmt]),
            c_int32(k0.plan.decimation), c_int32(ps0.k_first), c_int32(ps0.k_count), c_int32(outputs_per_block), table,
@@ -62,6 +62,7 @@
     use_mfma = True
     mfma_variant = "ring"
     ring_acc32 = True
+    ring_fold = True
     RING_ROWS_KSTEPS = 11
     mfma_min_outputs = 32768
 
@@ -101,6 +102,15 @@
             if self._ring_mode == 0:
                 self._ring_mode = int(N.lib().iqa_mfma_ring_mode(code, plan.decimation, 0, min(ks_all, self.RING_ROWS_KSTEPS), acc32))
         self._mfma_ok = bool(self.use_mfma and not self.exact and P.mfma_supported(plan) and (plan.fmt == "s16" or self._ring_mode == 2))
+        self.mfma_fold = None
+        self._fold_capable = bool(
+            self._mfma_ok and plan.fmt == "s16" and self._ring_mode == 1 and self.acc32 and not self.residual
+            and P.mfma_fold_supported(plan.ntaps, plan.decimation)
+            and int(N.lib().iqa_mfma_ring_mode(P.FMT_CODE["s16"], 2 * plan.decimation, 0, -(-4 * plan.decimation // 32), 1)) == 1)
+
+    @property
+    def fold(self) -> int:
+        return 2 if self._fold_capable and self.ring_fold else 1
 
     def _ensure_mfma(self):
         with self._lock:
@@ -112,6 +122,9 @@
                 self._passes = [(ps, None if ring else N.MfmaParams(
                     reserved=0, unit=mp.groups[ps.group].unit, c_re=ps.c_re, c_im=ps.c_im, q_group=mp.groups[ps.group].q,
                     k_first=ps.k_first, k_count=ps.k_count)) for ps in mp.passes]
+                if self._fold_capable:
+                    self.mfma_fold = P.plan_mfma(self.plan, acc32=True, fold=2)
+                    self.afrag_fold_dev = [D.from_numpy(g.afrag.reshape(-1).view(np.uint8)) for g in self.mfma_fold.groups]
                 self.mfma = mp
             return self.mfma
 
@@ -134,8 +147,8 @@
         rounds = max(1, -(-n_out // (blocks * rmax)))
         return _block_size(n_out, blocks * rounds, 512, rmax)
 
-    def _workgroups_per_cu(self, ps) -> int:
-        lds = int(N.lib().iqa_mfma_ring_lds_bytes(P.FMT_CODE[self.plan.fmt], self.plan.decimation, ps.k_first, ps.k_count,
+    def _workgroups_per_cu(self, ps, fold: int = 1) -> int:
+        lds = int(N.lib().iqa_mfma_ring_lds_bytes(P.FMT_CODE[self.plan.fmt], fold * self.plan.decimation, ps.k_first, ps.k_count,
                                                   1 if self.acc32 else 0))
         return 2 if 0 < lds <= 80 * 1024 else 1
 
@@ -144,8 +157,10 @@
             N.call("iqa_channelize", byref(self.params), N.ptr(self.taps_dev), N.ptr(raw_dev), c_int64(n_frames),
                    c_int64(consumed), N.ptr(hist_dev), c_int64(m_first), c_int64(n_out), N.ptr(out_dev), N.stream_ptr())
 
-    def _interior(self, consumed: int, n_frames: int, m_first: int, n_out: int) -> tuple[int, int]:
+    def _interior(self, consumed: int, n_frames: int, m_first: int, n_out: int, fold: int | None = None) -> tuple[int, int]:
         d = self.plan.decimation
+        if (self.fold if fold is None else fold) == 2:
+            return P.mfma_interior(consumed, n_frames, m_first, n_out, d, -(-4 * d // 32), 1, fold=2)
         ksteps = -(-2 * d // 32)
         n_groups = max(1, -(-(-(-self.plan.ntaps // d)) // P.MFMA_Q))
         m_a, m_b = P.mfma_interior(consumed, n_frames, m_first, n_out, d, ksteps, n_groups)
@@ -155,6 +170,14 @@
 
     def _mfma_passes(self, raw_dev, n_frames: int, consumed: int, m_a: int, n_int: int, out_dev, min_block: int = 512):
         self._ensure_mfma()
+        if self.fold == 2:
+            (ps,) = self.mfma_fold.passes
+            rng = self._block_outputs(n_int, 1 << 24, self._workgroups_per_cu(self._passes[0][0]))
+            if min_block < 512:
+                rng = _block_size(n_int, 256, min_block, rng)
+            _launch_lanes([(self, ps, out_dev.data_ptr(), None, None, False)], False, rng, raw_dev, n_frames, consumed, m_a, n_int,
+                          fold=True)
+            return
         buf = D.empty(2 * n_int, "float64") if len(self._passes) > 1 else None
         partial = N.ptr(buf).value
         for i, (ps, prm) in enumerate(self._passes):
@@ -404,7 +427,7 @@
         plans = [k._ensure_mfma() for k in kernels]
         if len(kernels) > self.MAX_LANES or any(len(mp.groups) != 1 or len(mp.passes) != 1 for mp in plans):
             return self._run_shared(x_all, n_frames, m_first, n_out, list(outs), None, None, interior_only=True) is not None
-        if any(k._interior(0, n_frames, m_first, n_out) != (m_first, m_first + n_out) for k in kernels):
+        if any(k._interior(0, n_frames, m_first, n_out, fold=1) != (m_first, m_first + n_out) for k in kernels):
             return False
         if len({(mp.passes[0].k_first, mp.passes[0].k_count) for mp in plans}) != 1:
             return False
@@ -421,7 +444,7 @@
         if halo is not None:
             big, lead = halo
             big_frames, big_consumed = int(big.numel()) // 2, consumed - int(lead)
-        spans = [k._interior(big_consumed, big_frames, m_first, n_out) for k in kernels]
+        spans = [k._interior(big_consumed, big_frames, m_first, n_out, fold=1) for k in kernels]
         m_a, m_b = max(s[0] for s in spans), min(s[1] for s in spans)
         if interior_only:
             if any(s != (m_first, m_first + n_out) for s in spans):
diff --git a/iq-to-audio_amd/csrc/channelize_mfma.hip b/iq-to-audio_amd/csrc/channelize_mfma.hip
--- a/iq-to-audio_amd/csrc/channelize_mfma.hip
+++ b/iq-to-audio_amd/csrc/channelize_mfma.hip
@@ -211,7 +211,8 @@
     if (n_out < 0 || n_frames < 0 || m_first < 0) return fail_inval("negative size");
     if (n_out == 0) return IQA_OK;
     if (!afrag_dev || !raw_dev || !z_out_dev) return fail_inval("NULL device pointer");
-    const int ksteps_all = static_cast<int>((2 * D + 31) / 32);
+    const bool fold = ring && (q->reserved & 512) != 0;
+    const int ksteps_all = static_cast<int>(((fold ? 4 : 2) * D + 31) / 32);
     const int k_first = q->k_first;
     const int ksteps = q->k_count > 0 ? q->k_count : ksteps_all - k_first;
     if (k_first < 0 || ksteps <= 0 || k_first + ksteps > ksteps_all) return fail_inval("bad k-step range");
@@ -236,7 +237,7 @@
         l.finalize = q->finalize;
         l.conj_sum = p->conj_sum;
         l.rotate = p->rotate;
-        l.reserved = (q->reserved & 128) ? 0 : 1;
+        l.reserved = ((q->reserved & 128) ? 0 : 1) | (fold ? 4 : 0);
         return channelize_mfma_lanes(p->fmt, p->decimation, k_first, ksteps, range, &l, 1, raw_dev, n_frames, consumed, m_first, n_out,
                                      stream, false);
     }
@@ -316,7 +317,8 @@
     if (n_out < 0 || n_frames < 0 || m_first < 0) return fail_inval("negative size");
     if (n_out == 0) return IQA_OK;
     if (!raw_dev) return fail_inval("NULL device pointer");
-    const int ksteps_all = static_cast<int>((2 * D + 31) / 32);
+    const bool fold = (lanes[0].reserved & 4) != 0;
+    const int ksteps_all = static_cast<int>(((fold ? 4 : 2) * D + 31) / 32);
     const int ksteps = k_count > 0 ? k_count : ksteps_all - k_first;
     if (k_first < 0 || ksteps <= 0 || k_first + ksteps > ksteps_all) return fail_inval("bad k-step range");
     const int range = outputs_per_block;
@@ -324,7 +326,11 @@
     const bool acc64 = (lanes[0].reserved & 1) != 0;
     for (int i = 1; i < n_lanes; ++i)
         if (lanes[i].afrag_dev && ((lanes[i].reserved & 1) != 0) != acc64) return fail_inval("the lanes of a launch share the sum width (reserved bit 0)");
-    const int ring_mode = mfma_ring_mode(static_cast<int>(D), k_first, ksteps, acc64, u8);
+    if (fold && (n_lanes != 1 || pairs || u8 || acc64 || k_first != 0 || lanes[0].q_group != 0 || (lanes[0].reserved & 2) != 0 ||
+                 !mfma_ring_fold_supported(static_cast<int>(D), ksteps)))
+        return fail_inval("the fold variant takes ONE int16 lane with 32-bit sums, tap-row group 0, all k steps of a column of 2 D frames "
+                          "(D % 4 == 0, 9..13 k steps: D = 68..104)");
+    const int ring_mode = fold ? 1 : mfma_ring_mode(static_cast<int>(D), k_first, ksteps, acc64, u8);
     if (ring_mode == 0) return fail_inval("the ring kernel does not cover this (decimation, k-step range, sum width): see iqa_mfma_ring_mode");
     if (acc64 && ring_mode != 1) return fail_inval("64-bit sums: contiguous slots only");
     if (pairs && !mfma_ring_pairs_supported(static_cast<int>(D), k_first, ksteps, u8, acc64))
@@ -342,12 +348,14 @@
     }
     const int64_t blocks = (n_out + range - 1) / range;
     const int64_t last_cnt = n_out - (blocks - 1) * range;
-    const int64_t last_tiles = (last_cnt + 63 + 31) / 32, full_tiles = (static_cast<int64_t>(range) + 63 + 31) / 32;
+    const auto tiles_of = [fold](int64_t cnt) { return fold ? (((cnt + 64) >> 1) + 31) / 32 : (cnt + 63 + 31) / 32; };
+    const int64_t tile_rows = fold ? 64 : 32;
+    const int64_t last_tiles = tiles_of(last_cnt), full_tiles = tiles_of(range);
     const int64_t f_min = (m_first - MF_Q - static_cast<int64_t>(MF_Q) * q_max) * D + 1 - consumed;
     const int64_t tail = ring_mode == 1 ? 512LL * ksteps : 16LL * (k_first + ksteps);
     const int64_t b_last = m_first - MF_Q - static_cast<int64_t>(MF_Q) * q_min;
-    const int64_t t_last = b_last + (blocks - 1) * range + (last_tiles - 1) * 32;
-    const int64_t t_full = blocks > 1 ? b_last + (blocks - 2) * range + (full_tiles - 1) * 32 : t_last;
+    const int64_t t_last = b_last + (blocks - 1) * range + (last_tiles - 1) * tile_rows;
+    const int64_t t_full = blocks > 1 ? b_last + (blocks - 2) * range + (full_tiles - 1) * tile_rows : t_last;
     const int64_t row_span = ring_mode == 1 ? 0 : 31;
     if (f_min < 0 || (t_last + row_span) * D + 1 - consumed + tail > n_frames || (t_full + row_span) * D + 1 - consumed + tail > n_frames)
         return fail_inval("multi-lane ring launch reads outside the block (use iqa_channelize for the edges)");
@@ -393,7 +401,7 @@
         if (s.raw_partials && acc64) return fail_inval("raw partials are int32 sums: not with 64-bit sums");
         l.high_taps_only = (s.reserved & 2) != 0 ? 1 : 0;
     }
-    return mfma_ring_launch_multi(a, packed, n_lanes, lds, as_stream(stream), ring_mode == 2, u8, pairs, acc64);
+    return mfma_ring_launch_multi(a, packed, n_lanes, lds, as_stream(stream), ring_mode == 2, u8, pairs, acc64, fold);
 }
 
 extern "C" int iqa_channelize_mfma_multi(int32_t fmt, int32_t decimation, int32_t k_first, int32_t k_count,
diff --git a/iq-to-audio_amd/csrc/channelize_ring.hip b/iq-to-audio_amd/csrc/channelize_ring.hip
--- a/iq-to-audio_amd/csrc/channelize_ring.hip
+++ b/iq-to-audio_amd/csrc/channelize_ring.hip
@@ -13,17 +13,27 @@
 
 constexpr int RG_MAX_KS = 16;
 constexpr int RG_ROWS_MAX_KS_C = 11;
+constexpr int RG_EMIT_LAG_C = 3;
 constexpr int RG_W = 512;
 constexpr int RG_GUARD = 64;
 constexpr int RG_AS = RG_W + RG_GUARD;
 constexpr int RG_ACC_BYTES = 2 * RG_AS * 8;
+template <int FOLD>
+struct RingWin {
+    static constexpr int W = FOLD == 1 ? RG_W : 1024;
+    static constexpr int AS = W + RG_GUARD;
+    static_assert(FOLD == 1 || FOLD == 2, "one or two data rows per matrix column");
+    static_assert(RG_EMIT_LAG_C * 64 * FOLD + 63 * FOLD + 64 <= W, "emit lag + scatter reach exceed the window");
+    static_assert(FOLD == 1 || 2 * AS * 4 <= RG_ACC_BYTES, "the folded window holds 32-bit sums only");
+};
 constexpr int RG_EMIT_WAVE = 2;
-constexpr int RG_EMIT_LAG = 3;
+constexpr int RG_EMIT_LAG = RG_EMIT_LAG_C;
 constexpr unsigned int RG_PACE_AHEAD = 2;
 constexpr int RG_PACE_SPINS = 20000;
 constexpr int RG_PACE_WORDS = 16384;
 constexpr int RG_PAIR_IDLE = 1 << 28;
 constexpr int RG_LOADERS_MAX_KS = 13;
+constexpr int RG_FOLD_MIN_KS = 9, RG_FOLD_MAX_KS = 13;
 constexpr int RG_ROUNDS_MAX = 5;
 constexpr int RG_PAIR_ROUNDS = 3;
 constexpr int RG_PD = 2;
@@ -107,9 +117,11 @@
     int i;
 };
 
-template <bool ACC64, bool EARLY>
+template <bool ACC64, bool EARLY, int FOLD = 1>
 __device__ __forceinline__ void ring_emit_load(const MfmaArgs &a, const RingCtx &c, int k, RingEmitRegs &g)
 {
+    static_assert(FOLD == 1 || !ACC64, "the folded window holds 32-bit sums");
+    constexpr int RG_W = RingWin<FOLD>::W, RG_AS = RingWin<FOLD>::AS;
     const int pos = 64 * k + 1 + c.lane;
     g.i = pos - MF_Q;
     const int s = pos & (RG_W - 1);
@@ -174,11 +186,11 @@
     e.wc = nc;
 }
 
-template <bool ACC64>
+template <bool ACC64, int FOLD = 1>
 __device__ __forceinline__ void ring_emit_group(const MfmaArgs &a, const RingCtx &c, RingEmit &e, int k)
 {
     RingEmitRegs g;
-    ring_emit_load<ACC64, false>(a, c, k, g);
+    ring_emit_load<ACC64, false, FOLD>(a, c, k, g);
     ring_emit_store<false>(a, c, e, g);
 }
 
@@ -252,9 +264,10 @@
     int x, y, z, w;
 };
 
-template <int KS, bool ACC64, bool ROWS, int HALF, bool PAIR = false>
+template <int KS, bool ACC64, bool ROWS, int HALF, bool PAIR = false, int FOLD = 1>
 __device__ __forceinline__ void ring_loader_split(const MfmaArgs &a, const RingCtx &c)
 {
+    static_assert(FOLD == 1 || (!PAIR && !ROWS && !ACC64), "the fold variant: one lane per workgroup, contiguous slots, 32-bit sums");
     constexpr bool EMITTER = PAIR ? HALF < 2 : HALF == 0;
     constexpr bool UNEVEN = !PAIR && KS >= 12;
     constexpr int P0 = KS >= 12 ? KS - 2 : KS;
@@ -346,6 +359,8 @@
         if constexpr (PAIR) {
             const int re = r - c.tshift, lag = 5 + cp;
             return (re >= lag && ((re - lag) & 1) == 0) ? (re - lag) >> 1 : -1;
+        } else if constexpr (FOLD == 2) {
+            return r >= RG_EMIT_LAG ? 2 * (r - RG_EMIT_LAG) + cp : -1;
         } else {
             return (r >= RG_EMIT_LAG && ((r - RG_EMIT_LAG) & 1) == cp) ? r - RG_EMIT_LAG : -1;
         }
@@ -369,11 +384,11 @@
             asm volatile("" ::: "memory");
             if constexpr (PR_AHEAD) {
                 RingEmitRegs g;
-                ring_emit_load<ACC64, false>(a2, c, k, g);
+                ring_emit_load<ACC64, false, FOLD>(a2, c, k, g);
                 g.pr = pr_now;
                 ring_emit_store<true>(a2, c, em, g);
             } else {
-                ring_emit_group<ACC64>(a2, c, em, k);
+                ring_emit_group<ACC64, FOLD>(a2, c, em, k);
             }
             asm volatile("" ::: "memory");
         }
@@ -405,17 +420,19 @@
             if (c.tshift < RG_PAIR_IDLE)
                 for (int k = k_next; k <= k_last; ++k) ring_emit_group<ACC64>(a2, c, em, k);
         } else {
-            for (int k = max(c.rounds - RG_EMIT_LAG, 0); k <= k_last; ++k)
-                if ((k & 1) == cp) ring_emit_group<ACC64>(a2, c, em, k);
-        }
-    }
-}
-
-template <int KS, bool ACC64, bool ROWS, bool U8, bool ISSUER, bool EMIT, bool DEFER, bool PAIR, typename SKIPT, bool HALF = false>
+            for (int k = FOLD * max(c.rounds - RG_EMIT_LAG, 0); k <= k_last; ++k)
+                if ((k & 1) == cp) ring_emit_group<ACC64, FOLD>(a2, c, em, k);
+        }
+    }
+}
+
+template <int KS, bool ACC64, bool ROWS, bool U8, bool ISSUER, bool EMIT, bool DEFER, bool PAIR, typename SKIPT, bool HALF = false, int FOLD = 1>
 __device__ __forceinline__ void ring_main(const MfmaArgs &a, const RingCtx &c, const v4i_t (&fq)[KS][2], SKIPT)
 {
     constexpr int SKIP = SKIPT::value;
     using G = RingGeo<KS, ROWS, U8, PAIR>;
+    static_assert(FOLD == 1 || (G::SPLIT && !PAIR && !ROWS && !ACC64 && !ISSUER && !EMIT && !HALF), "the fold variant: byte planes, one lane, 32-bit sums");
+    constexpr int RG_W = RingWin<FOLD>::W, RG_AS = RingWin<FOLD>::AS;
     constexpr int R = G::R, SLOT = G::SLOT;
     static_assert(!(ROWS && ISSUER), "row-staged slots are always fed by loader waves");
     const int RG_EMIT_LAG_PAIR = 5 + c.cp;
@@ -452,7 +469,7 @@
     }
     const v16i_t zero16 = {0, 0, 0, 0, 0, 0, 0, 0, 0, 0, 0, 0, 0, 0, 0, 0};
     auto scatter = [&](int t, const v16i_t &acc1, const v16i_t &acc2) {
-        const int slot_idx = ((t * 32 + c.col + 4 * c.h + 1) & (RG_W - 1)) + (rt >> 1) * RG_AS + (rt & 1) * 32;
+        const int slot_idx = ((FOLD * (t * 32 + c.col) + 4 * c.h + 1) & (RG_W - 1)) + (rt >> 1) * RG_AS + (rt & 1) * 32;
         if constexpr (ACC64) {
             const unsigned p = lds_addr(reinterpret_cast<long long *>(c.s_acc) + slot_idx);
 #pragma unroll
@@ -644,7 +661,7 @@
     }
 }
 
-template <int KS, bool ACC64, bool ROWS, bool U8, bool PAIR = false, bool SKIPK = false, bool HALF = false>
+template <int KS, bool ACC64, bool ROWS, bool U8, bool PAIR = false, bool SKIPK = false, bool HALF = false, int FOLD = 1>
 __device__ __forceinline__ void ring_block(const MfmaArgs &a, long long range_idx)
 {
     using G = RingGeo<KS, ROWS, U8, PAIR>;
@@ -663,7 +680,8 @@
     c.i0 = range_idx * a.range;
     c.cnt = static_cast<int>(min(static_cast<long long>(a.range), a.n_out - c.i0));
     c.m0 = a.m_lo + c.i0;
-    c.tiles = (c.cnt + 63 + 31) >> 5;
+    c.tiles = FOLD == 2 ? (((c.cnt + 64) >> 1) + 31) >> 5
+                        : (c.cnt + 63 + 31) >> 5;
     c.rounds = PAIR ? c.tiles + a.pair_extra : (c.tiles + 1) >> 1;
     c.tshift = PAIR ? a.pair_shift : 0;
     c.smem = smem;
@@ -672,7 +690,7 @@
     if (PAIR) c.s_acc += c.cp * (RG_ACC_BYTES / 4);
 
     constexpr int FB = U8 ? 2 : 4;
-    const long long row_bytes = static_cast<long long>(FB) * a.D;
+    const long long row_bytes = static_cast<long long>(FB) * a.D * FOLD;
     c.tile_bytes = 32 * row_bytes;
     const char *stream = reinterpret_cast<const char *>(a.raw) + FB * ((c.m0 - MF_Q - a.col_shift) * a.D + 1 - a.consumed) +
                          (ROWS ? G::KBYTES * a.k_first : 0);
@@ -692,8 +710,8 @@
                     default: ring_loader_split<KS, ACC64, ROWS, 3, true>(a, c); break;
                 }
             } else if constexpr (G::SPLIT) {
-                if ((wave - RG_WAVES) >> 1) ring_loader_split<KS, ACC64, ROWS, 1>(a, c);
-                else ring_loader_split<KS, ACC64, ROWS, 0>(a, c);
+                if ((wave - RG_WAVES) >> 1) ring_loader_split<KS, ACC64, ROWS, 1, false, FOLD>(a, c);
+                else ring_loader_split<KS, ACC64, ROWS, 0, false, FOLD>(a, c);
             } else {
                 ring_loader<KS, ACC64>(a, c);
             }
@@ -738,8 +756,8 @@
         else ring_main<KS, ACC64, ROWS, U8, false, false, false, true>(a, c, fq, std::integral_constant<int, SA>{});
     } else if constexpr (LOADERS) {
         constexpr int S1 = SKIPK ? 1 : 0;
-        if (c.cp) ring_main<KS, ACC64, ROWS, U8, false, false, true, false, std::integral_constant<int, S1>, HALF>(a, c, fq, std::integral_constant<int, S1>{});
-        else ring_main<KS, ACC64, ROWS, U8, false, false, false, false, std::integral_constant<int, S1>, HALF>(a, c, fq, std::integral_constant<int, S1>{});
+        if (c.cp) ring_main<KS, ACC64, ROWS, U8, false, false, true, false, std::integral_constant<int, S1>, HALF, FOLD>(a, c, fq, std::integral_constant<int, S1>{});
+        else ring_main<KS, ACC64, ROWS, U8, false, false, false, false, std::integral_constant<int, S1>, HALF, FOLD>(a, c, fq, std::integral_constant<int, S1>{});
     } else {
         constexpr int S1 = SKIPK ? 1 : 0;
         if ((c.rt >> 1) == c.cp) {
@@ -759,7 +777,7 @@
     MfmaLane lane[RG_MAX_LANES];
 };
 
-template <int KS, bool ROWS, bool U8, bool PAIR = false, bool ACC64 = false, bool SKIPK = false, bool HALF = false>
+template <int KS, bool ROWS, bool U8, bool PAIR = false, bool ACC64 = false, bool SKIPK = false, bool HALF = false, int FOLD = 1>
 __device__ __forceinline__ void ring_multi_block(const RingMultiArgs &m)
 {
     const int idx = blockIdx.x >> 3;
@@ -802,7 +820,7 @@
         a.pace_slot = static_cast<int>(range_idx) * units + idx % units;
     }
     if (range_idx * a.range >= a.n_out) return;
-    ring_block<KS, ACC64, ROWS, U8, PAIR, SKIPK, HALF>(a, range_idx);
+    ring_block<KS, ACC64, ROWS, U8, PAIR, SKIPK, HALF, FOLD>(a, range_idx);
 }
 
 template <int KS, bool ACC64 = false, bool SKIPK = false>
@@ -816,6 +834,13 @@
 {
     static_assert(RingGeo<KS, false>::SPLIT, "byte-plane kernels only");
     ring_multi_block<KS, false, false, false, false, false, true>(m);
+}
+
+template <int KS>
+__global__ __launch_bounds__((RingGeo<KS, false>::THREADS), 3) void k_channelize_mfma_s16_ring_multi_fold(RingMultiArgs m)
+{
+    static_assert(RingGeo<KS, false>::SPLIT && KS >= RG_FOLD_MIN_KS && KS <= RG_FOLD_MAX_KS, "byte-plane kernels, 9..13 k steps");
+    ring_multi_block<KS, false, false, false, false, false, false, 2>(m);
 }
 
 template <int KS, bool ACC64 = false, bool SKIPK = false>
@@ -856,9 +881,18 @@
 }
 
 template <int KS>
-static int ring_launch_multi(const RingMultiArgs &m, unsigned blocks, size_t lds, hipStream_t stream, bool rows, bool u8, bool acc64, bool skipk)
-{
-    static std::atomic<unsigned long long> done[8] = {{0}, {0}, {0}, {0}, {0}, {0}, {0}, {0}};
+static int ring_launch_multi(const RingMultiArgs &m, unsigned blocks, size_t lds, hipStream_t stream, bool rows, bool u8, bool acc64, bool skipk,
+                             bool fold)
+{
+    static std::atomic<unsigned long long> done[9] = {{0}, {0}, {0}, {0}, {0}, {0}, {0}, {0}, {0}};
+    if (fold) {
+        if constexpr (KS >= RG_FOLD_MIN_KS && KS <= RG_FOLD_MAX_KS) {
+            if (!rows && !u8 && !acc64 && !skipk)
+                return ring_launch_kernel(k_channelize_mfma_s16_ring_multi_fold<KS>, "k_channelize_mfma_s16_ring_multi", RingGeo<KS, false>::THREADS, m, blocks, lds, stream, done[8]);
+        }
+        set_error("the fold variant: one int16 lane, contiguous slots, 32-bit sums, %d..%d k steps per column (got %d)", RG_FOLD_MIN_KS, RG_FOLD_MAX_KS, KS);
+        return IQA_EINVAL;
+    }
     if (acc64) {
         if constexpr (KS < RG_MAX_KS) {
             if (!rows && !u8) {
@@ -966,6 +1000,13 @@
     return 0;
 }
 
+bool mfma_ring_fold_supported(int decimation, int k_count)
+{
+    const int ks = (4 * decimation + 31) / 32;
+    return decimation >= 4 && (decimation & 3) == 0 && k_count == ks && ks >= RG_FOLD_MIN_KS && ks <= RG_FOLD_MAX_KS &&
+           mfma_ring_mode(2 * decimation, 0, ks, false, false) == 1;
+}
+
 bool mfma_ring_supported(int decimation)
 {
     const int ks = (2 * decimation + 31) / 32;
@@ -996,8 +1037,12 @@
 }
 
 int mfma_ring_launch_multi(const MfmaArgs &a, const MfmaLane *lanes, int n_lanes, size_t lds, hipStream_t stream, bool rows, bool u8,
-                           bool pairs, bool acc64)
-{
+                           bool pairs, bool acc64, bool fold)
+{
+    if (fold && (pairs || n_lanes != 1)) {
+        set_error("the fold variant takes one lane per launch");
+        return IQA_EINVAL;
+    }
     if (n_lanes < 1 || n_lanes > RG_MAX_LANES) {
         set_error("a multi-lane launch takes 1..%d lanes (got %d)", RG_MAX_LANES, n_lanes);
         return IQA_EINVAL;
@@ -1043,7 +1088,7 @@
         return with_ks<1, RG_MAX_KS>(a.ksteps, [&](auto k) { return ring_launch_pairs<decltype(k)::value>(m, blocks, stream, acc64, skipk); });
     }
     return with_ks<1, RG_MAX_KS>(a.ksteps, [&](auto k) {
-        return ring_launch_multi<decltype(k)::value>(m, blocks, lds, stream, rows, u8, acc64, skipk);
+        return ring_launch_multi<decltype(k)::value>(m, blocks, lds, stream, rows, u8, acc64, skipk, fold);
     });
 }
 
diff --git a/iq-to-audio_amd/csrc/mfma_common.h b/iq-to-audio_amd/csrc/mfma_common.h
--- a/iq-to-audio_amd/csrc/mfma_common.h
+++ b/iq-to-audio_amd/csrc/mfma_common.h
@@ -102,7 +102,8 @@
     int col_shift, finalize, conj_sum, rotate, raw_partials, high_taps_only;
 };
 int mfma_ring_launch_multi(const MfmaArgs &common, const MfmaLane *lanes, int n_lanes, size_t lds_bytes, hipStream_t stream, bool rows,
-                           bool u8, bool pairs, bool acc64);
+                           bool u8, bool pairs, bool acc64, bool fold = false);
+bool mfma_ring_fold_supported(int decimation, int k_count);
 bool mfma_ring_pairs_supported(int decimation, int k_first, int k_count, bool u8, bool acc64 = false);
 
 }
diff --git a/iq-to-audio_amd/dsp_plan.py b/iq-to-audio_amd/dsp_plan.py
--- a/iq-to-audio_amd/dsp_plan.py
+++ b/iq-to-audio_amd/dsp_plan.py
@@ -155,6 +155,7 @@
     passes: list
     err_norm: float = 0.0
     floor_rms: float = 0.0
+    fold: int = 1
 
     @property
     def afrag(self):
@@ -184,12 +185,21 @@
     return plan.fmt in ("s16", "u8") and plan.taps_natural is not None
 
 
+def mfma_fold_rows(ntaps: int, decimation: int) -> int:
+    return -(-ntaps // decimation) + 1
+
+
+def mfma_fold_supported(ntaps: int, decimation: int) -> bool:
+    ks = -(-4 * decimation // 32)
+    return decimation % 4 == 0 and 9 <= ks <= 13 and mfma_fold_rows(ntaps, decimation) <= MFMA_Q
+
+
 @functools.lru_cache(maxsize=32)
-def _mfma_layout(ntaps: int, decimation: int, group: int):
+def _mfma_layout(ntaps: int, decimation: int, group: int, fold: int = 1):
     L, D = ntaps, decimation
-    ksteps = -(-2 * D // 32)
+    ksteps = -(-2 * fold * D // 32)
     q = np.arange(1, MFMA_Q + 1, dtype=np.int64)[:, None] + MFMA_Q * group
-    rho = np.arange(D, dtype=np.int64)[None, :]
+    rho = np.arange(fold * D, dtype=np.int64)[None, :]
     k = q * D - 1 - rho
     ok = (k >= 0) & (k < L)
     kc = np.clip(k, 0, L - 1)
@@ -203,7 +213,7 @@
 _LOW_BYTE_VAR = (256.0 * 256.0 - 1.0) / 12.0
 
 
-def _quantise_rows(a: np.ndarray, acc32: bool, high_byte_only: bool, col_ranges=None):
+def _quantise_rows(a: np.ndarray, acc32: bool, high_byte_only: bool, col_ranges=None, fold: int = 1):
     amax = float(np.abs(a).max())
     unit = amax / 32639.0 if amax > 0 else 1.0
     while True:
@@ -218,7 +228,7 @@
         if not acc32:
             break
         w = 128 * (257 * np.abs(q1).astype(np.int64) + np.abs(q2))
-        bound = max(int(w[r, c0:c1].sum()) for r in (slice(0, MFMA_Q), slice(MFMA_Q, 2 * MFMA_Q))
+        bound = max(int(w[r, c0:c1].sum()) for r in (slice(c * MFMA_Q + g, (c + 1) * MFMA_Q, fold) for c in (0, 1) for g in range(fold))
                     for c0, c1 in (col_ranges or [(0, a.shape[1])]))
         if bound < 2**31 - 1:
             break
@@ -226,36 +236,47 @@
     return unit, t, q1, q2
 
 
-def plan_mfma(plan: ChannelPlan, acc32: bool = False, max_ksteps: int | None = None, residual: bool = False) -> MfmaPlan:
+def plan_mfma(plan: ChannelPlan, acc32: bool = False, max_ksteps: int | None = None, residual: bool = False,
+              fold: int = 1) -> MfmaPlan:
     if not mfma_supported(plan):
         raise ValueError("MFMA channelizer needs an int16 or uint8 capture")
+    if fold not in (1, 2):
+        raise ValueError("fold must be 1 or 2")
     g = plan.taps_natural
     D = plan.decimation
     n_groups = max(1, -(-(-(-plan.ntaps // D)) // MFMA_Q))
+    if fold == 2:
+        if mfma_fold_rows(plan.ntaps, D) > MFMA_Q:
+            raise ValueError(f"fold=2 needs ceil(L/D) + 1 <= {MFMA_Q} tap rows (got {mfma_fold_rows(plan.ntaps, D)})")
+        if residual or plan.fmt != "s16":
+            raise ValueError("fold=2: int16 captures, one tap-row group without residue")
+        n_groups = 1
     groups, passes = [], []
     err_sq = floor_sq = 0.0
-    ksteps = -(-2 * D // 32)
+    ksteps = -(-2 * fold * D // 32)
+    if fold == 2 and ksteps > (max_ksteps or MFMA_MAX_KSTEPS_PER_PASS):
+        raise ValueError("fold=2 needs all k steps of a column in one pass")
     n_chunks = -(-ksteps // (max_ksteps or MFMA_MAX_KSTEPS_PER_PASS))
     bounds = [round(i * ksteps / n_chunks) for i in range(n_chunks + 1)]
     s16 = plan.fmt == "s16"
     for gi in range(n_groups):
-        _, kc, ok, flat = _mfma_layout(plan.ntaps, D, gi)
+        _, kc, ok, flat = _mfma_layout(plan.ntaps, D, gi, fold)
         kpad = 32 * ksteps
         gk = g[kc]
         gre = np.where(ok, gk.real, 0.0)
         gim = np.where(ok, gk.imag, 0.0)
         a = np.zeros((2 * MFMA_Q, kpad), dtype=np.float64)
-        a[:MFMA_Q, 0 : 2 * D : 2] = gre
-        a[:MFMA_Q, 1 : 2 * D : 2] = -gim
-        a[MFMA_Q:, 0 : 2 * D : 2] = gim
-        a[MFMA_Q:, 1 : 2 * D : 2] = gre
+        a[:MFMA_Q, 0 : 2 * fold * D : 2] = gre
+        a[:MFMA_Q, 1 : 2 * fold * D : 2] = -gim
+        a[MFMA_Q:, 0 : 2 * fold * D : 2] = gim
+        a[MFMA_Q:, 1 : 2 * fold * D : 2] = gre
         left = a
         for part in range(2 if residual else 1):
             unit, t, q1, q2 = _quantise_rows(left, acc32, high_byte_only=residual and part == 0 and s16,
-                                             col_ranges=[(32 * bounds[i], 32 * bounds[i + 1]) for i in range(n_chunks)])
+                                             col_ranges=[(32 * bounds[i], 32 * bounds[i + 1]) for i in range(n_chunks)], fold=fold)
             left = left - t * unit
             if s16:
-                floor_sq += unit * unit * _LOW_BYTE_VAR * float((q2.astype(np.float64) ** 2).sum())
+                floor_sq += unit * unit * _LOW_BYTE_VAR * float((q2.astype(np.float64) ** 2).sum()) / fold
             frag = np.empty((ksteps, 4, 2, 64, 16), dtype=np.int8)
             frag[:, :, 0] = q1.reshape(-1)[flat]
             frag[:, :, 1] = q2.reshape(-1)[flat]
@@ -264,16 +285,20 @@
                 k0, k1 = bounds[ci], bounds[ci + 1]
                 sl = t[:, 32 * k0 : 32 * k1]
                 bias = 128.0 if s16 else 0.0
-                passes.append(MfmaPass(len(groups) - 1, k0, k1 - k0, bias * float(sl[:MFMA_Q].sum(dtype=np.int64)),
-                                       bias * float(sl[MFMA_Q:].sum(dtype=np.int64))))
-        err_sq += 0.5 * float((left**2).sum())
-    return MfmaPlan(ksteps, groups, passes, math.sqrt(err_sq) / INGEST_SCALE[plan.fmt], math.sqrt(floor_sq))
+                sums = [(int(sl[g_:MFMA_Q:fold].sum(dtype=np.int64)), int(sl[MFMA_Q + g_ :: fold].sum(dtype=np.int64))) for g_ in range(fold)]
+                assert all(s_ == sums[0] for s_ in sums), "the row classes of a folded tap matrix hold the same taps"
+                passes.append(MfmaPass(len(groups) - 1, k0, k1 - k0, bias * float(sums[0][0]), bias * float(sums[0][1])))
+        err_sq += 0.5 * float((left**2).sum()) / fold
+    return MfmaPlan(ksteps, groups, passes, math.sqrt(err_sq) / INGEST_SCALE[plan.fmt], math.sqrt(floor_sq), fold)
 
 
 def mfma_interior(consumed: int, n_frames: int, m_first: int, n_out: int, decimation: int, ksteps: int,
-                  n_groups: int = 1):
+                  n_groups: int = 1, fold: int = 1):
     d = decimation
     m_a = max(m_first, MFMA_Q * n_groups + -(-(consumed - 1) // d))
+    if fold > 1:
+        m_b = min(m_first + n_out, (n_frames + consumed - 512 * ksteps - 1) // d + 2)
+        return (m_a, m_b) if m_b > m_a else (m_first, m_first)
     m_b = min(m_first + n_out, (n_frames + consumed - 16 * ksteps) // d - 30)
     return (m_a, m_b) if m_b > m_a else (m_first, m_first)
 
```
